# blefaudeux/rusty-marcher

Hardware: AMD Instinct MI355X
Metric: Mpixels/sec at 1920x1080, max-bounce=5 (higher is better)
Workload: dtype f64

## Files before the change

rusty-marcher_amd/csrc/rm_classify.inc:

```
namespace RM_FLAVOR_NS {
using namespace rmdev;

__device__ __forceinline__ V3 unit(V3 a) {
    const double x = dot(a, a);
    double y = __builtin_amdgcn_rsq(x);
    const double h = 0.5 * x;
    y = y * (1.5 - h * y * y);
    y = y * (1.5 - h * y * y);
    return scaled(a, y);
}

#if RM_KERNEL_ORIENTED
__device__ __forceinline__ V3 cls_dir(const KernelArgs &a, double bx, double by) {
    return mk((bx * a.cam_rx + by * a.cam_ux) + a.cam_fx, (bx * a.cam_ry + by * a.cam_uy) + a.cam_fy, (bx * a.cam_rz + by * a.cam_uz) + a.cam_fz);
}
#else
__device__ __forceinline__ V3 cls_dir(const KernelArgs &, double bx, double by) { return mk(bx, by, -1.); }
#endif
template <bool SHARED>
__device__ __forceinline__ bool cone_of(Bundle &b, const KernelArgs &a, double bx0, double bx1, double by0, double by1, uint32_t sub) {
    const V3 u = unit(cls_dir(a, 0.5 * (bx0 + bx1), 0.5 * (by0 + by1)));
    double cm;
    if (SHARED) {
        cm = dot(unit(cls_dir(a, (sub & 1u) ? bx1 : bx0, (sub & 2u) ? by1 : by0)), u);
        cm = __builtin_fmin(cm, __shfl_xor(cm, 1, 64));
        cm = __builtin_fmin(cm, __shfl_xor(cm, 2, 64));
    } else {
        cm = __builtin_fmin(__builtin_fmin(dot(unit(cls_dir(a, bx0, by0)), u), dot(unit(cls_dir(a, bx1, by0)), u)),
                            __builtin_fmin(dot(unit(cls_dir(a, bx0, by1)), u), dot(unit(cls_dir(a, bx1, by1)), u)));
    }
    cm -= 1e-9;
    b.ax = a.cam_x; b.ay = a.cam_y; b.az = a.cam_z;
    b.ux = u.x; b.uy = u.y; b.uz = u.z;
    b.cos2 = cm * cm;
    b.sin_t = (double)__builtin_sqrtf((float)__builtin_fmax((1. - cm) * (1. + cm), 0.)) * (1. + 1e-6) + 1e-7;
    b.chord = (double)__builtin_sqrtf((float)__builtin_fmax(2. * (1. - cm), 0.)) * (1. + 1e-6) + 1e-7;
    b.rho = 0.;
    b.two_sided = false;
    b.narrow = true;
    return cm > 0.5;
}

struct ClsView { const double *bounds, *planar, *poly, *tri; uint32_t poly_stride, tri_stride; };
__device__ __forceinline__ ClsView cls_view_of_blob(const double *blob, const rm_dev_header &H) {
    return ClsView{blob + H.off_bounds, blob + H.off_planar, blob + H.off_polygons, blob + H.off_triangles, RM_POLYGON_WORDS, RM_TRIANGLE_WORDS};
}
__device__ __forceinline__ uint32_t cls_stage_words(const rm_dev_header &H) {
    return 4u * (H.n_spheres + H.n_polygons + H.n_triangles) + 22u * (H.n_polygons + H.n_triangles);
}
__device__ __forceinline__ ClsView cls_stage(const double *__restrict__ blob, const rm_dev_header &H, double *lds) {
    const uint32_t lane = threadIdx.x & 63u, n = H.n_spheres + H.n_polygons + H.n_triangles, npl = H.n_polygons + H.n_triangles;
    double *bounds = lds, *planar = bounds + 4u * n, *poly = planar + 16u * npl, *tri = poly + 6u * H.n_polygons;
    cull_stage(blob, H, lds);
    for (uint32_t i = lane; i < 3u * H.n_polygons; i += 64u)
        reinterpret_cast<double2 *>(poly)[i] = reinterpret_cast<const double2 *>(blob + H.off_polygons + RM_POLYGON_WORDS * (i / 3u))[i % 3u];
    for (uint32_t i = lane; i < 3u * H.n_triangles; i += 64u)
        reinterpret_cast<double2 *>(tri)[i] = reinterpret_cast<const double2 *>(blob + H.off_triangles + RM_TRIANGLE_WORDS * (i / 3u))[i % 3u];
    __syncthreads();
    return ClsView{bounds, planar, poly, tri, 6u, 6u};
}

template <bool EDGES>
__device__ __forceinline__ bool keeps(const ClsView &v, const KernelArgs &a, const Bundle &b, uint32_t pid, bool in) {
    const uint32_t ns = a.H.n_spheres, np = a.H.n_polygons;
    const double2 *bp = reinterpret_cast<const double2 *>(v.bounds) + 2u * (in ? pid : 0u);
    const SphereCull sph = cull_sphere(bp, b);
    bool out = sph.out;
    const bool planar = in & (pid >= ns);
    if (EDGES && __any(planar)) {
        const double2 *pp = reinterpret_cast<const double2 *>(v.planar) + 8u * (planar ? pid - ns : 0u);
        out = out | cull_edges(pp, b, sph, planar & !out);
        const double *recw = !planar ? v.bounds : pid < ns + np ? v.poly + v.poly_stride * (pid - ns) : v.tri + v.tri_stride * (pid - ns - np);
        const double2 *rec = reinterpret_cast<const double2 *>(recw);
        const double2 r0 = rec[0], r1 = rec[1], r2 = rec[2];
        const double nn = (double)__builtin_sqrtf((float)(r0.x * r0.x + r0.y * r0.y + r1.x * r1.x)) * (1. + 1e-6);
        const double num = (r1.y - b.ax) * r0.x + (r2.x - b.ay) * r0.y + (r2.y - b.az) * r1.x;
        const double un = b.ux * r0.x + b.uy * r0.y + b.uz * r1.x, spread = (b.chord + 1e-7) * nn;
        const double tiny = 1e-9 * nn * (__builtin_fabs(r1.y - b.ax) + __builtin_fabs(r2.x - b.ay) + __builtin_fabs(r2.y - b.az)) + 1e-290;
        const bool away = ((num > tiny) & (un + spread < 0.)) | ((num < -tiny) & (un - spread > 0.));
        out = out | (planar & away);
    }
    return in & !out;
}

template <bool EDGES>
__device__ __forceinline__ void keeps2(const ClsView &v, const KernelArgs &a, const Bundle &b, uint32_t pid_a, bool in_a, uint32_t pid_b, bool in_b,
                                       bool &keep_a, bool &keep_b) {
    const uint32_t ns = a.H.n_spheres, np = a.H.n_polygons;
    const double2 *bounds = reinterpret_cast<const double2 *>(v.bounds);
    const SphereCull sph_a = cull_sphere(bounds + 2u * (in_a ? pid_a : 0u), b), sph_b = cull_sphere(bounds + 2u * (in_b ? pid_b : 0u), b);
    bool out_a = sph_a.out, out_b = sph_b.out;
    const bool planar_a = in_a & (pid_a >= ns), planar_b = in_b & (pid_b >= ns);
    if (EDGES && __any(planar_a | planar_b)) {
        const double2 *planar = reinterpret_cast<const double2 *>(v.planar);
        EdgeCull ea = cull_edges_begin(planar + 8u * (planar_a ? pid_a - ns : 0u), b, sph_a, planar_a & !out_a);
        EdgeCull eb = cull_edges_begin(planar + 8u * (planar_b ? pid_b - ns : 0u), b, sph_b, planar_b & !out_b);
        if (__any((ea.nv == 4u) | (eb.nv == 4u))) { cull_edges_fourth(ea, b); cull_edges_fourth(eb, b); }
        out_a = out_a | cull_edges_end(ea, b, planar_a & !out_a);
        out_b = out_b | cull_edges_end(eb, b, planar_b & !out_b);
        auto away = [&](uint32_t pid, bool planar_p) {
            const double *recw = !planar_p ? v.bounds : pid < ns + np ? v.poly + v.poly_stride * (pid - ns) : v.tri + v.tri_stride * (pid - ns - np);
            const double2 *rec = reinterpret_cast<const double2 *>(recw);
            const double2 r0 = rec[0], r1 = rec[1], r2 = rec[2];
            const double nn = (double)__builtin_sqrtf((float)(r0.x * r0.x + r0.y * r0.y + r1.x * r1.x)) * (1. + 1e-6);
            const double num = (r1.y - b.ax) * r0.x + (r2.x - b.ay) * r0.y + (r2.y - b.az) * r1.x;
            const double un = b.ux * r0.x + b.uy * r0.y + b.uz * r1.x, spread = (b.chord + 1e-7) * nn;
            const double tiny = 1e-9 * nn * (__builtin_fabs(r1.y - b.ax) + __builtin_fabs(r2.x - b.ay) + __builtin_fabs(r2.y - b.az)) + 1e-290;
            return planar_p & (((num > tiny) & (un + spread < 0.)) | ((num < -tiny) & (un - spread > 0.)));
        };
        const bool away_a = away(pid_a, planar_a), away_b = away(pid_b, planar_b);
        out_a = out_a | away_a;
        out_b = out_b | away_b;
    }
    keep_a = in_a & !out_a;
    keep_b = in_b & !out_b;
}

struct ClsAsked { double px0, px1, py0, py1, tx0, tx1, ty0, ty1; };
__device__ __forceinline__ ClsAsked classify_ask(const KernelArgs &a, uint32_t patch, bool valid) {
    const uint32_t tile = (valid ? patch : 0u) * 16u + (threadIdx.x & 15u);
    uint32_t tx0, ty0, tyf, ty8;
    tile_origin(a, tile, tx0, ty0, tyf, ty8);
    const uint32_t px0 = tx0 & ~31u, py0 = ty0 & ~31u;
    return ClsAsked{a.bp_x[px0], a.bp_x[px0 + 31u], a.bp_y[py0], a.bp_y[py0 + 31u],
                    a.bp_x[tx0], a.bp_x[tx0 + TILE_W - 1u], a.bp_y[ty0], a.bp_y[ty0 + TILE_H - 1u]};
}
template <bool EDGES>
__device__ __forceinline__ bool classify_patches(const ClsView &scene_blob, const KernelArgs &a, uint32_t patch, bool valid, const ClsAsked &asked,
                                                 unsigned long long *__restrict__ tile_mask, uint32_t n, uint32_t tag, unsigned long long &sig, unsigned long long &own) {
    const uint32_t lane = threadIdx.x & 63u, sub = lane & 15u;
    const uint32_t tile = (valid ? patch : 0u) * 16u + sub;

    Bundle b;
    const bool patch_usable = cone_of<true>(b, a, asked.px0, asked.px1, asked.py0, asked.py1, sub);
    unsigned long long pm = 0ull;
#ifdef RM_CLASSIFY_TWO_CHAINS
    for (uint32_t base = 0; base < n; base += 32u) {
        const uint32_t pid_a = base + sub, pid_b = base + 16u + sub;
        const bool in_a = pid_a < n, in_b = pid_b < n;
        bool keep_a, keep_b;
        keeps2<EDGES>(scene_blob, a, b, pid_a, in_a, pid_b, in_b, keep_a, keep_b);
        pm |= (in_a & (keep_a | !patch_usable)) ? (1ull << (pid_a & 63u)) : 0ull;
        pm |= (in_b & (keep_b | !patch_usable)) ? (1ull << (pid_b & 63u)) : 0ull;
    }
#else
    for (uint32_t base = 0; base < n; base += 16u) {
        const uint32_t pid = base + sub;
        const bool in = pid < n;
        const bool keep = in & (keeps<EDGES>(scene_blob, a, b, pid, in) | !patch_usable);
        pm |= keep ? (1ull << (pid & 63u)) : 0ull;
    }
#endif
    auto group_or = [](unsigned long long v) {
        for (uint32_t off = 1u; off < 16u; off <<= 1) {
            const uint32_t lo = (uint32_t)v | (uint32_t)__shfl_xor((int)(uint32_t)v, (int)off, 64);
            const uint32_t hi = (uint32_t)(v >> 32) | (uint32_t)__shfl_xor((int)(uint32_t)(v >> 32), (int)off, 64);
            v = ((unsigned long long)hi << 32) | lo;
        }
        return v;
    };
    pm = group_or(pm);

    unsigned long long mask = 0ull;
    if (n > (tag ? 56u : 64u)) {
        mask = pm != 0ull ? ~0ull : 0ull;
    } else if (__any(pm != 0ull)) {
        const bool tile_usable = cone_of<false>(b, a, asked.tx0, asked.tx1, asked.ty0, asked.ty1, sub);
        unsigned long long m = pm;
#ifdef RM_CLASSIFY_TWO_CHAINS
        while (__any(m != 0ull)) {
            const bool in_a = m != 0ull;
            const uint32_t pid_a = in_a ? (uint32_t)__builtin_ctzll(m) : 0u;
            m &= m - 1ull;
            const bool in_b = m != 0ull;
            const uint32_t pid_b = in_b ? (uint32_t)__builtin_ctzll(m) : 0u;
            m &= m - 1ull;
            bool keep_a, keep_b;
            keeps2<EDGES>(scene_blob, a, b, pid_a, in_a, pid_b, in_b, keep_a, keep_b);
            mask |= (in_a & (keep_a | !tile_usable)) ? (1ull << pid_a) : 0ull;
            mask |= (in_b & (keep_b | !tile_usable)) ? (1ull << pid_b) : 0ull;
        }
#else
        while (__any(m != 0ull)) {
            const bool in = m != 0ull;
            const uint32_t pid = in ? (uint32_t)__builtin_ctzll(m) : 0u;
            m &= m - 1ull;
            const bool keep = in & (keeps<EDGES>(scene_blob, a, b, pid, in) | !tile_usable);
            mask |= keep ? (1ull << pid) : 0ull;
        }
#endif
    }
    if (valid) {
        if (tag) __hip_atomic_store(tile_mask + tile, ((unsigned long long)tag << 56) | (mask & 0x00FFFFFFFFFFFFFFull), __ATOMIC_RELAXED, __HIP_MEMORY_SCOPE_AGENT);
        else tile_mask[tile] = mask;
    }
    own = valid ? mask : 0ull;
    sig = group_or(own);
    return sig != 0ull;
}

__device__ __forceinline__ uint32_t cost_bucket(uint32_t ticks) {
    if (ticks < 512u) return RM_ORD_SKY - 1u;
    const uint32_t e = 31u - (uint32_t)__builtin_clz(ticks);
    const uint32_t b = 2u * (e - 9u) + ((ticks >> (e - 1u)) & 1u);
    return RM_ORD_SKY - 1u - min(b, RM_ORD_SKY - 1u);
}

struct OrdRec { uint32_t patch, bucket_slot, index; };

// ... 131 lines not shown
```

rusty-marcher_amd/csrc/rm_device.hip:

```cpp
#include <hip/hip_runtime.h>

#include <chrono>
#include <cmath>
#include <cstdio>
#include <cstdlib>
#include <cstring>
#include <initializer_list>
#include <limits>
#include <new>
#include <string>
#include <utility>
#include <vector>

#include "rm_image.hpp"
#include "rm_internal.h"
#include "rm_kernel_args.hpp"
#include "rm_plan.hpp"
#include "rm_sampling.hpp"
#include "rm_query.hpp"
#include "rm_radiance.hpp"
#include "rm_refine.hpp"
#include "rm_lens.hpp"
#include "rm_accum.hpp"
#include "rm_soft.hpp"
// ... 133 lines not shown

    uint32_t *d_pid_map = nullptr;
    size_t pid_map_words = 0;
    void *d_query = nullptr;
    size_t query_bytes = 0;

    std::vector<std::pair<const void *, int>> shade_occupancy;

    void *d_refine_ws = nullptr;
    size_t refine_ws_bytes = 0;

    void *d_lens_table = nullptr;
    void *d_lens_frame = nullptr;
    size_t lens_frame_bytes = 0;

    rm_progressive *progressive = nullptr;

    rm_converging *converging = nullptr;

    unsigned long long *d_max = nullptr;
    uint8_t *d_rgb8 = nullptr;
    size_t rgb8_bytes = 0;
};

static void hostio_destroy(rm_ctx *ctx, bool device_ok);
static bool hostio_packs(rm_ctx *ctx, size_t band_bytes);
static void progressive_destroy(rm_ctx *ctx, bool device_ok);
static void converging_destroy(rm_ctx *ctx, bool device_ok);

static rm_status ctx_fail(rm_ctx *ctx, rm_status st, const std::string &msg) {
    if (ctx) ctx->error = msg;
    else rm_set_host_error(msg);
    return st;
}

template <class F>
static rm_status guarded(rm_ctx *ctx, const char *who, F &&body) {
    try {
        return body();
    } catch (const std::bad_alloc &) {
        return ctx_fail(ctx, RM_ERR_INVALID_ARG, std::string(who) + ": out of host memory");
    } catch (const std::exception &e) {
        return ctx_fail(ctx, RM_ERR_INVALID_ARG, std::string(who) + ": " + e.what());
    } catch (...) {
        return ctx_fail(ctx, RM_ERR_INVALID_ARG, std::string(who) + ": unexpected exception");
    }
}

template <class T>
static T *entry_of(std::vector<T> &v, hipStream_t stream) {
    T *t = nullptr;
    for (T &g : v)
        if (g.stream == stream) t = &g;
    return t;
}

#define RM_HIP(ctx, call)                                                                          \
    do {                                                                                           \
        hipError_t e__ = (call);                                                                   \
        if (e__ != hipSuccess)                                                                     \
            return ctx_fail(ctx, RM_ERR_HIP, std::string(#call) + ": " + hipGetErrorString(e__)); \
    } while (0)

static rm_status grow_device_buffer(rm_ctx *ctx, void **d, size_t *have, size_t need) {
    if (*have >= need) return RM_OK;
    if (*d) RM_HIP(ctx, hipFree(*d));
    *d = nullptr;
    *have = 0;
    RM_HIP(ctx, hipMalloc(d, need));
    *have = need;
    return RM_OK;
}

#define RM_DECLARE_GROUP(g) \
    const void *rm_pick_kernel_strict_g##g(bool edges, int order, int stack, int pow_mode); \
    const void *rm_pick_kernel_fast_g##g(bool edges, int order, int stack, int pow_mode);
#define RM_DECL_PICK_O(g) \
    const void *rm_pick_kernel_strict_o_g##g(bool edges, int order, int stack, int pow_mode); \
    const void *rm_pick_kernel_fast_o_g##g(bool edges, int order, int stack, int pow_mode);
RM_DECL_PICK_O(0) RM_DECL_PICK_O(1) RM_DECL_PICK_O(2) RM_DECL_PICK_O(3)
RM_DECLARE_GROUP(0) RM_DECLARE_GROUP(1) RM_DECLARE_GROUP(2) RM_DECLARE_GROUP(3) RM_DECLARE_GROUP(4)
#undef RM_DECLARE_GROUP

const void *rm_pick_kernel(bool fast, bool staged, bool bvh, bool cull, bool edges, int order, bool feedback, int stack, int pow_mode) {
    const int group = staged ? (cull ? 1 : 0) : !bvh ? 2 : feedback ? 4 : 3;
    if (staged && (bvh || feedback)) return nullptr;
    if (!staged && !cull) return nullptr;
    switch (group) {
    case 0: return fast ? rm_pick_kernel_fast_g0(edges, order, stack, pow_mode) : rm_pick_kernel_strict_g0(edges, order, stack, pow_mode);
    case 1: return fast ? rm_pick_kernel_fast_g1(edges, order, stack, pow_mode) : rm_pick_kernel_strict_g1(edges, order, stack, pow_mode);
    case 2: return fast ? rm_pick_kernel_fast_g2(edges, order, stack, pow_mode) : rm_pick_kernel_strict_g2(edges, order, stack, pow_mode);
    case 3: return fast ? rm_pick_kernel_fast_g3(edges, order, stack, pow_mode) : rm_pick_kernel_strict_g3(edges, order, stack, pow_mode);
    default: return fast ? rm_pick_kernel_fast_g4(edges, order, stack, pow_mode) : rm_pick_kernel_strict_g4(edges, order, stack, pow_mode);
    }
}

const void *rm_pick_kernel_oriented(bool fast, bool staged, bool bvh, bool cull, bool edges, int stack, int pow_mode) {
    const int group = staged ? (cull ? 1 : 0) : !bvh ? 2 : 3;
    if (staged && bvh) return nullptr;
    if (!staged && !cull) return nullptr;
    switch (group) {
    case 0: return fast ? rm_pick_kernel_fast_o_g0(edges, 1, stack, pow_mode) : rm_pick_kernel_strict_o_g0(edges, 1, stack, pow_mode);
    case 1: return fast ? rm_pick_kernel_fast_o_g1(edges, 1, stack, pow_mode) : rm_pick_kernel_strict_o_g1(edges, 1, stack, pow_mode);
    case 2: return fast ? rm_pick_kernel_fast_o_g2(edges, 1, stack, pow_mode) : rm_pick_kernel_strict_o_g2(edges, 1, stack, pow_mode);
    default: return fast ? rm_pick_kernel_fast_o_g3(edges, 1, stack, pow_mode) : rm_pick_kernel_strict_o_g3(edges, 1, stack, pow_mode);
    }
}

extern "C" {

const char *rm_build_info(void) {
    return "rusty-marcher_amd " RM_BUILD_FLAVOR " gfx950 abi5 queries camera ranges radiance antialias lens progressive soft motion moving-shapes converge-motion converge";
}

const char *rm_last_error(const rm_ctx *ctx) {
    return ctx ? ctx->error.c_str() : rm_get_host_error();
}

rm_status rm_init(int device_ordinal, rm_ctx **out) {
    if (!out) return ctx_fail(nullptr, RM_ERR_INVALID_ARG, "rm_init: out is NULL");
    *out = nullptr;
    int n = 0;
    hipError_t e = hipGetDeviceCount(&n);
    if (e != hipSuccess || n <= 0)
        return ctx_fail(nullptr, RM_ERR_NO_DEVICE,
                        std::string("rm_init: no HIP device visible (") + hipGetErrorString(e) +
                            "); this backend has no CPU fallback");
    if (device_ordinal < 0 || device_ordinal >= n)
        return ctx_fail(nullptr, RM_ERR_NO_DEVICE, "rm_init: device ordinal out of range");
    rm_ctx *ctx = new rm_ctx();
    ctx->device = device_ordinal;
    auto bail = [&](const char *what, hipError_t err) {
        rm_set_host_error(std::string("rm_init: ") + what + ": " + hipGetErrorString(err));
        delete ctx;
        return RM_ERR_HIP;
    };
    if ((e = hipSetDevice(device_ordinal)) != hipSuccess) return bail("hipSetDevice", e);
    if ((e = hipGetDeviceProperties(&ctx->prop, device_ordinal)) != hipSuccess) return bail("hipGetDeviceProperties", e);
    if (std::string(ctx->prop.gcnArchName).rfind("gfx950", 0) != 0) {
        rm_set_host_error(std::string("rm_init: device is ") + ctx->prop.gcnArchName +
                          ", this library carries gfx950 code only");
        delete ctx;
        return RM_ERR_NO_DEVICE;
    }
    if ((e = hipStreamCreateWithFlags(&ctx->stream, hipStreamNonBlocking)) != hipSuccess) return bail("hipStreamCreate", e);
    if ((e = hipEventCreate(&ctx->ev0)) != hipSuccess) return bail("hipEventCreate", e);
    if ((e = hipEventCreate(&ctx->ev1)) != hipSuccess) return bail("hipEventCreate", e);
    if ((e = hipMalloc(&ctx->d_max, sizeof(unsigned long long))) != hipSuccess) return bail("hipMalloc", e);
    if ((e = hipMalloc(&ctx->d_redo, sizeof(uint32_t))) != hipSuccess) return bail("hipMalloc", e);
    if ((e = hipMemset(ctx->d_redo, 0, sizeof(uint32_t))) != hipSuccess) return bail("hipMemset", e);
    *out = ctx;
    return RM_OK;
}

void rm_destroy(rm_ctx *ctx) {
    if (!ctx) return;
    (void)hipSetDevice(ctx->device);
    if (ctx->stream && !ctx->comm_failed) (void)hipStreamSynchronize(ctx->stream);
    rm_comm_destroy(ctx);
    const bool device_ok = !ctx->comm_stuck;
    hostio_destroy(ctx, device_ok);
    progressive_destroy(ctx, device_ok);
    converging_destroy(ctx, device_ok);
    if (device_ok) {
        for (rm_frame_slot &s : ctx->slots) {
            if (s.render && !ctx->comm_failed) { (void)hipStreamSynchronize(s.render); (void)hipStreamDestroy(s.render); }
            for (hipEvent_t e : {s.begun, s.rendered, s.gathered, s.exchanged})
// ... 501 lines not shown
        ctx->frame_w = params->frame_width;
        ctx->frame_h = params->frame_height;
    }

    const size_t row_bytes = (size_t)params->frame_width * 3u * sizeof(double);
    const uint32_t n_rows = band.count();
    if (host_rgb && n_rows > 0 && hostio_packs(ctx, (size_t)n_rows * 32u * row_bytes)) {
        std::vector<double *> rows(params->frame_height);
        for (uint32_t y = 0; y < params->frame_height; y++) rows[y] = host_rgb + (size_t)y * params->frame_width * 3u;
        return rm_render_rows(ctx, params, rows.data(), timing);
    }
    RM_HIP(ctx, hipEventRecord(ctx->ev0, ctx->stream));
    st = launch_render(ctx, params, band, ctx->d_frame, nullptr, ctx->stream);
    if (st != RM_OK) return st;
    RM_HIP(ctx, hipEventRecord(ctx->ev1, ctx->stream));

    double d2h_ms = 0.;
    if (host_rgb && n_rows > 0) {
        RM_HIP(ctx, hipStreamSynchronize(ctx->stream));
        const auto t0 = std::chrono::steady_clock::now();
        const uint32_t run = band.stride == 1 ? n_rows : 1u;
        for (uint32_t k = 0; k < n_rows; k += run) {
            const size_t off = (size_t)(band.begin + k * band.stride) * 32u * row_bytes;
            RM_HIP(ctx, hipMemcpy((char *)host_rgb + off, (const char *)ctx->d_frame + off, (size_t)run * 32u * row_bytes,
                                  hipMemcpyDeviceToHost));
        }
        d2h_ms = std::chrono::duration<double, std::milli>(std::chrono::steady_clock::now() - t0).count();
    } else {
        RM_HIP(ctx, hipStreamSynchronize(ctx->stream));
    }
    if (rm_status vst = void_frame_check(ctx, "rm_render")) return vst;
    if (timing) {
        float ms = 0.f;
        RM_HIP(ctx, hipEventElapsedTime(&ms, ctx->ev0, ctx->ev1));
        timing->kernel_ms = ms;
        timing->d2h_ms = d2h_ms;
        timing->total_ms = std::chrono::duration<double, std::milli>(std::chrono::steady_clock::now() - t_begin).count();
    }
    return RM_OK;
}

rm_status rm_render(rm_ctx *ctx, const rm_params *params, double *host_rgb, rm_timing *timing) {
    return guarded(ctx, "rm_render", [&]() { return rm_render_impl(ctx, params, host_rgb, timing); });
}

rm_status rm_kernel_name(rm_ctx *ctx, const rm_params *params, char *buf, size_t buflen) {
    if (!ctx) return ctx_fail(nullptr, RM_ERR_INVALID_ARG, "rm_kernel_name: NULL ctx");
    if (!buf || buflen == 0) return ctx_fail(ctx, RM_ERR_INVALID_ARG, "rm_kernel_name: NULL buffer");
    rm_band band;
    rm_status st = check_params(ctx, params, &band);
    if (st != RM_OK) return st;
    if (params->max_depth == 0) { std::snprintf(buf, buflen, "rm_fill_band_kernel"); return RM_OK; }
    rm_kernel_choice k;
    st = choose_kernel(ctx, params, band.count() * (params->frame_width / RM_PATCH_SIZE) * 16u, &k);
    if (st != RM_OK) return st;
    std::snprintf(buf, buflen, "%s%s::rm_render_static<%d, %d, %d, %d, %s, %s, %s, %s, %s, %s>", k.fast ? "rmdev_fast" : "rmdev_strict", ctx->oriented ? "_o" : "", k.stack,
                  k.pow_mode, k.mode.waves, k.mode.per_wave, k.staged ? "true" : "false", k.bvh ? "true" : "false",
                  k.cull ? "true" : "false", k.edges ? "true" : "false", (k.order || ctx->oriented) ? "true" : "false", k.feedback ? "true" : "false");
    return RM_OK;
}

rm_status rm_launch_stats(rm_ctx *ctx, uint32_t *workgroups, uint32_t *tail_patches) {
    if (!ctx) return ctx_fail(nullptr, RM_ERR_INVALID_ARG, "rm_launch_stats: NULL ctx");
    if (workgroups) *workgroups = ctx->last_launch_grid;
    if (tail_patches) *tail_patches = ctx->last_launch_tail;
    return RM_OK;
}

static rm_status rm_tile_stats_impl(rm_ctx *ctx, void *hip_stream, uint32_t *tiles, uint32_t *tiles_listed) {
    if (!ctx) return ctx_fail(nullptr, RM_ERR_INVALID_ARG, "rm_tile_stats: NULL ctx");
    RM_HIP(ctx, hipSetDevice(ctx->device));
    RM_HIP(ctx, hipDeviceSynchronize());
    const uint32_t n = ctx->last_launch_tiles;
    uint32_t listed = n;
    for (const rm_tile_lists &t : ctx->tile_lists)
        if (t.stream == (hip_stream ? (hipStream_t)hip_stream : ctx->last_launch_stream) && t.block && ctx->last_launch_classified && n <= t.cap) {
            std::vector<unsigned long long> m(n);
            RM_HIP(ctx, hipMemcpy(m.data(), t.mask(), (size_t)n * 8u, hipMemcpyDeviceToHost));
            listed = 0;
            uint32_t hist[64] = {};
            uint64_t bits = 0;
            for (unsigned long long v : m) {
                if (t.s.tagged) v &= 0x00FFFFFFFFFFFFFFull;
                listed += v != 0ull;
                for (int b = 0; b < 64 && v != ~0ull; b++)
                    if (v >> b & 1ull) { hist[b]++; bits++; }
            }
            if (std::getenv("RM_DEBUG_CLASSIFY")) {
                std::fprintf(stderr, "[rm_classify] %u of %u tiles have something to hit, %.2f primitives each; tiles per pid:", listed, n,
                             listed ? (double)bits / listed : 0.);
                for (int b = 0; b < 64; b++)
                    if (hist[b]) std::fprintf(stderr, " %d:%u", b, hist[b]);
                std::fprintf(stderr, "\n");
            }
        }
    if (tiles) *tiles = n;
    if (tiles_listed) *tiles_listed = listed;
    return RM_OK;
}

rm_status rm_tile_stats(rm_ctx *ctx, void *hip_stream, uint32_t *tiles, uint32_t *tiles_listed) {
    return guarded(ctx, "rm_tile_stats", [&]() { return rm_tile_stats_impl(ctx, hip_stream, tiles, tiles_listed); });
}

rm_status rm_device_framebuffer(rm_ctx *ctx, void **device_rgb, size_t *bytes) {
    if (!ctx) return ctx_fail(nullptr, RM_ERR_INVALID_ARG, "rm_device_framebuffer: NULL ctx");
    if (!ctx->d_frame) return ctx_fail(ctx, RM_ERR_INVALID_ARG, "rm_device_framebuffer: nothing rendered yet");
    if (device_rgb) *device_rgb = ctx->d_frame;
    if (bytes) *bytes = ctx->frame_bytes;
    return RM_OK;
}

static rm_status rm_postprocess_impl(rm_ctx *ctx, void *device_rgb, uint32_t w, uint32_t h, int normalize, uint8_t *host_rgb8,
                         double *max_out) {
    if (!ctx) return ctx_fail(nullptr, RM_ERR_INVALID_ARG, "rm_postprocess: NULL ctx");
    RM_HIP(ctx, hipSetDevice(ctx->device));
    double *v = (double *)device_rgb;
    if (!v) {
        if (!ctx->d_frame) return ctx_fail(ctx, RM_ERR_INVALID_ARG, "rm_postprocess: nothing rendered yet");
        if (w != ctx->frame_w || h != ctx->frame_h)
            return ctx_fail(ctx, RM_ERR_INVALID_ARG, "rm_postprocess: size differs from the rendered frame");
        v = ctx->d_frame;
    }
    const size_t n = (size_t)w * h * 3u;
    if (n == 0) return ctx_fail(ctx, RM_ERR_INVALID_ARG, "rm_postprocess: empty frame");
    const unsigned blocks = (unsigned)std::min<size_t>((n + 255) / 256, 2048);
    RM_HIP(ctx, hipMemsetAsync(ctx->d_max, 0, sizeof(unsigned long long), ctx->stream));
    if (normalize) {
        hipLaunchKernelGGL(rm_max_kernel, dim3(blocks), dim3(256), 0, ctx->stream, v, n, ctx->d_max);
        RM_HIP(ctx, hipGetLastError());
    }
    uint8_t *d8 = nullptr;
    if (host_rgb8) {
        if (ctx->rgb8_bytes < n) {
            RM_HIP(ctx, hipStreamSynchronize(ctx->stream));
            if (ctx->d_rgb8) RM_HIP(ctx, hipFree(ctx->d_rgb8));
            ctx->d_rgb8 = nullptr;
            ctx->rgb8_bytes = 0;
            RM_HIP(ctx, hipMalloc(&ctx->d_rgb8, n));
            ctx->rgb8_bytes = n;
        }
        d8 = ctx->d_rgb8;
    }
    if (normalize || d8) {
        hipLaunchKernelGGL(rm_scale_quantize_kernel, dim3(blocks), dim3(256), 0, ctx->stream, v, n, ctx->d_max,
                           normalize ? 1 : 0, d8);
        RM_HIP(ctx, hipGetLastError());
    }
    RM_HIP(ctx, hipStreamSynchronize(ctx->stream));
    if (host_rgb8) RM_HIP(ctx, hipMemcpy(host_rgb8, d8, n, hipMemcpyDeviceToHost));
    if (max_out) {
        unsigned long long bits = 0;
        RM_HIP(ctx, hipMemcpy(&bits, ctx->d_max, sizeof bits, hipMemcpyDeviceToHost));
        std::memcpy(max_out, &bits, sizeof bits);
    }
    return RM_OK;
}

rm_status rm_postprocess(rm_ctx *ctx, void *device_rgb, uint32_t w, uint32_t h, int normalize, uint8_t *host_rgb8,
                         double *max_out) {
    return guarded(ctx, "rm_postprocess", [&]() { return rm_postprocess_impl(ctx, device_rgb, w, h, normalize, host_rgb8, max_out); });
}

}

#include "rm_exchange.inc"
#include "rm_hostio.inc"
#include "rm_query_host.inc"
#include "rm_shade_host.inc"
#include "rm_radiance_host.inc"
#include "rm_refine_host.inc"
#include "rm_lens_host.inc"
#include "rm_accum_host.inc"
#include "rm_soft_host.inc"
#include "rm_motion_host.inc"
#include "rm_motion_shapes_host.inc"
#include "rm_converge_host.inc"
#include "rm_converge_motion_host.inc"
```

rusty-marcher_amd/csrc/rm_kernel_args.hpp:

```cpp
#ifndef RM_KERNEL_ARGS_HPP
#define RM_KERNEL_ARGS_HPP

#include <stdint.h>

#include "rm_internal.h"

#define RM_ORD_BUCKETS 16u
#define RM_ORD_SKY 15u
#define RM_ORD_MAX_CLS 1024u
#define RM_ORD_LINE 32u
#define RM_ORD_SUBS 4u
#define RM_ORD_COUNTERS (RM_ORD_BUCKETS * RM_ORD_SUBS)
#define RM_ORD_FIRST (RM_ORD_COUNTERS * RM_ORD_LINE)
#define RM_ORD_ARRIVE (2u * RM_ORD_COUNTERS * RM_ORD_LINE)
#define RM_ORD_GROUPS (RM_ORD_ARRIVE + (RM_ORD_MAX_CLS / 32u) * RM_ORD_LINE)
#define RM_ORD_GO (RM_ORD_GROUPS + RM_ORD_LINE)
#define RM_ORD_CNT_WORDS (RM_ORD_GO + RM_ORD_LINE)
#define RM_ORD_STATIC_BIT 0x80000000u
#define RM_ORD_FALLBACK_BIT 0x80000000u
#define RM_ORD_PATIENCE 4096u
#define RM_ORD_PATCH_BITS 20u
#define RM_ORD_SKY_BIT (1u << RM_ORD_PATCH_BITS)
#define RM_ORD_TAG_SHIFT (RM_ORD_PATCH_BITS + 1u)
#define RM_ORD_TAG_BITS 11u
// ... 12 lines not shown
enum { POW_GENERIC = 0, POW_INTEGER = 1 };


#ifndef RM_TILE_W
#define RM_TILE_W 16
#endif
constexpr uint32_t TILE_W = RM_TILE_W, TILE_H = 64u / RM_TILE_W;
static_assert(TILE_W == 8 || TILE_W == 16 || TILE_W == 32, "tile width");

struct KernelArgs {
    rm_dev_header H;
    double half_fov, height, width, ratio;
    double cam_x, cam_y, cam_z;
    double bg_x, bg_y, bg_z;
    uint32_t frame_width;
    uint32_t patch_row_begin;
    uint32_t patch_row_stride;
    uint32_t u8_compact;
    uint32_t max_depth;
    uint32_t n_width;
    uint32_t n_tiles;
    uint32_t order_mul;
    uint32_t order_add;
    uint32_t f64_compact;
    double cull_cos;
    uint8_t *frame8;
    const double *bp_x, *bp_y;
    unsigned long long *debug_stamps;
    const uint32_t *fb_list;
    const uint32_t *fb_count;
    const uint8_t *fb_flag;
    const uint32_t *fb_hist;
    uint32_t *fb_next_list, *fb_next_count, *fb_next_hist;
    uint8_t *fb_next_flag;
    uint32_t *fb_zero;
    uint32_t *fb_threshold;
    uint32_t fb_cap;
    uint32_t fb_long_ticks;
    uint32_t fb_target;
    const unsigned long long *tile_mask;
    uint32_t mask_exact;
    uint32_t mask_tag;
    uint32_t mask_tag_prev;
    uint32_t cls_blocks;
    uint32_t cls_prims;
    uint32_t cls_lds_words;
    uint32_t cull_lds_words;
    uint32_t *ord_cnt;
    uint32_t *ord_cnt_next;
    uint32_t *ord_flat;
    const uint32_t *ord_read;
    uint32_t ord_read_tag;
    uint32_t *ord_rec;
    uint32_t ord_cap;
    uint32_t ord_tag;
    uint32_t cls_iters;
    const uint32_t *static_list;
    const uint32_t *dyn_index;
    const uint32_t *dyn_inv;
    uint32_t *static_next, *dyn_index_next, *dyn_inv_next;
    const uint32_t *lists_done;
    uint32_t lists_tag;
    uint32_t *lists_done_next;
    uint32_t n_static;
    uint32_t key_mode;
    uint32_t *patch_cost;
    const uint32_t *cost_prev;
    uint32_t *cost_zero;
    const uint32_t *ctab;
    uint32_t *ctab_cur;
    uint32_t *ctab_zero;
    uint32_t tail_patches;
    uint32_t ov_cap;
    uint32_t first_round;
    uint32_t tail_q;
    unsigned long long *ord_hint;
    unsigned long long *err_word;
    uint32_t launch_seq;
    uint32_t test_stall;
    double cam_rx, cam_ry, cam_rz, cam_ux, cam_uy, cam_uz, cam_fx, cam_fy, cam_fz;
    uint32_t exact_only;
    uint32_t dead_children;
    uint32_t *redo_count;
};

struct ClassifyArgs {
    unsigned long long *tile_mask;
    uint32_t n_prims;
    uint32_t _pad;
};

const void *rm_classify_kernel(bool edges);
const void *rm_classify_kernel_oriented(bool edges);

#define RM_FB_BUCKETS 64u
#define RM_FB_SAMPLE 8u
struct StackEntry {
    double ox, oy, oz, dx, dy, dz, w;
    uint32_t depth, _pad;
};

#define RM_WAVE_L0_DEPTH_WORDS 448u
#define RM_WAVE_BVH_STACK_WORDS 480u
#define RM_WAVE_SUM_WORDS 512u
#define RM_WAVE_PAIR_WORDS 704u
#define RM_WAVE_T0_WORDS 736u
#define RM_WAVE_LDS_WORDS 738u
#define RM_LDS_SCENE_LIMIT_WORDS 512u

}

const void *rm_pick_kernel(bool fast, bool staged, bool bvh, bool cull, bool edges, int order, bool feedback, int stack, int pow_mode);
const void *rm_pick_kernel_oriented(bool fast, bool staged, bool bvh, bool cull, bool edges, int stack, int pow_mode);

#endif
```

rusty-marcher_amd/csrc/rm_kernels.hip:

```cpp
#include "rm_render_kernel.hpp"

#if RM_KERNEL_FAST && RM_KERNEL_ORIENTED
namespace flavour = rmdev_fast_o;
#elif RM_KERNEL_FAST
namespace flavour = rmdev_fast;
#elif RM_KERNEL_ORIENTED
namespace flavour = rmdev_strict_o;
#else
namespace flavour = rmdev_strict;
#endif

using namespace rmdev;

namespace {

template <bool STAGED, bool BVH, bool CULL, bool EDGES, bool ORDER, bool FB>
const void *pick(int stack, int pow_mode) {
#define RM_ROW(S)                                                                                                            \
    if (stack == S)                                                                                                          \
        return pow_mode == POW_INTEGER ? (const void *)flavour::rm_render_static<S, POW_INTEGER, 1, 1, STAGED, BVH, CULL, EDGES, ORDER, FB> \
                                       : (const void *)flavour::rm_render_static<S, POW_GENERIC, 1, 1, STAGED, BVH, CULL, EDGES, ORDER, FB>;
    RM_ROW(4) RM_ROW(8) RM_ROW(16) RM_ROW(32)
#undef RM_ROW
    return nullptr;
}

}

#define RM_PICK_CAT2(a, b, c) rm_pick_kernel_##a##_g##b
#define RM_PICK_CAT(a, b) RM_PICK_CAT2(a, b, )
#if RM_KERNEL_FAST && RM_KERNEL_ORIENTED
#define RM_PICK_NAME RM_PICK_CAT(fast_o, RM_KERNEL_GROUP)
#elif RM_KERNEL_FAST
#define RM_PICK_NAME RM_PICK_CAT(fast, RM_KERNEL_GROUP)
#elif RM_KERNEL_ORIENTED
#define RM_PICK_NAME RM_PICK_CAT(strict_o, RM_KERNEL_GROUP)
#else
#define RM_PICK_NAME RM_PICK_CAT(strict, RM_KERNEL_GROUP)
#endif

template <bool STAGED, bool BVH, bool CULL, bool FB>
static const void *pick_eo(bool edges, int order, int stack, int pow_mode) {
#if RM_KERNEL_ORIENTED
    static_assert(!FB, "no oriented kernels with the tile-level feedback");
    (void)order;
    if constexpr (CULL) {
        if (edges) return pick<STAGED, BVH, CULL, true, true, false>(stack, pow_mode);
    }
    return pick<STAGED, BVH, CULL, false, true, false>(stack, pow_mode);
#else
    if constexpr (FB) {
        return edges ? pick<STAGED, BVH, CULL, true, false, true>(stack, pow_mode) : pick<STAGED, BVH, CULL, false, false, true>(stack, pow_mode);
    } else {
        if constexpr (CULL) {
            if (edges) return order ? pick<STAGED, BVH, CULL, true, true, false>(stack, pow_mode) : pick<STAGED, BVH, CULL, true, false, false>(stack, pow_mode);
        }
        return order ? pick<STAGED, BVH, CULL, false, true, false>(stack, pow_mode) : pick<STAGED, BVH, CULL, false, false, false>(stack, pow_mode);
    }
#endif
}

const void *RM_PICK_NAME(bool edges, int order, int stack, int pow_mode) {
#if RM_KERNEL_GROUP == 0
    return pick_eo<true, false, false, false>(false, order, stack, pow_mode);
#elif RM_KERNEL_GROUP == 1
    return pick_eo<true, false, true, false>(edges, order, stack, pow_mode);
#elif RM_KERNEL_GROUP == 2
    return pick_eo<false, false, true, false>(edges, order, stack, pow_mode);
#elif RM_KERNEL_GROUP == 3
    return pick_eo<false, true, true, false>(edges, order, stack, pow_mode);
#elif RM_KERNEL_GROUP == 4 && !RM_KERNEL_ORIENTED
    return pick_eo<false, true, true, true>(edges, 0, stack, pow_mode);
#else
#error "RM_KERNEL_GROUP must be 0..4"
#endif
}
```

rusty-marcher_amd/csrc/rm_plan.cpp:

```cpp
#include "rm_plan.hpp"

#include <algorithm>
#include <cmath>
#include <cstdlib>
#include <cstring>
#include <string>

using namespace rmdev;

namespace {

enum knob_rule {
    IS_1,
    NOT_0,
    IS_SET,
    ONE_OR_ZERO,
    ATOI,
    ATOI_MIN_0,
    ATOI_MIN_1,
    STRTOUL,
    TILE_ORDER,
    TAIL_PLACE,
    CULL_OFF,
    CULL_COS,
};

struct knob {
    const char *name;
    knob_rule rule;
    bool rm_knobs::*b = nullptr;
    int rm_knobs::*i = nullptr;
    uint32_t rm_knobs::*u = nullptr;
    double rm_knobs::*d = nullptr;
    constexpr knob(const char *n, bool rm_knobs::*f, knob_rule r) : name(n), rule(r), b(f) {}
    constexpr knob(const char *n, int rm_knobs::*f, knob_rule r) : name(n), rule(r), i(f) {}
    constexpr knob(const char *n, uint32_t rm_knobs::*f, knob_rule r) : name(n), rule(r), u(f) {}
    constexpr knob(const char *n, double rm_knobs::*f, knob_rule r) : name(n), rule(r), d(f) {}
};

const knob k_knobs[] = {
    {"RM_FORCE_GENERIC_POW", &rm_knobs::force_generic_pow, IS_1},
    {"RM_FORCE_FAST_FP", &rm_knobs::force_fast_fp, IS_1},
    {"RM_FORCE_UNSTAGED", &rm_knobs::force_unstaged, IS_1},
    {"RM_SHADOW_MASKS", &rm_knobs::shadow_masks, NOT_0},
    {"RM_DEAD_CHILDREN", &rm_knobs::dead_children, NOT_0},
    {"RM_DISABLE_BVH", &rm_knobs::disable_bvh, IS_1},
    {"RM_FORCE_STACK", &rm_knobs::force_stack, ATOI},
    {"RM_FEEDBACK", &rm_knobs::feedback_mode, ONE_OR_ZERO},
    {"RM_FEEDBACK_US", &rm_knobs::feedback_us, ATOI_MIN_1},
    {"RM_FEEDBACK_TARGET", &rm_knobs::feedback_target, ATOI_MIN_0},
    {"RM_DEBUG_EMPTY", &rm_knobs::debug_empty, IS_1},
    {"RM_TILE_CLASSIFY", &rm_knobs::classify_mode, ONE_OR_ZERO},
    {"RM_CLASSIFY_IN_LAUNCH", &rm_knobs::classify_in_launch, IS_1},
    {"RM_PATCH_ORDER", &rm_knobs::patch_order_mode, ONE_OR_ZERO},
    {"RM_SKY_TAIL", &rm_knobs::sky_tail, NOT_0},
    {"RM_SKY_TAIL_FORCE", &rm_knobs::sky_tail_force, ATOI},
    {"RM_PATCH_ORDER_MAX", &rm_knobs::patch_order_max, ATOI_MIN_0},
    {"RM_SKY_TAIL_BIG", &rm_knobs::sky_tail_big, NOT_0},
    {"RM_PATCH_ORDER_MAX_DEEP", &rm_knobs::patch_order_max_deep, ATOI_MIN_0},
    {"RM_SKY_TAIL_ROOM_DIV", &rm_knobs::sky_tail_room_div, ATOI_MIN_1},
    {"RM_SKY_TAIL_BIG_MIN", &rm_knobs::sky_tail_big_min, ATOI_MIN_0},
    {"RM_SKY_TAIL_PLACE", &rm_knobs::sky_tail_place, TAIL_PLACE},
    {"RM_SKY_TAIL_MOTION", &rm_knobs::sky_tail_motion, NOT_0},
    {"RM_SKY_TAIL_CAP", &rm_knobs::sky_tail_cap, ATOI_MIN_0},
    {"RM_ORDER_KEYS", &rm_knobs::order_keys, ATOI},
    {"RM_FIRST_ROUND", &rm_knobs::first_round, ATOI_MIN_0},
    {"RM_FIRST_ROUND_FROM_ORDER", &rm_knobs::first_round_from_order, NOT_0},
    {"RM_ORDER_REUSE", &rm_knobs::order_reuse, NOT_0},
    {"RM_STATIC_ROUNDS", &rm_knobs::static_rounds, ATOI_MIN_1},
    {"RM_CLS_MAX_BLOCKS", &rm_knobs::cls_max_blocks, ATOI_MIN_1},
    {"RM_ORDER_FREEZE", &rm_knobs::order_freeze, ATOI_MIN_0},
    {"RM_ORDER_LATE_PLACES", &rm_knobs::order_late_places, NOT_0},
    {"RM_MASK_REUSE", &rm_knobs::mask_reuse, NOT_0},
    {"RM_CLASSIFY_LDS", &rm_knobs::classify_lds, NOT_0},
    {"RM_CLASSIFY_IN_LAUNCH_PRIMS", &rm_knobs::classify_in_launch_prims, ATOI_MIN_0},
    {"RM_CLASSIFY_MIN_TILES", &rm_knobs::classify_min_tiles, ATOI_MIN_0},
    {"RM_ORD_TAG_WRAP", &rm_knobs::ord_tag_wrap, ATOI_MIN_1},
    {"RM_TEST_STALL_ORDER", &rm_knobs::test_stall_order, ATOI},
    {"RM_TILE_ORDER", &rm_knobs::tile_order, TILE_ORDER},
    {"RM_DISABLE_CULL", &rm_knobs::cull_cos, CULL_OFF},
    {"RM_CULL_COS", &rm_knobs::cull_cos, CULL_COS},
    {"RM_CULL_MIN", &rm_knobs::cull_min_prims, STRTOUL},
    {"RM_CULL_EDGES", &rm_knobs::cull_edges, NOT_0},
    {"RM_CHECKED_NUMERICS", &rm_knobs::checked_numerics, NOT_0},
    {"RM_REFINE_MAX_BLOCKS", &rm_knobs::refine_max_blocks, ATOI_MIN_0},
    {"RM_LENS_MAX_BLOCKS", &rm_knobs::lens_max_blocks, ATOI_MIN_0},
    {"RM_DEBUG_TAIL", &rm_knobs::debug_tail, IS_SET},
};

}

rm_knobs rm_knobs_from_env() {
    rm_knobs kn;
    for (const knob &k : k_knobs) {
        const char *env = std::getenv(k.name);
        if (!env) continue;
        switch (k.rule) {
        case IS_1: kn.*k.b = env[0] == '1'; break;
        case NOT_0: kn.*k.b = env[0] != '0'; break;
        case IS_SET: kn.*k.b = true; break;
        case ONE_OR_ZERO: kn.*k.i = env[0] == '1' ? 1 : 0; break;
        case ATOI: kn.*k.i = std::atoi(env); break;
        case ATOI_MIN_0:
            if (k.i) kn.*k.i = std::max(0, std::atoi(env));
            else kn.*k.u = (uint32_t)std::max(0, std::atoi(env));
            break;
        case ATOI_MIN_1: kn.*k.u = (uint32_t)std::max(1, std::atoi(env)); break;
        case STRTOUL: kn.*k.u = (uint32_t)std::strtoul(env, nullptr, 10); break;
        case TILE_ORDER:
            kn.*k.i = !std::strcmp(env, "reverse") ? TILE_ORDER_REVERSE : !std::strcmp(env, "hash") ? TILE_ORDER_HASH : TILE_ORDER_NATURAL;
            break;
        case TAIL_PLACE: kn.*k.i = env[0] == 'e' && env[1] == 'v' ? 1 : env[0] == 'e' ? 2 : 0; break;
        case CULL_OFF: kn.*k.d = env[0] == '1' ? 2. : kn.*k.d; break;
        case CULL_COS: kn.*k.d = std::max(0.05, std::atof(env)); break;
        }
    }
    if (kn.classify_min_tiles == 0u) kn.classify_min_tiles = RM_CLASSIFY_MIN_TILES_DEFAULT;
    return kn;
}


static constexpr size_t RM_LDS_SCENE_LIMIT_BYTES = RM_LDS_SCENE_LIMIT_WORDS * sizeof(double);
static constexpr uint32_t RM_FEEDBACK_MIN_TILES = 32768;
static constexpr uint32_t RM_CLASSIFY_MAX_COST = 4000;
static constexpr uint32_t RM_CLASSIFY_IN_LAUNCH_MAX_COST = 1000;

bool choose_kernel(const rm_knobs &kn, const rm_plan_scene &sc, const rm_params &p, uint32_t tiles, rm_kernel_choice *k) {
    const rm_dev_header &H = *sc.H;
// ... 64 lines not shown

bool plan_launch(const rm_knobs &kn, const rm_plan_scene &sc, const rm_params &p, const rm_band &band, const rm_stream_state &before,
                 uint32_t order_cap, const rm_feedback_state &fb, unsigned long long hint, rm_launch_plan *out) {
    rm_launch_plan &P = *out;
    KernelArgs &a = P.args;
    const rm_dev_header &H = *sc.H;
    a.H = H;
    a.half_fov = p.half_fov; a.height = p.height; a.width = p.width; a.ratio = p.ratio;
    a.cam_x = sc.camera.x; a.cam_y = sc.camera.y; a.cam_z = sc.camera.z;
    const rm_camera_basis &cb = *sc.basis;
    a.cam_rx = cb.right.x; a.cam_ry = cb.right.y; a.cam_rz = cb.right.z;
    a.cam_ux = cb.up.x; a.cam_uy = cb.up.y; a.cam_uz = cb.up.z;
    a.cam_fx = cb.forward.x; a.cam_fy = cb.forward.y; a.cam_fz = cb.forward.z;
    if (!(std::fabs(sc.camera.x) + std::fabs(sc.camera.y) + std::fabs(sc.camera.z) <= sc.occ_camera_limit)) a.H.off_occ = 0u;
    a.bg_x = p.background.x; a.bg_y = p.background.y; a.bg_z = p.background.z;
    P.exact_only = !kn.checked_numerics || sc.exact_only || rm_camera_exact_only(sc);
    a.exact_only = P.exact_only ? 1u : 0u;
    a.frame_width = p.frame_width;
    a.patch_row_begin = band.begin;
    a.patch_row_stride = band.stride;
    a.u8_compact = (p.flags & RM_FLAG_U8_COMPACT) ? 1u : 0u;
    a.f64_compact = (p.flags & RM_FLAG_F64_COMPACT) ? 1u : 0u;
    a.max_depth = p.max_depth;
    a.n_width = p.frame_width / RM_PATCH_SIZE;
    a.n_tiles = band.count() * a.n_width * 16u;
    a.order_mul = 1; a.order_add = 0;
    if (kn.tile_order == TILE_ORDER_REVERSE && a.n_tiles > 1) {
        a.order_mul = a.n_tiles - 1; a.order_add = a.n_tiles - 1;
    } else if (kn.tile_order == TILE_ORDER_HASH && a.n_tiles > 2) {
        uint32_t mul = (uint32_t)(a.n_tiles * 0.6180339887) | 1u;
        auto gcd = [](uint32_t x, uint32_t y) { while (y) { uint32_t t = x % y; x = y; y = t; } return x; };
        while (gcd(mul, a.n_tiles) != 1) mul += 2;
        a.order_mul = mul % a.n_tiles;
    }

    if (!choose_kernel(kn, sc, p, a.n_tiles, &P.k)) return false;
    const rm_kernel_choice &k = P.k;
    const uint32_t n_prims = k.n_prims, n_planar = k.n_planar;
    a.dead_children = (kn.dead_children && !k.bvh && !k.cull && sc.dead_camera_limit > 0. &&
                       std::fabs(sc.camera.x) + std::fabs(sc.camera.y) + std::fabs(sc.camera.z) <= sc.dead_camera_limit) ? 1u : 0u;
    const uint32_t cull_steps = (n_prims + 63u) / 64u;
    const uint32_t planar_steps = n_planar ? cull_steps - H.n_spheres / 64u : 0u;
    const uint32_t cull_cost = 25u * cull_steps + (k.planar_edges ? 85u * planar_steps : 0u);
    a.cull_cos = cull_cost > RM_CULL_MAX_COST ? 2. : kn.cull_cos;
    a.first_round = sc.n_cus * 4u * (k.edges ? RM_EDGES_WAVES : RM_MIN_WAVES);
    if (kn.first_round >= 0) a.first_round = (uint32_t)kn.first_round;
    P.block = (uint32_t)k.mode.waves * 64u;
    P.lds_bytes = k.lds_bytes;
    const uint32_t per_wg = (uint32_t)(k.mode.waves * k.mode.per_wave);
    P.grid = (a.n_tiles + per_wg - 1) / per_wg;
    P.feedback = k.feedback && per_wg == 1u && !kn.debug_empty;
    if (P.feedback) {
        const rm_feedback_layout L(a.n_tiles);
        rm_feedback_state &next = P.feedback_after;
        next.valid = true;
        next.key[0] = (uint64_t)a.n_tiles | ((uint64_t)p.frame_width << 32);
        next.key[1] = (uint64_t)band.begin | ((uint64_t)band.stride << 32);
        next.key[2] = sc.scene_epoch;
        next.n_tiles = a.n_tiles;
        const bool same = fb.valid && fb.n_tiles == a.n_tiles && std::memcmp(fb.key, next.key, sizeof fb.key) == 0;
        P.feedback_reset = !same;
        P.feedback_bytes = L.bytes();
        P.feedback_set_bytes = L.set_bytes;
        const int r = same ? fb.cur : 0, w = (r + 1) % 3, z = (r + 2) % 3;
        next.cur = w;
        point(P, &KernelArgs::fb_list, RM_BUF_FEEDBACK, L.list(r)); point(P, &KernelArgs::fb_count, RM_BUF_FEEDBACK, L.count(r));
        point(P, &KernelArgs::fb_flag, RM_BUF_FEEDBACK, L.flag(r)); point(P, &KernelArgs::fb_hist, RM_BUF_FEEDBACK, L.hist(r));
        point(P, &KernelArgs::fb_next_list, RM_BUF_FEEDBACK, L.list(w)); point(P, &KernelArgs::fb_next_count, RM_BUF_FEEDBACK, L.count(w));
        point(P, &KernelArgs::fb_next_flag, RM_BUF_FEEDBACK, L.flag(w)); point(P, &KernelArgs::fb_next_hist, RM_BUF_FEEDBACK, L.hist(w));
        point(P, &KernelArgs::fb_zero, RM_BUF_FEEDBACK, L.hist(z));
        point(P, &KernelArgs::fb_threshold, RM_BUF_FEEDBACK, L.threshold());
        a.fb_cap = L.cap;
        a.fb_long_ticks = kn.feedback_us * 100u;
        const uint32_t slots = sc.n_cus * 16u;
        a.fb_target = kn.feedback_target >= 0 ? (uint32_t)kn.feedback_target : 4u * slots;
        a.fb_target = std::min(a.fb_target, L.cap / 2u);
        P.grid = a.n_tiles + L.cap;
    }
    if (kn.debug_empty) a.n_tiles = 0;

    rm_stream_state s = before;
    uint32_t mask_tag_before = 0u;
    uint32_t cls_words_wanted = 0u;
    P.classify = kn.classify_mode != 0 && !kn.debug_empty && per_wg == 1u && n_prims > 0u &&
                 k.classify_cost <= RM_CLASSIFY_MAX_COST && (kn.classify_mode == 1 || a.n_tiles >= kn.classify_min_tiles);
    if (P.classify) {
        const bool in_launch = kn.classify_in_launch && (n_prims <= kn.classify_in_launch_prims || k.order_in_big_scene) && !k.feedback;
        if (in_launch) {
            if (!s.tagged || s.tagged_tiles != a.n_tiles || s.tagged_scene != sc.scene_epoch || s.tag >= 255u) {
                P.clear_masks = true;
                s.tag = 0;
                s.tagged = true; s.tagged_tiles = a.n_tiles; s.tagged_scene = sc.scene_epoch;
            }
            a.mask_tag = ++s.tag;
            mask_tag_before = a.mask_tag > 1u ? a.mask_tag - 1u : 0u;
            a.cls_blocks = (a.n_tiles / 16u + 3u) / 4u;
            a.cls_prims = n_prims;
            P.grid += a.cls_blocks;
            cls_words_wanted = (!k.staged && kn.classify_lds) ? 4u * n_prims + 22u * n_planar : 0u;
        } else {
            s.tagged = false;
            P.cls_fn = sc.oriented ? rm_classify_kernel_oriented(n_planar > 0u) : rm_classify_kernel(n_planar > 0u);
            P.cls_grid = (a.n_tiles / 16u + 3u) / 4u;
            P.cls_args.n_prims = n_prims;
        }
        point(P, &KernelArgs::tile_mask, RM_BUF_MASKS, 0);
        a.mask_exact = n_prims <= (in_launch ? 56u : 64u) ? 1u : 0u;
    }
    const uint32_t n_patches = a.n_tiles / 16u;
    const uint64_t rounds = (uint64_t)a.first_round * kn.static_rounds * 2u <= a.n_tiles ? kn.static_rounds : 1u;
    a.n_static = (uint32_t)std::min<uint64_t>(((uint64_t)a.first_round * rounds) & ~15ull, a.n_tiles);
    const uint32_t n_dyn = n_patches - a.n_static / 16u;
    const uint32_t cls_max = std::min<uint32_t>(RM_ORD_MAX_CLS, std::max(1u, kn.cls_max_blocks));
    P.ordered = k.order && per_wg == 1u && a.cls_blocks != 0u && n_dyn > 0u && n_patches < (1u << RM_ORD_PATCH_BITS) &&
                n_patches <= 16u * 4u * cls_max;
    if (P.ordered) {
        const uint64_t key[3] = {(uint64_t)a.n_tiles | ((uint64_t)p.frame_width << 32), (uint64_t)band.begin | ((uint64_t)band.stride << 32),
                                 sc.scene_epoch ^ ((uint64_t)a.n_static << 40)};
        P.order_patches = n_patches;
        const bool grown = order_cap < n_patches;
        const rm_order_layout L{grown ? n_patches : order_cap};
        P.order_cap = (uint32_t)L.cap;
        const uint32_t tag_wrap = kn.ord_tag_wrap ? kn.ord_tag_wrap : (1u << RM_ORD_TAG_BITS) - 1u;
        const bool fresh = grown || std::memcmp(s.order_key, key, sizeof key) != 0;
        if (fresh || s.ord_tag >= tag_wrap) {
            P.order_clear = fresh ? rm_launch_plan::ORDER_CLEAR_ALL : rm_launch_plan::ORDER_CLEAR_FLAT;
            if (fresh) {
                std::memcpy(s.order_key, key, sizeof key);
                s.order_frames = 0;
                s.static_read = s.static_written = -1;
                s.list_tag[0] = s.list_tag[1] = 0u;
            }
            s.ord_tag = 0;
            s.last_tag = 0;
        }
        const uint32_t f = s.order_frames++;
        const uint32_t seq = ++s.seq;
        if (f == 0u) s.key_seq0 = seq;
        const double view[16] = {sc.camera.x, sc.camera.y, sc.camera.z, p.half_fov, p.height, p.width, p.ratio,
                                 cb.right.x, cb.right.y, cb.right.z, cb.up.x, cb.up.y, cb.up.z, cb.forward.x, cb.forward.y, cb.forward.z};
        if (f == 0u || std::memcmp(s.view, view, sizeof view) != 0) {
            std::memcpy(s.view, view, sizeof view);
            s.view_seq0 = seq;
        }
        const bool timed = n_patches <= (k.order_in_big_scene ? kn.patch_order_max_deep : kn.patch_order_max);
        const uint32_t groups4 = (n_patches + 3u) / 4u;
        a.cls_iters = (groups4 + cls_max - 1u) / cls_max;
        a.cls_blocks = (groups4 + a.cls_iters - 1u) / a.cls_iters;
        const bool reuse = kn.order_reuse && f >= 3u && seq >= s.view_seq0 + 3u && s.last_tag != 0u;
        a.ord_cap = P.order_cap;
        a.ord_tag = ++s.ord_tag;
        a.ord_read_tag = reuse ? s.last_tag : a.ord_tag;
        s.last_tag = a.ord_tag;
        const bool late_places = reuse && kn.order_late_places;
        a.mask_tag_prev = reuse && kn.mask_reuse ? mask_tag_before : 0u;
        P.frozen = kn.order_freeze > 0 && reuse && f >= 4u && before.frozen_run < (uint32_t)kn.order_freeze && a.mask_tag > 1u &&
                   a.mask_tag_prev != 0u && late_places && kn.test_stall_order == 0 && kn.sky_tail_force < 0 && !kn.debug_tail;
        const bool lays_out = !P.frozen;
        point(P, &KernelArgs::ord_cnt, RM_BUF_ORDER, 4u * L.cnt(f & 1u));
        point(P, &KernelArgs::ord_flat, RM_BUF_ORDER, 4u * L.flat(f & 1u));
        point(P, &KernelArgs::ord_read, RM_BUF_ORDER, 4u * L.flat(reuse ? (f + 1u) & 1u : f & 1u));
        if (lays_out) point(P, &KernelArgs::ord_cnt_next, RM_BUF_ORDER, 4u * L.cnt((f + 1u) & 1u));
        if (lays_out && late_places) point(P, &KernelArgs::ord_rec, RM_BUF_ORDER, 4u * L.rec());
        if (timed) point(P, &KernelArgs::patch_cost, RM_BUF_ORDER, 4u * L.cost(f % 3u));
        if (timed) point(P, &KernelArgs::cost_prev, RM_BUF_ORDER, 4u * L.cost((f + 2u) % 3u));
        if (timed && lays_out) point(P, &KernelArgs::cost_zero, RM_BUF_ORDER, 4u * L.cost((f + 1u) % 3u));
        point(P, &KernelArgs::ctab, RM_BUF_ORDER, 4u * L.ctab((f + 2u) % 3u));
        if (timed && kn.order_keys != 1) point(P, &KernelArgs::ctab_cur, RM_BUF_ORDER, 4u * L.ctab(f % 3u));
        if (lays_out) point(P, &KernelArgs::ctab_zero, RM_BUF_ORDER, 4u * L.ctab((f + 1u) % 3u));
        if (kn.first_round_from_order) {
            const int read = reuse ? s.static_read : s.static_written;
            const uint32_t write = read == 0 ? 1u : 0u;
            if (read >= 0) {
                point(P, &KernelArgs::static_list, RM_BUF_ORDER, 4u * L.first((uint32_t)read));
                point(P, &KernelArgs::dyn_index, RM_BUF_ORDER, 4u * L.index((uint32_t)read));
                point(P, &KernelArgs::dyn_inv, RM_BUF_ORDER, 4u * L.inv((uint32_t)read));
                point(P, &KernelArgs::lists_done, RM_BUF_ORDER, 4u * (L.done() + (uint32_t)read));
                a.lists_tag = s.list_tag[read];
            }
            if (lays_out) {
                point(P, &KernelArgs::static_next, RM_BUF_ORDER, 4u * L.first(write));
                point(P, &KernelArgs::dyn_index_next, RM_BUF_ORDER, 4u * L.index(write));
                point(P, &KernelArgs::dyn_inv_next, RM_BUF_ORDER, 4u * L.inv(write));
                point(P, &KernelArgs::lists_done_next, RM_BUF_ORDER, 4u * (L.done() + write));
            }
            s.list_tag[write] = a.ord_tag;
            s.static_read = read;
            s.static_written = (int)write;
        } else {
            s.static_read = s.static_written = -1;
        }
        a.key_mode = !timed || f == 0u || kn.order_keys == 0 ? RM_KEY_PLACE
                   : (seq > s.view_seq0 && kn.order_keys != 2) ? RM_KEY_COST
                   : (a.mask_exact && a.mask_tag && kn.order_keys != 1) ? RM_KEY_CONTENT : RM_KEY_PLACE;
        point(P, &KernelArgs::ord_hint, RM_BUF_HINT, 0);
        point(P, &KernelArgs::err_word, RM_BUF_HINT, sizeof(unsigned long long));
        a.launch_seq = seq;
        a.test_stall = (uint32_t)kn.test_stall_order;
        uint32_t tail = 0, cap = 0;
        if (kn.sky_tail) {
            bool guess = false;
            if (kn.sky_tail_force >= 0) {
                tail = std::min((uint32_t)kn.sky_tail_force, n_dyn);
                guess = true;
            } else {
                const uint32_t h_seq = (uint32_t)(hint >> 32), n_lit = (uint32_t)hint;
                const bool valid = h_seq >= s.key_seq0 && h_seq < seq && hint != 0ull && n_lit <= n_dyn;
                guess = h_seq < s.view_seq0 + 1u;
                if (valid && (!guess || kn.sky_tail_motion)) tail = n_dyn - n_lit;
                if (tail < 8u) tail = 0u;
            }
            if (tail) cap = std::min(tail, kn.sky_tail_cap >= 0 ? (uint32_t)kn.sky_tail_cap : guess ? std::max(768u, n_patches / kn.sky_tail_room_div) : 32u);
        }
        a.tail_patches = tail;
        a.ov_cap = cap;
        const uint64_t behind = 16ull * (n_dyn - tail);
        a.tail_q = (tail && behind) ? (uint32_t)((((uint64_t)tail << 32) + behind + tail - 1u) / (behind + tail)) : 0u;
        if (a.tail_q > 1u && (kn.sky_tail_place == 2 || (kn.sky_tail_place == 0 && timed))) a.tail_q = 1u;
        if (P.frozen) {
            a.cls_blocks = 0u; a.cls_iters = 0u; a.cls_prims = 0u;
            a.mask_tag = a.mask_tag_prev = before.tag;
            cls_words_wanted = 0u;
            s = before;
            s.frozen_run = before.frozen_run + 1u;
        } else {
            s.frozen_run = 0u;
        }
        P.grid = a.cls_blocks + a.n_static + 16u * (n_dyn - tail) + tail + 16u * cap + (lays_out && late_places ? a.cls_blocks : 0u);
    }
    if (cls_words_wanted) {
        const uint32_t rec_words = (std::max(a.cls_iters, 1u) * 4u * 3u + 1u) / 2u;
        if (cls_words_wanted + rec_words <= (k.edges ? 1664u : 1248u)) {
            a.cls_lds_words = cls_words_wanted;
            P.lds_bytes = std::max(P.lds_bytes, (size_t)(cls_words_wanted + rec_words) * sizeof(double));
        }
    }
    P.after = s;
    return true;
// ... 8 lines not shown
    band->end = e;
    band->stride = p.patch_row_stride == 0 ? 1u : p.patch_row_stride;
    return true;
}

struct rmi_plan_case {
    uint32_t n_spheres, n_polygons, n_triangles, total_words;
    uint32_t bvh, integer_exponents, oriented, n_cus;
    uint64_t scene_epoch;
    rm_params params;
    rm_vec3 camera;
    rm_camera_basis basis;
    unsigned long long hint;
};
struct rmi_plan_row {
    uint32_t grid, block, lds_bytes;
    uint32_t fast, stack, pow_mode, waves, per_wave, staged, bvh, cull, edges, order, feedback;
    uint32_t classify, classify_in_front, ordered, frozen;
    uint32_t clear_masks, order_patches, order_clear;
    uint32_t n_tiles, cls_blocks, cls_iters, n_static, tail_patches, ov_cap, key_mode, mask_tag, mask_tag_prev, ord_tag, ord_read_tag, launch_seq;
    uint32_t reads_own_order, late_places;
    rm_stream_state after;
};
extern "C" rm_status rmi_plan_launches(const rmi_plan_case *cases, uint32_t n, rmi_plan_row *rows) {
    if (!cases || !rows) { rm_set_host_error("rmi_plan_launches: NULL argument"); return RM_ERR_INVALID_ARG; }
    const rm_knobs kn = rm_knobs_from_env();
    rm_stream_state s;
    rm_feedback_state fb;
    uint32_t order_cap = 0;
    for (uint32_t i = 0; i < n; i++) {
        const rmi_plan_case &c = cases[i];
        rm_dev_header H{};
        H.n_spheres = c.n_spheres; H.n_polygons = c.n_polygons; H.n_triangles = c.n_triangles; H.total_words = c.total_words;
        H.off_bvh_spheres = c.bvh;
        const rm_plan_scene sc{&H, c.scene_epoch, 0., c.integer_exponents != 0, c.oriented != 0, c.camera, &c.basis, c.n_cus};
        rm_band band;
        rm_launch_plan P;
        if (!rm_band_of(c.params, &band) || band.count() == 0 || !plan_launch(kn, sc, c.params, band, s, order_cap, fb, c.hint, &P)) {
            rm_set_host_error("rmi_plan_launches: launch " + std::to_string(i) + " has no plan");
            return RM_ERR_INVALID_ARG;
        }
        auto offset_of = [&](size_t field) {
            for (uint32_t r = 0; r < P.n_refs; r++)
                if (P.refs[r].field == field) return P.refs[r].offset + 1u;
            return 0u;
        };
        const KernelArgs &a = P.args;
        const rm_kernel_choice &k = P.k;
        rows[i] = rmi_plan_row{P.grid, P.block, (uint32_t)P.lds_bytes,
                               k.fast, (uint32_t)k.stack, (uint32_t)k.pow_mode, (uint32_t)k.mode.waves, (uint32_t)k.mode.per_wave, k.staged, k.bvh, k.cull, k.edges, k.order || c.oriented, k.feedback,
                               P.classify, P.cls_fn != nullptr, P.ordered, P.frozen, P.clear_masks, P.order_patches, (uint32_t)P.order_clear,
                               a.n_tiles, a.cls_blocks, a.cls_iters, a.n_static, a.tail_patches, a.ov_cap, a.key_mode, a.mask_tag, a.mask_tag_prev, a.ord_tag, a.ord_read_tag, a.launch_seq,
                               P.ordered && offset_of(offsetof(KernelArgs, ord_read)) == offset_of(offsetof(KernelArgs, ord_flat)), offset_of(offsetof(KernelArgs, ord_rec)) != 0u,
                               P.after};
        if (P.classify) s = P.after;
        if (P.ordered) order_cap = P.order_cap;
        if (P.feedback) fb = P.feedback_after;
    }
    return RM_OK;
}

extern "C" rm_status rmi_plan_dead_children(const rm_vec3 *camera, double dead_camera_limit, uint32_t n_spheres, uint32_t n_polygons,
                                            uint32_t n_triangles, uint32_t total_words, uint32_t *out) {
    if (!camera || !out) { rm_set_host_error("rmi_plan_dead_children: NULL argument"); return RM_ERR_INVALID_ARG; }
    const rm_knobs kn = rm_knobs_from_env();
    rm_dev_header H{};
    H.n_spheres = n_spheres; H.n_polygons = n_polygons; H.n_triangles = n_triangles; H.total_words = total_words;
    const rm_camera_basis basis{rm_vec3{1., 0., 0.}, rm_vec3{0., 1., 0.}, rm_vec3{0., 0., -1.}};
    const rm_plan_scene sc{&H, 1u, 0., true, false, *camera, &basis, 256u, false, dead_camera_limit};
    rm_params p{};
    p.half_fov = 0.75; p.height = 64.; p.width = 64.; p.ratio = 1.;
    p.frame_width = 64; p.frame_height = 64; p.max_depth = 3;
    rm_band band;
    rm_launch_plan P;
    if (!rm_band_of(p, &band) || !plan_launch(kn, sc, p, band, rm_stream_state{}, 0u, rm_feedback_state{}, 0ull, &P)) {
        rm_set_host_error("rmi_plan_dead_children: no plan");
        return RM_ERR_INVALID_ARG;
    }
    out[0] = P.args.dead_children;
    out[1] = (!P.k.bvh && !P.k.cull) ? 1u : 0u;
    return RM_OK;
}

extern "C" rm_status rmi_plan_exact_only(const rm_vec3 *camera, const rm_camera_basis *basis, uint32_t oriented, uint32_t scene_exact_only, uint32_t *out) {
    if (!camera || !basis || !out) { rm_set_host_error("rmi_plan_exact_only: NULL argument"); return RM_ERR_INVALID_ARG; }
    const rm_knobs kn = rm_knobs_from_env();
    rm_dev_header H{};
    H.n_spheres = 1; H.total_words = 128;
    const rm_plan_scene sc{&H, 1u, 0., true, oriented != 0, *camera, basis, 256u, scene_exact_only != 0};
    rm_params p{};
    p.half_fov = 0.75; p.height = 64.; p.width = 64.; p.ratio = 1.;
    p.frame_width = 64; p.frame_height = 64; p.max_depth = 3;
    rm_band band;
    rm_launch_plan P;
    if (!rm_band_of(p, &band) || !plan_launch(kn, sc, p, band, rm_stream_state{}, 0u, rm_feedback_state{}, 0ull, &P)) {
        rm_set_host_error("rmi_plan_exact_only: no plan");
        return RM_ERR_INVALID_ARG;
    }
    *out = (P.exact_only ? 1u : 0u) | (P.args.exact_only ? 2u : 0u);
    return RM_OK;
}

extern "C" rm_status rmi_shading_launch(const uint32_t *header, uint32_t integer_exponents, uint32_t max_depth, uint32_t *variant,
                                        uint32_t total, uint32_t rays_per_pixel, int32_t n_cus, int32_t per_cu, uint32_t max_blocks,
                                        uint32_t *grid) {
    if (header) {
        if (!variant) { rm_set_host_error("rmi_shading_launch: NULL variant"); return RM_ERR_INVALID_ARG; }
        rm_dev_header H{};
        std::memcpy(&H, header, 19u * sizeof(uint32_t));
        const rm_shading_variant v = rm_shading_variant_of(rm_knobs_from_env(), H, integer_exponents != 0, max_depth);
        variant[0] = v.bvh ? 1u : 0u; variant[1] = (uint32_t)v.pow_mode; variant[2] = (uint32_t)v.stack;
    }
    if (grid) {
        if (rays_per_pixel < 1u || rays_per_pixel > 64u) { rm_set_host_error("rmi_shading_launch: rays_per_pixel is outside 1..64"); return RM_ERR_INVALID_ARG; }
        *grid = rm_shading_grid(total, rays_per_pixel, n_cus, per_cu, max_blocks);
    }
    return RM_OK;
}
```

rusty-marcher_amd/csrc/rm_plan.hpp:

```cpp
#ifndef RM_PLAN_HPP
#define RM_PLAN_HPP

#include <stddef.h>
#include <stdint.h>

#include "rm_internal.h"
#include "rm_kernel_args.hpp"

enum { TILE_ORDER_NATURAL = 0, TILE_ORDER_REVERSE = 1, TILE_ORDER_HASH = 2 };

static constexpr uint32_t RM_CLASSIFY_MIN_TILES_DEFAULT = 3584;
static constexpr uint32_t RM_CULL_MIN_PRIMS = 12, RM_CULL_EDGES_MIN_PLANAR = 4, RM_CULL_MAX_COST = 250;

struct rm_knobs {
    bool force_generic_pow = false;
    bool force_fast_fp = false;
    int tile_order = TILE_ORDER_REVERSE;
    bool disable_bvh = false;
    double cull_cos = 0.975;
    uint32_t cull_min_prims = RM_CULL_MIN_PRIMS;
    bool cull_edges = true;
    bool force_unstaged = false;
    bool shadow_masks = true;
    bool dead_children = true;
    int force_stack = 0;
    bool debug_empty = false;
    int feedback_mode = -1;
    uint32_t feedback_us = 50;
    int feedback_target = -1;
    int classify_mode = -1;
    bool classify_in_launch = true;
    bool sky_tail = true;
    uint32_t patch_order_max = 4096;
    uint32_t patch_order_max_deep = 65536;
    uint32_t sky_tail_big_min = 16384;
    uint32_t sky_tail_room_div = 16;
    bool sky_tail_big = true;
    bool sky_tail_motion = true;
    int sky_tail_place = 0;
    int sky_tail_cap = -1;
    bool classify_lds = true;
    uint32_t classify_in_launch_prims = 56;
    uint32_t classify_min_tiles = RM_CLASSIFY_MIN_TILES_DEFAULT;
    bool mask_reuse = true;
    uint32_t static_rounds = 2;
    uint32_t cls_max_blocks = RM_ORD_MAX_CLS;
    int order_freeze = 7;
    bool order_late_places = true;
    bool order_reuse = true;
    bool first_round_from_order = true;
    int first_round = -1;
    int order_keys = -1;
    uint32_t ord_tag_wrap = 0;
    int test_stall_order = 0;
    int sky_tail_force = -1;
    int patch_order_mode = -1;
    bool checked_numerics = true;
    uint32_t refine_max_blocks = 0;
    uint32_t lens_max_blocks = 0;
    bool debug_tail = false;
};
rm_knobs rm_knobs_from_env();

struct rm_band {
    uint32_t begin = 0, end = 0, stride = 1;
    uint32_t count() const { return end > begin ? (end - begin + stride - 1) / stride : 0; }
};

bool rm_band_of(const rm_params &p, rm_band *band);

struct rm_plan_scene {
    const rm_dev_header *H;
    uint64_t scene_epoch;
    double occ_camera_limit;
    bool integer_exponents;
    bool oriented;
    rm_vec3 camera;
    const rm_camera_basis *basis;
    uint32_t n_cus;
    bool exact_only = false;
    double dead_camera_limit = 0.;
};

static constexpr double RM_CHECKED_COORD_MAX = 0x1p+200;
static constexpr double RM_CHECKED_R2_MIN = 0x1p-600, RM_CHECKED_R2_MAX = 0x1p+600;
inline bool rm_checked_coord_ok(double v) { return v >= -RM_CHECKED_COORD_MAX && v <= RM_CHECKED_COORD_MAX; }
bool rm_camera_exact_only(const rm_plan_scene &sc);

struct rm_launch_mode {
    int waves = 0;
    int per_wave = 1;
};

struct rm_kernel_choice {
    const void *fn = nullptr;
    rm_launch_mode mode;
    size_t lds_bytes = 0;
    int stack = 0, pow_mode = 0;
    bool fast = false, staged = false, bvh = false, cull = false, edges = false, order = false, feedback = false;
    bool order_in_big_scene = false;
    uint32_t n_prims = 0, n_planar = 0, classify_cost = 0;
    bool planar_edges = false;
};
bool choose_kernel(const rm_knobs &kn, const rm_plan_scene &sc, const rm_params &p, uint32_t tiles, rm_kernel_choice *k);

struct rm_shading_variant {
    bool bvh;
    int pow_mode;
    int stack;
};
rm_shading_variant rm_shading_variant_of(const rm_knobs &kn, const rm_dev_header &H, bool integer_exponents, uint32_t max_depth);

uint32_t rm_shading_grid(uint32_t total, uint32_t rays_per_pixel, int n_cus, int per_cu, uint32_t max_blocks);

struct rm_stream_state {
    uint32_t order_frames = 0;
    uint64_t order_key[3] = {0, 0, 0};
    uint32_t list_tag[2] = {0, 0};
    int static_read = -1, static_written = -1;
    uint32_t last_tag = 0;
    uint32_t seq = 0, view_seq0 = 0, key_seq0 = 0, ord_tag = 0;
    double view[16] = {0., 0., 0., 0., 0., 0., 0., 0., 0., 0., 0., 0., 0., 0., 0., 0.};
    uint32_t tag = 0, tagged_tiles = 0;
    uint64_t tagged_scene = 0;
    bool tagged = false;
    uint32_t frozen_run = 0;
};

struct rm_feedback_state {
    bool valid = false;
    uint64_t key[3] = {0, 0, 0};
    uint32_t n_tiles = 0;
    int cur = 0;
};

struct rm_order_layout {
    size_t cap;
    size_t cost(uint32_t j) const { return (size_t)j * cap; }
    size_t ctab(uint32_t j) const { return 3u * cap + j * RM_CTAB_WORDS; }
    size_t cnt(uint32_t j) const { return 3u * cap + 3u * RM_CTAB_WORDS + j * RM_ORD_CNT_WORDS; }
    size_t flat(uint32_t j) const { return cnt(2) + (size_t)j * cap; }
    size_t first(uint32_t j) const { return flat(2u + j); }
    size_t index(uint32_t j) const { return flat(4u + j); }
    size_t inv(uint32_t j) const { return flat(6u + j); }
    size_t rec() const { return flat(8u); }
    size_t done() const { return rec() + 3u * (cap + 4096u); }
    size_t bytes() const { return (cap * 11u + 64u + 3u * (cap + 4096u) + 3u * RM_CTAB_WORDS + 2u * RM_ORD_CNT_WORDS) * 4u; }
};

struct rm_feedback_layout {
    uint32_t n_tiles, cap;
    size_t set_bytes;
    explicit rm_feedback_layout(uint32_t tiles)
        : n_tiles(tiles), cap((tiles + 7u) / 8u > 64u ? (tiles + 7u) / 8u : 64u),
          set_bytes((((size_t)cap + RM_FB_BUCKETS + 4u) * sizeof(uint32_t) + tiles + 255u) & ~(size_t)255u) {}
    size_t hist(int j) const { return (size_t)j * set_bytes; }
    size_t count(int j) const { return hist(j) + RM_FB_BUCKETS * 4u; }
    size_t list(int j) const { return hist(j) + (RM_FB_BUCKETS + 4u) * 4u; }
    size_t flag(int j) const { return list(j) + (size_t)cap * 4u; }
    size_t threshold() const { return hist(3); }
    size_t bytes() const { return 3u * set_bytes + 256u; }
};

enum rm_buf : uint8_t { RM_BUF_MASKS, RM_BUF_ORDER, RM_BUF_HINT, RM_BUF_FEEDBACK, RM_BUF_COUNT };
struct rm_arg_ref {
    uint16_t field;
    rm_buf buf;
    uint32_t offset;
};

struct rm_launch_plan {
    rm_kernel_choice k;
    uint32_t grid = 0, block = 0;
    size_t lds_bytes = 0;
    rmdev::KernelArgs args{};
    rm_arg_ref refs[40];
    uint32_t n_refs = 0;
    bool feedback = false;
    bool classify = false;
    const void *cls_fn = nullptr;
    uint32_t cls_grid = 0;
    rmdev::ClassifyArgs cls_args{};
    bool exact_only = false;
    bool ordered = false;
    bool frozen = false;
    bool feedback_reset = false;
    size_t feedback_bytes = 0, feedback_set_bytes = 0;
    bool clear_masks = false;
    uint32_t order_patches = 0;
    enum { ORDER_CLEAR_NONE, ORDER_CLEAR_FLAT, ORDER_CLEAR_ALL } order_clear = ORDER_CLEAR_NONE;
    uint32_t order_cap = 0;
    rm_stream_state after;
    rm_feedback_state feedback_after;
};

bool plan_launch(const rm_knobs &kn, const rm_plan_scene &sc, const rm_params &p, const rm_band &band, const rm_stream_state &s,
                 uint32_t order_cap, const rm_feedback_state &fb, unsigned long long hint, rm_launch_plan *out);

#endif
```

rusty-marcher_amd/csrc/rm_render_kernel.hpp:

```cpp
#ifndef RM_RENDER_KERNEL_HPP
#define RM_RENDER_KERNEL_HPP

#include <hip/hip_runtime.h>

#include "rm_kernel_args.hpp"

namespace rmdev {

__device__ __forceinline__ uint32_t fb_bucket(uint32_t ticks) {
    const uint32_t t = ticks < 4u ? 4u : ticks;
    const uint32_t e = 31u - (uint32_t)__builtin_clz(t);
    const uint32_t b = 4u * (e - 2u) + ((t >> (e - 2u)) & 3u);
    return b < RM_FB_BUCKETS ? b : RM_FB_BUCKETS - 1u;
}
__device__ __forceinline__ uint32_t fb_edge(uint32_t b) { return (4u + (b & 3u)) << (b >> 2); }

__device__ __forceinline__ double own_sgpr(double v) { double r; asm("s_mov_b64 %0, %1" : "=s"(r) : "s"(v)); return r; }
__device__ __forceinline__ uint32_t own_sgpr(uint32_t v) { uint32_t r; asm("s_mov_b32 %0, %1" : "=s"(r) : "s"(v)); return r; }

__device__ __forceinline__ uint32_t uniform_u32(uint32_t v) { return (uint32_t)__builtin_amdgcn_readfirstlane((int)v); }
__device__ __forceinline__ unsigned long long uniform_u64(unsigned long long v) {
    return ((unsigned long long)uniform_u32((uint32_t)(v >> 32)) << 32) | uniform_u32((uint32_t)v);
}

__device__ __forceinline__ bool lists_ok(const KernelArgs &a) {
    return a.static_list && a.lists_done && uniform_u32(*a.lists_done) == a.lists_tag;
}

__device__ __forceinline__ const char *reread_kernargs(const char *kargs) {
    unsigned long long p = uniform_u64((unsigned long long)kargs);
    asm volatile("s_mov_b64 %0, %1" : "=s"(p) : "s"(p));
    return (const char *)reinterpret_cast<const __attribute__((address_space(4))) char *>(p);
}

extern __shared__ double rm_lds[];

__device__ __forceinline__ void stage_scene(const double *__restrict__ scene_blob, const rm_dev_header &H) {
    const double2 *src = reinterpret_cast<const double2 *>(scene_blob);
    double2 *dst = reinterpret_cast<double2 *>(rm_lds);
    const uint32_t n2 = H.total_words / 2;
    for (uint32_t i = threadIdx.x; i < n2; i += blockDim.x) dst[i] = src[i];
    __syncthreads();
}

struct SceneAsked { double2 v[RM_LDS_SCENE_LIMIT_WORDS / 128u]; };
__device__ __forceinline__ SceneAsked stage_scene_ask(const double *__restrict__ scene_blob, const rm_dev_header &H) {
    const double2 *src = reinterpret_cast<const double2 *>(scene_blob);
    const uint32_t n2 = H.total_words / 2, lane = threadIdx.x & 63u;
    SceneAsked p;
#pragma unroll
    for (uint32_t k = 0; k < RM_LDS_SCENE_LIMIT_WORDS / 128u; k++) {
        p.v[k] = double2{0., 0.};
        if (lane + 64u * k < n2) p.v[k] = src[lane + 64u * k];
    }
    return p;
}
__device__ __forceinline__ void stage_scene_put(const SceneAsked &p, const rm_dev_header &H) {
    double2 *dst = reinterpret_cast<double2 *>(rm_lds);
    const uint32_t n2 = H.total_words / 2, lane = threadIdx.x & 63u;
#pragma unroll
    for (uint32_t k = 0; k < RM_LDS_SCENE_LIMIT_WORDS / 128u; k++)
        if (lane + 64u * k < n2) dst[lane + 64u * k] = p.v[k];
    __syncthreads();
}

__device__ __forceinline__ uint32_t tile_of_id(const KernelArgs &a, uint32_t id) {
    const uint32_t last = a.n_tiles - 1u;
    return (a.order_mul == 1u && a.order_add == 0u) ? id
         : (a.order_mul == last && a.order_add == last) ? last - id
         : (uint32_t)(((unsigned long long)id * a.order_mul + a.order_add) % a.n_tiles);
}

__device__ __forceinline__ void tile_origin(const KernelArgs &a, uint32_t tile, uint32_t &tx0, uint32_t &ty0, uint32_t &tyf,
                                            uint32_t &ty8) {
    const uint32_t patch = tile >> 4, sub = tile & 15u;
    const uint32_t pcol = patch % a.n_width, prow = patch / a.n_width;
    tx0 = pcol * 32u + (sub & (32u / TILE_W - 1u)) * TILE_W;
    const uint32_t in_patch = (sub / (32u / TILE_W)) * TILE_H;
    ty0 = (a.patch_row_begin + prow * a.patch_row_stride) * 32u + in_patch;
    const uint32_t packed = prow * 32u + in_patch;
    tyf = a.f64_compact ? packed : ty0;
    ty8 = a.u8_compact ? packed : ty0;
}

}

#ifndef RM_KERNEL_ORIENTED
#define RM_KERNEL_ORIENTED 0
#endif
#if !defined(RM_KERNEL_FAST) || !RM_KERNEL_FAST
#if RM_KERNEL_ORIENTED
#define RM_FLAVOR_NS rmdev_strict_o
#else
#define RM_FLAVOR_NS rmdev_strict
#endif
#define RM_FAST 0
#pragma clang fp contract(off)
#if defined(RM_KERNEL_GROUP) && RM_KERNEL_GROUP == 0 && !defined(RM_CHECKED_NUMERICS_OFF)
#if RM_KERNEL_ORIENTED
#define RM_CHECKED_NS rmdev_strict_o_checked
#else
#define RM_CHECKED_NS rmdev_strict_checked
#endif
#undef RM_FLAVOR_NS
#define RM_FLAVOR_NS RM_CHECKED_NS
#define RM_CHECKED 1
#include "rm_trace.inc"
#include "rm_render_kernel.inc"
#undef RM_CHECKED
#undef RM_FLAVOR_NS
#if RM_KERNEL_ORIENTED
#define RM_FLAVOR_NS rmdev_strict_o
#else
#define RM_FLAVOR_NS rmdev_strict
#endif
#endif
#include "rm_trace.inc"
#include "rm_classify.inc"
#include "rm_render_kernel.inc"
#undef RM_FLAVOR_NS
#undef RM_FAST
#endif

#if !defined(RM_KERNEL_FAST) || RM_KERNEL_FAST
#if RM_KERNEL_ORIENTED
#define RM_FLAVOR_NS rmdev_fast_o
#else
#define RM_FLAVOR_NS rmdev_fast
#endif
#define RM_FAST 1
#pragma clang fp contract(fast)
#include "rm_trace.inc"
#include "rm_classify.inc"
#include "rm_render_kernel.inc"
#undef RM_FLAVOR_NS
#undef RM_FAST
#pragma clang fp contract(off)
#endif

#endif
```

rusty-marcher_amd/csrc/rm_render_kernel.inc:

```
namespace RM_FLAVOR_NS {
using namespace rmdev;

template <int STACK, int POW, bool BVH, bool CULL, bool EDGES, bool PREFETCHED>
__device__ __forceinline__ bool render_tile(const SceneView &sc, const KernelArgs &a, uint32_t tx0, uint32_t ty0,
                                            uint32_t tyf, uint32_t ty8, double bp_x, double bp_y, double *wl,
                                            double *__restrict__ frame_in, unsigned long long *stats, bool have_mask,
                                            unsigned long long first_mask, const char *kargs_of_kernel) {
    const uint32_t lane = threadIdx.x & 63u;
    const V3 bg = mk(own_sgpr(a.bg_x), own_sgpr(a.bg_y), own_sgpr(a.bg_z));
    const uint32_t max_depth = own_sgpr(a.max_depth);
#if RM_CHECKED
    bool sus = false;
#endif

    double *const lds0 = wl + lane;
    uint32_t *const l0_depth = reinterpret_cast<uint32_t *>(wl + RM_WAVE_L0_DEPTH_WORDS);
    double *const sum = wl + RM_WAVE_SUM_WORDS;
    uint32_t *const pair = reinterpret_cast<uint32_t *>(wl + RM_WAVE_PAIR_WORDS);

#if RM_KERNEL_ORIENTED
    const double bx = PREFETCHED ? bp_x : a.bp_x[tx0 + (lane % TILE_W)], by = PREFETCHED ? bp_y : a.bp_y[ty0 + (lane / TILE_W)];
    V3 dir = RM_NORMALIZED(mk((bx * a.cam_rx + by * a.cam_ux) + a.cam_fx, (bx * a.cam_ry + by * a.cam_uy) + a.cam_fy, (bx * a.cam_rz + by * a.cam_uz) + a.cam_fz), true);
#else
    V3 dir = RM_NORMALIZED(PREFETCHED ? mk(bp_x, bp_y, -1.) : mk(a.bp_x[tx0 + (lane % TILE_W)], a.bp_y[ty0 + (lane / TILE_W)], -1.), true);
#endif
    V3 orig = mk(a.cam_x, a.cam_y, a.cam_z);
    double weight = 1.;
    uint32_t depth = 1;
    uint32_t pix = lane;
    bool on = true;
    V3 acc = mk(0., 0., 0.);
    bool handed = false;

    StackEntry deep[STACK > 1 ? STACK - 1 : 1];
    uint32_t n_deep = 0;
    bool l0_full = false;
#ifdef RM_EXP_STAMPS
    uint32_t st_steps = 0, st_rays = 0, st_taken = 0;
#endif
    __builtin_amdgcn_wave_barrier();
#if defined(RM_EXP_STAMPS) && defined(RM_EXP_STARTUP)
    if (dir.x == 12345.678) sc.cnt[2] = 1u;
    sc.cnt[1] |= (((uint32_t)__builtin_amdgcn_s_memrealtime() - sc.cnt[3]) & 0xFFFFu) << 16;
#endif

    constexpr bool DIV = !CULL;
    constexpr bool HANDOVER = CULL;
    const bool dead_children = DIV && own_sgpr(a.dead_children) != 0u;
    uint32_t step = 0;
    for (;; step++) {
        if (step == 1u) __builtin_amdgcn_s_setprio(1);
        else if (step == 2u) __builtin_amdgcn_s_setprio(2);
        else if (step == 3u) __builtin_amdgcn_s_setprio(3);
#ifdef RM_EXP_STAMPS
        st_steps++; st_rays += (uint32_t)__popcll(__ballot(on));
#endif
        bool next = false;
        if (where<DIV>(on)) {
            Hit h;
            const unsigned long long t_ch = RM_PHASE_T();
            const bool got = closest_hit<BVH, CULL, EDGES>(sc, orig, dir, on, h, have_mask & (step == 0u), first_mask) & on;
            RM_PHASE_ADD(sc, 0, t_ch);
            V3 L = bg;
            const double w_add = (on & (got | (depth > 1u))) ? weight : 0.;
            double w_cap = 0.;
            if (DIV && !got && depth > 1u) acc = acc + scaled(bg, weight);
            if (where<DIV>(got)) {
                const Surface s = surface_at<DIV>(sc, orig, dir, h, got RM_SUS_ARG);
                const unsigned long long t_sd = RM_PHASE_T();
                L = pick(got, bg + shade_direct<POW, BVH, CULL, EDGES>(sc, neg(dir), s, got, h.pid RM_SUS_ARG), bg);
                RM_PHASE_ADD(sc, 3, t_sd);
                if (DIV) acc = acc + scaled(L, weight);
                const bool glass = got & (s.mat[8] != 0.);
                if (where<DIV>(glass)) {
                    const double reflection = s.mat[6], ri = s.mat[7], inv_ri = s.mat[9];
                    V3 ro, rd, to, td;
                    double dn_r, dn_t;
                    const bool has_r = glass & reflect_child<DIV>(dir, s, ri, inv_ri, ro, rd, dn_r);
                    const bool has_t = glass & refract_child(dir, s, ri, inv_ri, glass, to, td, dn_t RM_SUS_ARG);
                    const double wr = weight * reflection, wt = weight * (1. - reflection);
                    const bool capped = depth + 1u > max_depth;
                    w_cap = ((capped & has_r) ? wr : 0.) + ((capped & has_t) ? wt : 0.);
                    if (DIV && capped) acc = acc + scaled(bg, w_cap);
                    bool live_r = has_r & !capped, live_t = has_t & !capped;
                    if (DIV && dead_children) {
                        const uint32_t sides = (uint32_t)s.mat[8];
                        const bool dead_t = live_t & (((dn_t > 0.) & ((sides & 2u) != 0u)) | ((dn_t < 0.) & ((sides & 4u) != 0u)));
                        if (dead_t) acc = acc + scaled(bg, wt);
                        live_t = live_t & !dead_t;
                        if (live_r & !live_t) {
                            const bool dead_r = ((dn_r > 0.) & ((sides & 2u) != 0u)) | ((dn_r < 0.) & ((sides & 4u) != 0u));
                            if (dead_r) acc = acc + scaled(bg, wr);
                            live_r = live_r & !dead_r;
                        }
                    }
                    const bool park = live_r & live_t, park_l0 = park & (n_deep == 0u) & !l0_full;
                    if (park_l0) {
                        lds0[0] = ro.x; lds0[64] = ro.y; lds0[128] = ro.z;
                        lds0[192] = rd.x; lds0[256] = rd.y; lds0[320] = rd.z;
                        lds0[384] = wr;
                        l0_depth[lane] = depth + 1u;
                    }
                    if (park & !park_l0) {
                        StackEntry &e = deep[n_deep];
                        e.ox = ro.x; e.oy = ro.y; e.oz = ro.z;
                        e.dx = rd.x; e.dy = rd.y; e.dz = rd.z;
                        e.w = wr; e.depth = depth + 1u;
                    }
                    n_deep += (park & !park_l0) ? 1u : 0u;
                    l0_full = l0_full | park_l0;
                    next = live_r | live_t;
                    orig = pick(live_t, to, ro);
                    dir = pick(live_t, td, rd);
                    weight = live_t ? wt : wr;
                    depth += 1u;
                }
            }
            const V3 term = mk(__builtin_fma(bg.x, w_cap, L.x * w_add), __builtin_fma(bg.y, w_cap, L.y * w_add),
                               __builtin_fma(bg.z, w_cap, L.z * w_add));
            if (DIV) {
            } else if (!HANDOVER || pix == lane) {
                acc = acc + term;
            } else {
                __hip_atomic_fetch_add(&sum[pix * 3 + 0], term.x, __ATOMIC_RELAXED, __HIP_MEMORY_SCOPE_WAVEFRONT);
                __hip_atomic_fetch_add(&sum[pix * 3 + 1], term.y, __ATOMIC_RELAXED, __HIP_MEMORY_SCOPE_WAVEFRONT);
                __hip_atomic_fetch_add(&sum[pix * 3 + 2], term.z, __ATOMIC_RELAXED, __HIP_MEMORY_SCOPE_WAVEFRONT);
            }
            const bool pop_deep = on & !next & (n_deep > 0u);
            if (where<DIV>(pop_deep)) {
                n_deep -= pop_deep ? 1u : 0u;
                const StackEntry &e = deep[pop_deep ? n_deep : 0u];
                orig = pick(pop_deep, mk(e.ox, e.oy, e.oz), orig);
                dir = pick(pop_deep, mk(e.dx, e.dy, e.dz), dir);
                weight = pop_deep ? e.w : weight;
                depth = pop_deep ? e.depth : depth;
            }
            const bool pop_l0 = on & !next & !pop_deep & l0_full;
            if (where<DIV>(pop_l0)) {
                orig = pick(pop_l0, mk(lds0[0], lds0[64], lds0[128]), orig);
                dir = pick(pop_l0, mk(lds0[192], lds0[256], lds0[320]), dir);
                weight = pop_l0 ? lds0[384] : weight;
                depth = pop_l0 ? l0_depth[lane] : depth;
                l0_full = l0_full & !pop_l0;
            }
            next = next | pop_deep | pop_l0;
        }
        on = on & next;

        if (!HANDOVER) {
            if (!on) break;
            continue;
        }
        const unsigned long long idle = __ballot(!on), donors = __ballot(l0_full);
        if (idle == ~0ull) break;
        if (idle != 0ull && donors != 0ull) {
            const uint32_t n_pairs = min((uint32_t)__popcll(idle), (uint32_t)__popcll(donors));
            const uint32_t my_idle = __builtin_amdgcn_mbcnt_hi((uint32_t)(idle >> 32), __builtin_amdgcn_mbcnt_lo((uint32_t)idle, 0u));
            const uint32_t my_donor = __builtin_amdgcn_mbcnt_hi((uint32_t)(donors >> 32), __builtin_amdgcn_mbcnt_lo((uint32_t)donors, 0u));
            const bool give = l0_full & (my_donor < n_pairs), take = !on & (my_idle < n_pairs);
            if (!handed) {
                sum[lane * 3 + 0] = 0.; sum[lane * 3 + 1] = 0.; sum[lane * 3 + 2] = 0.;
                handed = true;
            }
            if (give) pair[my_donor] = lane | (pix << 8);
            __builtin_amdgcn_wave_barrier();
            if (take) {
                const uint32_t from = pair[my_idle];
                const double *src = wl + (from & 63u);
                orig = mk(src[0], src[64], src[128]);
                dir = mk(src[192], src[256], src[320]);
                weight = src[384];
                depth = l0_depth[from & 63u];
                pix = from >> 8;
                on = true;
            }
            l0_full = l0_full & !give;
            __builtin_amdgcn_wave_barrier();
#ifdef RM_EXP_STAMPS
// ... 34 lines not shown
        dst[piece] = sum2[row * PIECES + piece];
    }

    if (frame8) {
        const double vx = acc.x, vy = acc.y, vz = acc.z;
        uint8_t *slab8 = reinterpret_cast<uint8_t *>(wl);
        slab8[lane * 3 + 0] = (uint8_t)(255. * __builtin_fmin(__builtin_fmax(vx, 0.), 1.));
        slab8[lane * 3 + 1] = (uint8_t)(255. * __builtin_fmin(__builtin_fmax(vy, 0.), 1.));
        slab8[lane * 3 + 2] = (uint8_t)(255. * __builtin_fmin(__builtin_fmax(vz, 0.), 1.));
        __builtin_amdgcn_wave_barrier();
        constexpr uint32_t P8 = TILE_W * 3u / 8u;
        if (lane < 24u) {
            const uint32_t row = lane / P8, piece = lane % P8;
            unsigned long long *dst = reinterpret_cast<unsigned long long *>(
                frame8 + ((size_t)(ty8 + row) * frame_width + tx0) * 3u);
            dst[piece] = reinterpret_cast<const unsigned long long *>(wl)[row * P8 + piece];
        }
    }
    __builtin_amdgcn_wave_barrier();
#ifdef RM_EXP_STAMPS
    if (stats) *stats = (unsigned long long)st_steps | ((unsigned long long)st_rays << 16) | ((unsigned long long)st_taken << 40);
#else
    (void)stats;
#endif
    return false;
}
#undef RM_SUS_PARAM
#undef RM_SUS_ARG
#undef RM_NORMALIZED
#undef RM_SQRT_DISCRIMINANT
#if RM_CHECKED
#undef RM_CHECKED_X_MIN
#undef RM_CHECKED_X_MAX
#endif

#if !RM_CHECKED

#ifndef RM_PATCH_COST_OP
#define RM_PATCH_COST_OP atomicMax
#endif

#ifndef RM_ORD_POLLS
#define RM_ORD_POLLS 65536u
#endif
__device__ __forceinline__ uint32_t order_entry(const KernelArgs &a, uint32_t k, bool &sky, bool &last_resort) {
    const uint32_t n_dyn = (a.n_tiles >> 4) - (a.n_static >> 4);
    uint32_t entry = 0u;
    bool gave_up = k >= a.ord_cap || k >= n_dyn;
    last_resort = false;
    if (a.ord_read != a.ord_flat) {
        if (!gave_up) entry = a.ord_read[k];
        last_resort = (entry >> RM_ORD_TAG_SHIFT) != a.ord_read_tag;
    } else {
        for (uint32_t polls = 0u; !gave_up; polls++) {
            entry = uniform_u32(__hip_atomic_load(a.ord_flat + k, __ATOMIC_RELAXED, __HIP_MEMORY_SCOPE_AGENT));
            if ((entry >> RM_ORD_TAG_SHIFT) == a.ord_tag) break;
            if ((polls & 63u) == 63u) {
                uint32_t go = uniform_u32(__hip_atomic_load(a.ord_cnt + RM_ORD_GO, __ATOMIC_RELAXED, __HIP_MEMORY_SCOPE_AGENT));
                if (go == 0u && polls >= RM_ORD_PATIENCE) {
                    uint32_t expected = 0u;
                    if ((threadIdx.x & 63u) == 0u)
                        (void)__hip_atomic_compare_exchange_strong(a.ord_cnt + RM_ORD_GO, &expected, a.ord_tag | RM_ORD_FALLBACK_BIT, __ATOMIC_RELAXED, __ATOMIC_RELAXED, __HIP_MEMORY_SCOPE_AGENT);
                    go = uniform_u32(__hip_atomic_load(a.ord_cnt + RM_ORD_GO, __ATOMIC_RELAXED, __HIP_MEMORY_SCOPE_AGENT));
                }
                if (go == (a.ord_tag | RM_ORD_FALLBACK_BIT)) { last_resort = true; break; }
                if (polls >= RM_ORD_POLLS) { gave_up = true; break; }
            }
            __builtin_amdgcn_s_sleep(8);
        }
    }
    uint32_t patch = entry & (RM_ORD_SKY_BIT - 1u);
    sky = (entry & RM_ORD_SKY_BIT) != 0u;
    if (last_resort && !gave_up) {
        patch = lists_ok(a) ? a.dyn_inv[k] : n_dyn - 1u - k;
        sky = false;
    }
    if (gave_up || patch >= (a.n_tiles >> 4)) {
        if ((threadIdx.x & 63u) == 0u && a.err_word) __hip_atomic_store(a.err_word, ((unsigned long long)a.launch_seq << 32) | 1ull, __ATOMIC_RELAXED, __HIP_MEMORY_SCOPE_SYSTEM);
        return ~0u;
    }
    return patch;
}

template <int STACK, int POW, bool STAGED, bool BVH, bool CULL, bool EDGES>
__device__ __attribute__((noinline)) void render_patch_alone(const char *kargs_of_kernel, uint32_t tile0, uint32_t n = 16u, bool staged = false) {
    const unsigned long long kv = (unsigned long long)kargs_of_kernel;
    const unsigned long long ku = ((unsigned long long)(uint32_t)__builtin_amdgcn_readfirstlane((int)(uint32_t)(kv >> 32)) << 32) |
                                  (uint32_t)__builtin_amdgcn_readfirstlane((int)(uint32_t)kv);
    const char *kargs = (const char *)reinterpret_cast<const __attribute__((address_space(4))) char *>(ku);
    const double *__restrict__ scene_blob = *reinterpret_cast<const double *const *>(kargs);
    const KernelArgs &a = *reinterpret_cast<const KernelArgs *>(kargs + sizeof(const double *));
    double *__restrict__ frame = *reinterpret_cast<double *const *>(kargs + sizeof(const double *) + sizeof(KernelArgs));
    for (uint32_t t = 0; t < n; t++) {
        const uint32_t tile = tile0 + t;
        uint32_t tx0, ty0, tyf, ty8;
        tile_origin(a, tile, tx0, ty0, tyf, ty8);
        unsigned long long first_mask = ~0ull;
        bool have_mask = false;
        if (a.tile_mask && a.mask_tag) {
            const unsigned long long w = uniform_u64(__hip_atomic_load(const_cast<unsigned long long *>(a.tile_mask) + tile, __ATOMIC_RELAXED, __HIP_MEMORY_SCOPE_AGENT));
            if ((uint32_t)(w >> 56) == a.mask_tag) { first_mask = w & 0x00FFFFFFFFFFFFFFull; have_mask = true; }
        }
        if (STAGED && !staged) stage_scene(scene_blob, a.H);
        double *wl = rm_lds + (STAGED ? a.H.total_words : 0u);
        const unsigned long long t0 = __builtin_amdgcn_s_memrealtime();
        SceneView sc;
        if (STAGED) sc.S = rm_lds; else sc.S = scene_blob;
        sc.G = scene_blob;
        sc.cull_bounds = scene_blob + a.H.off_bounds;
        sc.cull_planar = scene_blob + a.H.off_planar;
        sc.bstack = reinterpret_cast<uint32_t *>(wl + RM_WAVE_BVH_STACK_WORDS);
        sc.cull_cos = a.cull_cos;
        sc.H = a.H;
#ifdef RM_EXP_STAMPS
        uint32_t cull_counts[4] = {0u, 0u, 0u, 0u};
        sc.cnt = cull_counts;
#endif
        (void)render_tile<STACK, POW, BVH, CULL, EDGES, false>(sc, a, tx0, ty0, tyf, ty8, 0., 0., wl, frame, nullptr, have_mask & (a.mask_exact != 0u), first_mask, kargs_of_kernel);
        if (a.patch_cost && (threadIdx.x & 63u) == 0u) {
            const unsigned long long dt = __builtin_amdgcn_s_memrealtime() - t0;
            RM_PATCH_COST_OP(a.patch_cost + (tile >> 4), dt < 0x00FFFFFFull ? (uint32_t)dt : 0x00FFFFFFu);
        }
        __builtin_amdgcn_wave_barrier();
    }
}

template <int STACK, int POW, bool STAGED, bool BVH, bool CULL, bool EDGES>
__device__ __attribute__((noinline)) void sky_tail_patch(const char *kargs_of_kernel, uint32_t t) {
    const unsigned long long kv = (unsigned long long)kargs_of_kernel;
    const unsigned long long ku = ((unsigned long long)(uint32_t)__builtin_amdgcn_readfirstlane((int)(uint32_t)(kv >> 32)) << 32) |
                                  (uint32_t)__builtin_amdgcn_readfirstlane((int)(uint32_t)kv);
    const char *kargs = (const char *)reinterpret_cast<const __attribute__((address_space(4))) char *>(ku);
    const KernelArgs &a = *reinterpret_cast<const KernelArgs *>(kargs + sizeof(const double *));
    double *__restrict__ frame = *reinterpret_cast<double *const *>(kargs + sizeof(const double *) + sizeof(KernelArgs));
    const uint32_t n_dyn = (a.n_tiles >> 4) - (a.n_static >> 4);
    bool sky, last_resort;
    const uint32_t patch = order_entry(a, n_dyn - a.tail_patches + t, sky, last_resort);
    if (patch == ~0u) return;
    const uint32_t tile0 = patch * 16u, lane = threadIdx.x & 63u;
    if (last_resort && a.tile_mask && a.mask_tag) {
        unsigned long long *word = const_cast<unsigned long long *>(a.tile_mask) + tile0 + (lane & 15u);
        for (uint32_t polls = 0u; polls < 64u; polls++) {
            const unsigned long long w = __hip_atomic_load(word, __ATOMIC_RELAXED, __HIP_MEMORY_SCOPE_AGENT);
            if (__all((uint32_t)(w >> 56) == a.mask_tag)) { sky = !__any((w & 0x00FFFFFFFFFFFFFFull) != 0ull); break; }
            __builtin_amdgcn_s_sleep(8);
        }
    }
    if (!sky) {
        if (t < a.ov_cap && !last_resort) return;
        render_patch_alone<STACK, POW, STAGED, BVH, CULL, EDGES>(kargs, tile0);
        return;
    }
    constexpr uint32_t PIECES = TILE_W * 3u / 2u, P8 = TILE_W * 3u / 8u;
    for (uint32_t i = 0; i < 16u; i++) {
        uint32_t tx0, ty0, tyf, ty8;
        tile_origin(a, tile0 + i, tx0, ty0, tyf, ty8);
        for (uint32_t q = lane; q < 96u; q += 64u) {
            double2 *dst = reinterpret_cast<double2 *>(frame + ((size_t)(tyf + q / PIECES) * a.frame_width + tx0) * 3u);
            dst[q % PIECES] = double2{0., 0.};
        }
        if (a.frame8 && lane < 24u) {
            unsigned long long *dst = reinterpret_cast<unsigned long long *>(a.frame8 + ((size_t)(ty8 + lane / P8) * a.frame_width + tx0) * 3u);
            dst[lane % P8] = 0ull;
        }
    }
}

#ifndef RM_ORDERED_TILE_INLINE
#define RM_ORDERED_TILE_INLINE __forceinline__
#endif
template <int STACK, int POW, bool STAGED, bool BVH, bool CULL, bool EDGES>
__device__ RM_ORDERED_TILE_INLINE uint32_t ordered_tile(const char *kargs_of_kernel, uint32_t id_v) {
    const unsigned long long kv = (unsigned long long)kargs_of_kernel;
    const unsigned long long ku = ((unsigned long long)(uint32_t)__builtin_amdgcn_readfirstlane((int)(uint32_t)(kv >> 32)) << 32) |
                                  (uint32_t)__builtin_amdgcn_readfirstlane((int)(uint32_t)kv);
    const char *kargs = (const char *)reinterpret_cast<const __attribute__((address_space(4))) char *>(ku);
    const KernelArgs &a = *reinterpret_cast<const KernelArgs *>(kargs + sizeof(const double *));
    const uint32_t id = (uint32_t)__builtin_amdgcn_readfirstlane((int)id_v);
    const uint32_t n_dyn = (a.n_tiles >> 4) - (a.n_static >> 4), behind = 16u * (n_dyn - a.tail_patches);
    uint32_t m = id - a.n_static, k, sub;
    bool handed = false;
    if (m >= behind + a.tail_patches) {
        m -= behind + a.tail_patches;
        if (m >= 16u * a.ov_cap) {
            order_places(a, m - 16u * a.ov_cap, nullptr, false, true);
            return ~0u;
        }
        k = n_dyn - a.tail_patches + (m >> 4);
        sub = m & 15u;
        handed = true;
    } else {
        if (a.tail_patches) {
            const uint32_t before = a.tail_q == 1u ? (m >= behind ? m - behind : 0u) : a.tail_q ? __umulhi(m, a.tail_q) : min(m, a.tail_patches);
            const bool mine = a.tail_q == 1u ? m >= behind : a.tail_q ? __umulhi(m + 1u, a.tail_q) > before : m < a.tail_patches;
            if (mine) {
                sky_tail_patch<STACK, POW, STAGED, BVH, CULL, EDGES>(kargs_of_kernel, before);
                return ~0u;
            }
            m -= before;
        }
        k = m >> 4;
        sub = 15u - (m & 15u);
    }
    bool sky, last_resort;
    const uint32_t patch = order_entry(a, k, sky, last_resort);
    if (patch == ~0u || (handed && (sky || last_resort))) return ~0u;
    return patch * 16u + sub;
}

#ifndef RM_CLASSIFY_WG_INLINE
#define RM_CLASSIFY_WG_INLINE __forceinline__
#endif
template <bool ORDER, bool STAGED>
__device__ RM_CLASSIFY_WG_INLINE unsigned long long classify_workgroup(const char *kargs_of_kernel, uint32_t id_v, unsigned long long t_start) {
    const unsigned long long kv = (unsigned long long)kargs_of_kernel;
    const unsigned long long ku = ((unsigned long long)(uint32_t)__builtin_amdgcn_readfirstlane((int)(uint32_t)(kv >> 32)) << 32) |
                                  (uint32_t)__builtin_amdgcn_readfirstlane((int)(uint32_t)kv);
    const char *kargs = (const char *)reinterpret_cast<const __attribute__((address_space(4))) char *>(ku);
    const double *__restrict__ scene_blob = *reinterpret_cast<const double *const *>(kargs);
    const KernelArgs &a = *reinterpret_cast<const KernelArgs *>(kargs + sizeof(const double *));
    const uint32_t id = (uint32_t)__builtin_amdgcn_readfirstlane((int)id_v);
    unsigned long long stats = 0ull;
    (void)t_start;
    const uint32_t n_patches = a.n_tiles >> 4;
    const bool bottom_up = a.order_mul == a.n_tiles - 1u && a.order_add == a.n_tiles - 1u && a.n_tiles > 1u;
    const bool ordering = ORDER && a.ord_cnt;
    if (ordering && a.ord_read == a.ord_flat) __builtin_amdgcn_s_setprio(3);
    const uint32_t iters = ordering ? a.cls_iters : 1u;
    auto patch_of = [&](uint32_t it, bool &valid) {
        const uint32_t q = (it * a.cls_blocks + id) * 4u + ((threadIdx.x & 63u) >> 4);
        valid = q < n_patches;
        return !valid ? 0u : bottom_up ? n_patches - 1u - q : q;
    };
    bool valid;
    uint32_t patch = patch_of(0u, valid);
    ClsAsked cls_asked = classify_ask(a, patch, valid);
    OrdAsked ord_asked{0u, 0u, 0u};
    if (ordering) ord_asked = order_ask(a, patch, valid);
    uint32_t ct_sum = 0u, ct_num = 0u;
    if (ordering && a.key_mode == RM_KEY_CONTENT) { ct_sum = a.ctab[threadIdx.x & 63u]; ct_num = a.ctab[64u + (threadIdx.x & 63u)]; }
#ifndef RM_CLASSIFY_FROM_MEMORY
    ClsView blob;
    OrdRec *rec;
    if (STAGED) {
        stage_scene(scene_blob, a.H);
        blob = cls_view_of_blob(rm_lds, a.H);
        rec = reinterpret_cast<OrdRec *>(rm_lds + a.H.total_words);
    } else if (a.cls_lds_words) {
        blob = cls_stage(scene_blob, a.H, rm_lds);
        rec = reinterpret_cast<OrdRec *>(rm_lds + a.cls_lds_words);
    } else {
        blob = cls_view_of_blob(scene_blob, a.H);
        rec = reinterpret_cast<OrdRec *>(rm_lds);
    }
#else
    const ClsView blob = cls_view_of_blob(scene_blob, a.H);
    OrdRec *rec = reinterpret_cast<OrdRec *>(rm_lds);
#endif
    const uint32_t prim_cost = !(ordering && a.key_mode == RM_KEY_CONTENT) ? 0u : ct_num ? (ct_sum / ct_num) << 6 : ~0u;
    if (ordering && id == 0u) {
        if (a.ord_cnt_next) for (uint32_t i = threadIdx.x & 63u; i < RM_ORD_CNT_WORDS; i += 64u) a.ord_cnt_next[i] = 0u;
        if (a.ctab_zero) for (uint32_t i = threadIdx.x & 63u; i < RM_CTAB_WORDS; i += 64u) a.ctab_zero[i] = 0u;
    }
    for (uint32_t it = 0; it < iters; it++) {
        bool valid_next = false;
        uint32_t patch_next = 0u;
        ClsAsked cls_next = cls_asked;
        OrdAsked ord_next = ord_asked;
        if (it + 1u < iters) {
            patch_next = patch_of(it + 1u, valid_next);
            cls_next = classify_ask(a, patch_next, valid_next);
            ord_next = order_ask(a, patch_next, valid_next);
        }
        unsigned long long sig, own;
        (void)classify_patches<true>(blob, a, patch, valid, cls_asked, const_cast<unsigned long long *>(a.tile_mask), a.cls_prims, a.mask_tag, sig, own);
#ifdef RM_EXP_STAMPS
        if (it + 1u == iters) stats = (__builtin_amdgcn_s_memrealtime() - t_start) & 0xFFFFFull;
#endif
        if (ordering) order_slot(a, id, patch, valid, sig, a.mask_exact ? own : ~0ull, prim_cost, ord_asked, rec + it * 4u, a.ord_rec ? a.ord_rec + (size_t)(it * a.cls_blocks + id) * 12u : nullptr);
        patch = patch_next; valid = valid_next; cls_asked = cls_next; ord_asked = ord_next;
    }
    if (ordering) {
        __builtin_amdgcn_wave_barrier();
#ifdef RM_EXP_STAMPS
        stats |= ((__builtin_amdgcn_s_memrealtime() - t_start) & 0xFFFFFull) << 20;
#endif
        order_places(a, id, rec, true, a.ord_rec == nullptr);
    }
    return stats;
}

template <int STACK, int POW, int WAVES, int TPW, bool STAGED = true, bool BVH = false, bool CULL = false, bool EDGES = false, bool ORDER = false, bool FEEDBACK = false>
__global__ __launch_bounds__(WAVES * 64) __attribute__((amdgpu_waves_per_eu(POW == POW_INTEGER ? (EDGES ? RM_EDGES_WAVES : RM_MIN_WAVES) : 1, 8))) void rm_render_static(const double *__restrict__ scene_blob, KernelArgs a,
                                                              double *__restrict__ frame) {
    static_assert(WAVES == 1 && TPW == 1, "one tile per wave, one wave per workgroup");
#ifdef RM_EXP_STAMPS
    const unsigned long long t_start = __builtin_amdgcn_s_memrealtime();
    unsigned long long tile_stats = 0;
    uint32_t cull_counts[4] = {0u, 0u, 0u, 0u};
    uint32_t st_tile = ~0u;
    unsigned long long st_mask = ~0ull;
    auto stamp = [&]() {
        if ((threadIdx.x & 63u) == 0 && a.debug_stamps) {
            unsigned long long *o = a.debug_stamps + 4ull * blockIdx.x;
            o[0] = t_start; o[1] = tile_stats; o[2] = __builtin_amdgcn_s_memrealtime();
            unsigned long long *x = a.debug_stamps + 4ull * gridDim.x + 2ull * blockIdx.x;
#if defined(RM_EXP_WALKSTATS) || defined(RM_EXP_PHASES) || defined(RM_EXP_STARTUP)
            o[3] = (unsigned long long)cull_counts[0] | ((unsigned long long)cull_counts[1] << 32);
            x[0] = st_tile; x[1] = (unsigned long long)cull_counts[2] | ((unsigned long long)cull_counts[3] << 32);
#else
            o[3] = (unsigned long long)cull_counts[0] | ((unsigned long long)cull_counts[1] << 16) |
                   ((unsigned long long)cull_counts[2] << 40) | ((unsigned long long)cull_counts[3] << 52);
            x[0] = st_tile; x[1] = st_mask;
#endif
        }
    };
#else
    auto stamp = []() {};
#endif
    const bool feedback = FEEDBACK && a.fb_flag != nullptr;
    if (feedback && blockIdx.x == 0u) {
        const uint32_t b = threadIdx.x;
        a.fb_zero[b] = 0u;
        if (b == 0u) a.fb_zero[RM_FB_BUCKETS] = 0u;
        if (a.fb_target != 0u) {
            uint32_t above = a.fb_hist[b] * RM_FB_SAMPLE;
            for (uint32_t off = 1u; off < 64u; off <<= 1) {
                const uint32_t o = (uint32_t)__shfl_down((int)above, off, 64);
                above += (b + off < 64u) ? o : 0u;
            }
            const unsigned long long fits = __ballot(above <= a.fb_target);
            const uint32_t first = (uint32_t)__builtin_ctzll(fits | (1ull << 63));
            const uint32_t total = (uint32_t)__shfl((int)above, 0, 64);
            if (b == 0u) *a.fb_threshold = total == 0u ? a.fb_long_ticks : max(fb_edge(first), 200u);
        }
    }

    uint32_t id = blockIdx.x;
    if (a.cls_blocks) {
        if (id < a.cls_blocks) {
#ifdef RM_EXP_STAMPS
            tile_stats = classify_workgroup<ORDER, STAGED>((const char *)__builtin_amdgcn_kernarg_segment_ptr(), id, t_start);
#else
            (void)classify_workgroup<ORDER, STAGED>((const char *)__builtin_amdgcn_kernarg_segment_ptr(), id, 0ull);
#endif
            stamp();
            return;
        }
        id -= a.cls_blocks;
    }
#ifdef RM_EARLY_LOADS
    constexpr bool EARLY = ORDER;
#else
    constexpr bool EARLY = false;
#endif
    SceneAsked scene_asked;
    if (STAGED && EARLY) scene_asked = stage_scene_ask(scene_blob, a.H);
    uint32_t tile = 0u;
    bool late = id >= a.first_round;
    bool listed_tile = false;
    if (ORDER && a.ord_cnt && id >= a.n_static) {
        tile = uniform_u32(ordered_tile<STACK, POW, STAGED, BVH, CULL, EDGES>((const char *)__builtin_amdgcn_kernarg_segment_ptr(), id));
        if (tile == ~0u) { stamp(); return; }
        late = true;
    } else if (feedback && id < a.fb_cap) {
        if (id >= min(a.fb_count[0], a.fb_cap)) { stamp(); return; }
        tile = a.fb_list[id];
        if (tile >= a.n_tiles) { stamp(); return; }
        listed_tile = true;
    } else {
        if (feedback) id -= a.fb_cap;
        if (id >= a.n_tiles) { stamp(); return; }
        if (ORDER && a.ord_cnt && a.static_list && a.lists_done) {
            const uint32_t done = *a.lists_done, cand = a.static_list[id >> 4];
            tile = done == a.lists_tag ? cand * 16u + (15u - (id & 15u)) : tile_of_id(a, id);
        } else {
            tile = tile_of_id(a, id);
        }
    }
#if defined(RM_EXP_STAMPS) && defined(RM_EXP_STARTUP)
    cull_counts[3] = (uint32_t)t_start;
    cull_counts[0] = ((uint32_t)__builtin_amdgcn_s_memrealtime() - cull_counts[3]) & 0xFFFFu;
#endif
    const uint32_t flagged = (feedback && !listed_tile) ? a.fb_flag[tile] : 0u;
    uint32_t tx0, ty0, tyf, ty8;
    tile_origin(a, tile, tx0, ty0, tyf, ty8);
    double bp_x = 0., bp_y = 0.;
    if (FEEDBACK || EARLY) { bp_x = a.bp_x[tx0 + ((threadIdx.x & 63u) % TILE_W)]; bp_y = a.bp_y[ty0 + ((threadIdx.x & 63u) / TILE_W)]; }
    uint32_t fb_thr = a.fb_long_ticks;
    if (feedback && a.fb_target != 0u) {
        fb_thr = __hip_atomic_load(a.fb_threshold, __ATOMIC_RELAXED, __HIP_MEMORY_SCOPE_AGENT);
        fb_thr = fb_thr ? fb_thr : a.fb_long_ticks;
    }
    if (flagged) { stamp(); return; }

    bool have_mask = a.tile_mask != nullptr && a.mask_exact != 0u;
    unsigned long long first_mask = ~0ull;
    if (a.tile_mask && a.mask_tag) {
        have_mask = false;
        if (late || a.mask_tag_prev) {
            unsigned long long *word = const_cast<unsigned long long *>(a.tile_mask) + tile;
            const unsigned long long t0 = __builtin_amdgcn_s_memrealtime();
            if (a.mask_tag_prev) {
                const unsigned long long w = a.tile_mask[tile];
                if ((uint32_t)(w >> 56) == a.mask_tag || (uint32_t)(w >> 56) == a.mask_tag_prev) { first_mask = w & 0x00FFFFFFFFFFFFFFull; have_mask = true; }
            }
            while (!have_mask) {
                const unsigned long long w = uniform_u64(__hip_atomic_load(word, __ATOMIC_RELAXED, __HIP_MEMORY_SCOPE_AGENT));
                if ((uint32_t)(w >> 56) == a.mask_tag || (a.mask_tag_prev && (uint32_t)(w >> 56) == a.mask_tag_prev)) { first_mask = w & 0x00FFFFFFFFFFFFFFull; have_mask = true; break; }
                if (__builtin_amdgcn_s_memrealtime() - t0 > 2000ull) break;
                __builtin_amdgcn_s_sleep(4);
            }
        }
    } else if (a.tile_mask) {
        first_mask = uniform_u64(a.tile_mask[tile]);
    }
    if (a.tile_mask) {
        if (first_mask == 0ull && !listed_tile) {
            const uint32_t lane = threadIdx.x & 63u;
            constexpr uint32_t PIECES = TILE_W * 3u / 2u, P8 = TILE_W * 3u / 8u;
            for (uint32_t q = lane; q < 96u; q += 64u) {
                double2 *dst = reinterpret_cast<double2 *>(frame + ((size_t)(tyf + q / PIECES) * a.frame_width + tx0) * 3u);
                dst[q % PIECES] = double2{0., 0.};
            }
            if (a.frame8 && lane < 24u) {
                unsigned long long *dst = reinterpret_cast<unsigned long long *>(a.frame8 + ((size_t)(ty8 + lane / P8) * a.frame_width + tx0) * 3u);
                dst[lane % P8] = 0ull;
            }
            if (feedback && (threadIdx.x & 63u) == 0u) a.fb_next_flag[tile] = 0;
            stamp();
            return;
        }
    }

#ifdef RM_EXP_STAMPS
    st_tile = tile; st_mask = have_mask ? first_mask : ~0ull;
#endif
    have_mask = have_mask & (a.mask_exact != 0u);
#if defined(RM_EXP_STAMPS) && defined(RM_EXP_STARTUP)
    cull_counts[0] |= (((uint32_t)__builtin_amdgcn_s_memrealtime() - cull_counts[3]) & 0xFFFFu) << 16;
#endif
    if (STAGED) { if (EARLY) stage_scene_put(scene_asked, a.H); else stage_scene(scene_blob, a.H); }
#if defined(RM_EXP_STAMPS) && defined(RM_EXP_STARTUP)
    cull_counts[1] = ((uint32_t)__builtin_amdgcn_s_memrealtime() - cull_counts[3]) & 0xFFFFu;
#endif
    const uint32_t cull_words = (!STAGED && CULL) ? a.cull_lds_words : 0u;
    if (!STAGED && CULL && cull_words) { cull_stage(scene_blob, a.H, rm_lds); __syncthreads(); }
    double *wl = rm_lds + (STAGED ? a.H.total_words : cull_words);
    if (ORDER && (threadIdx.x & 63u) == 0u) reinterpret_cast<uint32_t *>(wl + RM_WAVE_T0_WORDS)[0] = (uint32_t)__builtin_amdgcn_s_memrealtime();
#ifdef RM_CHECKED_NS
    constexpr bool CHECKED = STAGED && !BVH && !CULL;
    namespace tile_ns = RM_CHECKED_NS;
#else
    constexpr bool CHECKED = false;
    namespace tile_ns = RM_FLAVOR_NS;
#endif
    const unsigned long long fb_t0 = feedback ? __builtin_amdgcn_s_memrealtime() : 0ull;
    bool exact = CHECKED && a.exact_only != 0u;
    if (!exact) {
        tile_ns::SceneView sc;
        if (STAGED) sc.S = rm_lds; else sc.S = scene_blob;
        sc.G = scene_blob;
        sc.cull_bounds = cull_words ? rm_lds : scene_blob + a.H.off_bounds;
        sc.cull_planar = cull_words ? rm_lds + 4u * (a.H.n_spheres + a.H.n_polygons + a.H.n_triangles) : scene_blob + a.H.off_planar;
        sc.bstack = reinterpret_cast<uint32_t *>(wl + RM_WAVE_BVH_STACK_WORDS);
        sc.cull_cos = own_sgpr(a.cull_cos);
#ifdef RM_EXP_STAMPS
        sc.cnt = cull_counts;
#endif
        sc.H.n_spheres = own_sgpr(a.H.n_spheres);         sc.H.n_polygons = own_sgpr(a.H.n_polygons);
        sc.H.n_triangles = own_sgpr(a.H.n_triangles);     sc.H.n_lights = own_sgpr(a.H.n_lights);
        sc.H.off_spheres = own_sgpr(a.H.off_spheres);     sc.H.off_polygons = own_sgpr(a.H.off_polygons);
        sc.H.off_pverts = own_sgpr(a.H.off_pverts);       sc.H.off_triangles = own_sgpr(a.H.off_triangles);
        sc.H.off_materials = own_sgpr(a.H.off_materials); sc.H.off_lights = own_sgpr(a.H.off_lights);
        sc.H.off_keys = own_sgpr(a.H.off_keys);           sc.H.total_words = a.H.total_words;
        sc.H.list_ordered = own_sgpr(a.H.list_ordered);   sc.H.off_bvh_spheres = own_sgpr(a.H.off_bvh_spheres);
        sc.H.off_bvh_triangles = own_sgpr(a.H.off_bvh_triangles); sc.H.off_bounds = own_sgpr(a.H.off_bounds);
        sc.H.off_planar = own_sgpr(a.H.off_planar);       sc.H.off_groups = own_sgpr(a.H.off_groups);
        sc.H.off_occ = own_sgpr(a.H.off_occ);
        sc.H.shadow_rho = own_sgpr(a.H.shadow_rho);

#if defined(RM_EXP_STAMPS) && defined(RM_EXP_PHASES)
        cull_counts[2] = (uint32_t)(__builtin_amdgcn_s_memrealtime() - t_start);
#endif
#ifdef RM_EXP_STAMPS
        exact = tile_ns::render_tile<STACK, POW, BVH, CULL, EDGES, FEEDBACK || EARLY>(sc, a, tx0, ty0, tyf, ty8, bp_x, bp_y, wl, frame, &tile_stats, have_mask, first_mask, (const char *)__builtin_amdgcn_kernarg_segment_ptr());
#else
        exact = tile_ns::render_tile<STACK, POW, BVH, CULL, EDGES, FEEDBACK || EARLY>(sc, a, tx0, ty0, tyf, ty8, bp_x, bp_y, wl, frame, nullptr, have_mask, first_mask, (const char *)__builtin_amdgcn_kernarg_segment_ptr());
#endif
        if (CHECKED && exact) {
            const KernelArgs &b = *reinterpret_cast<const KernelArgs *>(reread_kernargs((const char *)__builtin_amdgcn_kernarg_segment_ptr()) + sizeof(const double *));
            if (b.redo_count && (threadIdx.x & 63u) == 0u) atomicAdd(b.redo_count, 1u);
        }
    }
    if constexpr (CHECKED) if (exact) render_patch_alone<STACK, POW, STAGED, BVH, CULL, EDGES>((const char *)__builtin_amdgcn_kernarg_segment_ptr(), tile, 1u, true);
    if (ORDER) {
#ifdef RM_NO_REREAD
        const KernelArgs &b = a;
#else
        const KernelArgs &b = *reinterpret_cast<const KernelArgs *>(reread_kernargs((const char *)__builtin_amdgcn_kernarg_segment_ptr()) + sizeof(const double *));
#endif
        if (b.patch_cost) {
            const uint32_t dt = min(uniform_u32((uint32_t)__builtin_amdgcn_s_memrealtime() - reinterpret_cast<const uint32_t *>(wl + RM_WAVE_T0_WORDS)[0]), 0x00FFFFFFu);
            if ((threadIdx.x & 63u) == 0u) RM_PATCH_COST_OP(b.patch_cost + (tile >> 4), dt);
            if ((tile & 15u) == 0u && b.ctab_cur && b.tile_mask && b.mask_tag && b.mask_exact) {
                const unsigned long long w = uniform_u64(__hip_atomic_load(const_cast<unsigned long long *>(b.tile_mask) + tile, __ATOMIC_RELAXED, __HIP_MEMORY_SCOPE_AGENT));
                if ((uint32_t)(w >> 56) == b.mask_tag && ((w >> (threadIdx.x & 63u)) & 1ull) && (threadIdx.x & 63u) < 56u) {
                    atomicAdd(b.ctab_cur + (threadIdx.x & 63u), dt >> 6);
                    atomicAdd(b.ctab_cur + 64u + (threadIdx.x & 63u), 1u);
                }
            }
        }
    }
#ifdef RM_EXP_STAMPS
    if (a.tile_mask) st_mask = __hip_atomic_load(const_cast<unsigned long long *>(a.tile_mask) + tile, __ATOMIC_RELAXED, __HIP_MEMORY_SCOPE_AGENT) & 0x00FFFFFFFFFFFFFFull;
#endif
    if (feedback) {
        const unsigned long long fb_dt = __builtin_amdgcn_s_memrealtime() - fb_t0;
        const uint32_t ticks = fb_dt < 0x7FFFFFFFull ? (uint32_t)fb_dt : 0x7FFFFFFFu;
        const bool is_long = ticks >= fb_thr;
        if ((threadIdx.x & 63u) == 0u) {
            if (a.fb_target != 0u && tile % RM_FB_SAMPLE == 0u) atomicAdd(a.fb_next_hist + fb_bucket(ticks), 1u);
            bool listed = false;
            if (is_long) {
                const uint32_t slot = atomicAdd(a.fb_next_count, 1u);
                if (slot < a.fb_cap) { a.fb_next_list[slot] = tile; listed = true; }
            }
            a.fb_next_flag[tile] = listed ? 1 : 0;
        }
    }
    stamp();
}

#endif

}
```

rusty-marcher_amd/csrc/rm_trace.inc:

```
namespace RM_FLAVOR_NS {
using namespace rmdev;


struct V3 { double x, y, z; };

__device__ __forceinline__ V3 mk(double x, double y, double z) { return V3{x, y, z}; }
__device__ __forceinline__ V3 operator+(V3 a, V3 b) { return mk(a.x + b.x, a.y + b.y, a.z + b.z); }
__device__ __forceinline__ V3 operator-(V3 a, V3 b) { return mk(a.x - b.x, a.y - b.y, a.z - b.z); }
__device__ __forceinline__ V3 operator*(V3 a, V3 b) { return mk(a.x * b.x, a.y * b.y, a.z * b.z); }
__device__ __forceinline__ V3 neg(V3 a) { return mk(-a.x, -a.y, -a.z); }
__device__ __forceinline__ V3 scaled(V3 a, double s) { return mk(a.x * s, a.y * s, a.z * s); }
__device__ __forceinline__ V3 pick(bool c, V3 a, V3 b) { return mk(c ? a.x : b.x, c ? a.y : b.y, c ? a.z : b.z); }
__device__ __forceinline__ double dot(V3 a, V3 b) { return a.x * b.x + a.y * b.y + a.z * b.z; }
#ifndef RM_CHECKED
#define RM_CHECKED 0
#endif
#if RM_CHECKED
#define RM_SUS_PARAM , bool &sus
#define RM_SUS_ARG , sus
#else
#define RM_SUS_PARAM
#define RM_SUS_ARG
#endif
#if RM_CHECKED
// ... 869 lines not shown
    const uint32_t ns = sc.H.n_spheres, np = sc.H.n_polygons;
    const uint32_t pid = got ? h.pid : 0u;
    const bool is_s = got & (pid < ns);
    const bool is_p = got & !is_s & (pid < ns + np);
    const bool is_t = got & !is_s & !is_p;
    s.normal = mk(0., 0., 0.);
    if (where<DIV>(is_s)) {
        const double *sp = sc.S + sc.H.off_spheres + RM_SPHERE_WORDS * (is_s ? pid : 0u);
        const V3 centre = spheres.centre(sp, is_s ? pid : 0u);
        s.normal = RM_NORMALIZED(mk(s.point.x - centre.x, s.point.y - centre.y, s.point.z - centre.z), is_s);
    }
    if (where<DIV>(is_p | is_t)) {
        const uint32_t word = is_p ? sc.H.off_polygons + RM_POLYGON_WORDS * (pid - ns)
                            : is_t ? sc.H.off_triangles + RM_TRIANGLE_WORDS * (pid - ns - np)
                                   : 0u;
        const double *rec = sc.S + word;
        s.normal = pick(is_s, s.normal, mk(rec[0], rec[1], rec[2]));
    }
    s.mat = sc.S + sc.H.off_materials + RM_MATERIAL_WORDS * pid;
    return s;
}

__device__ __forceinline__ V3 reflect(V3 incident, V3 normal) {
    return incident - scaled(normal, 2. * dot(incident, normal));
}

template <int POW>
__device__ __forceinline__ double specular_pow(double x, double y) {
    if (POW == POW_GENERIC) return pow(x, y);
    uint32_t n = (uint32_t)y;
    double r = 1., b = x;
    const uint32_t n0 = __builtin_amdgcn_readfirstlane(n);
    if (__all(n == n0)) {
        for (uint32_t m = n0; m != 0u; m >>= 1) {
            if (m & 1u) r = r * b;
            if (m > 1u) b = b * b;
        }
        return r;
    }
    while (__any(n != 0u)) {
        if (n & 1u) r = r * b;
        b = b * b;
        n >>= 1;
    }
    return r;
}

__device__ __forceinline__ double dot_fused(V3 a, V3 b) {
    return __builtin_fma(a.z, b.z, __builtin_fma(a.y, b.y, a.x * b.x));
}

struct LightAt {
    V3 dir;
    V3 from;
    V3 pos;
    double ldn, sf;
    bool dark;
};

struct StoredLights {
    __device__ __forceinline__ V3 operator()(const double *lt, uint32_t) const { return mk(lt[0], lt[1], lt[2]); }
};

template <class LIGHTS = StoredLights>
__device__ __forceinline__ LightAt light_at(const SceneView &sc, uint32_t l, const Surface &s, V3 dir_to_viewer, double exponent, bool got RM_SUS_PARAM,
                                            const LIGHTS &lights = LIGHTS()) {
    (void)got;
    LightAt a;
    const double *lt = sc.G + sc.H.off_lights + RM_LIGHT_WORDS * l;
    a.pos = lights(lt, l);
    a.dir = RM_NORMALIZED(a.pos - s.point, got);
    a.ldn = dot(a.dir, s.normal);
    a.from = s.point + scaled(s.normal, (a.ldn < 0.) ? -1e-3 : 1e-3);
    const double k2 = -2. * dot_fused(a.dir, s.normal);
    const V3 reflected = mk(__builtin_fma(-k2, s.normal.x, -a.dir.x), __builtin_fma(-k2, s.normal.y, -a.dir.y),
                            __builtin_fma(-k2, s.normal.z, -a.dir.z));
    a.sf = __builtin_fmax(dot_fused(reflected, dir_to_viewer), 0.);
    a.dark = !(a.ldn > 0.) & !(a.sf > 0.) & (exponent > 0.);
    return a;
}

template <int POW, bool BVH, bool CULL, bool EDGES, class LIGHTS = StoredLights, class SPHERES = StoredSpheres>
__device__ __forceinline__ V3 shade_direct(const SceneView &sc, V3 neg_dir, const Surface &s, bool got, uint32_t pid RM_SUS_PARAM,
                                           const LIGHTS &lights = LIGHTS(), const SPHERES &spheres = SPHERES()) {
    const double *m = s.mat;
    const double exponent = m[5];
    const V3 dir_to_viewer = neg_dir;
    V3 li = mk(0., 0., 0.);
    auto add_light = [&](uint32_t l, const LightAt &a, bool lit) {
        if (lit) {
            const double *lt = sc.G + sc.H.off_lights + RM_LIGHT_WORDS * l;
            const V3 lcol = mk(lt[3], lt[4], lt[5]);
            const double intensity = lt[6];
            const V3 diffuse_color = mk(m[1], m[2], m[3]);
            const double specular_k = m[4];
            const double diffusion = __builtin_fmax(a.ldn, 0.);
            const double di = diffusion * intensity;
            const double spec = specular_pow<POW>(a.sf * specular_k, exponent);
            li = mk(__builtin_fma(lcol.x, spec, __builtin_fma(lcol.x * diffuse_color.x, di, li.x)),
                    __builtin_fma(lcol.y, spec, __builtin_fma(lcol.y * diffuse_color.y, di, li.y)),
                    __builtin_fma(lcol.z, spec, __builtin_fma(lcol.z * diffuse_color.z, di, li.z)));
        }
    };
    const bool masks = !BVH && !CULL && !SPHERES::moves && sc.H.off_occ != 0u;
    for (uint32_t l = 0; l < sc.H.n_lights;) {
        const LightAt a = light_at(sc, l, s, dir_to_viewer, exponent, got RM_SUS_ARG, lights);
        const bool dec_a = !got | a.dark;
        if (!BVH && !CULL && l + 1u < sc.H.n_lights) {
            const LightAt b = light_at(sc, l + 1u, s, dir_to_viewer, exponent, got RM_SUS_ARG, lights);
            const bool dec_b = !got | b.dark;
            if (__all(dec_a | dec_b | ((a.ldn < 0.) == (b.ldn < 0.)))) {
                bool occ_a, occ_b;
                const unsigned long long t_sh = RM_PHASE_T();
                const V3 from = pick(dec_a, b.from, a.from);
                unsigned long long m_a = 0ull, m_b = 0ull;
                if (masks) shadow_masks2(sc, got, pid, l, m_a, m_b);
                const uint32_t n = sc.H.n_spheres + sc.H.n_polygons + sc.H.n_triangles;
                if (masks && (m_a & m_b) != ((n >= 64u) ? ~0ull : (1ull << n) - 1ull))
                    any_hit2_masked(sc, from, a.dir, b.dir, dec_a, dec_b, occ_a, occ_b, m_a, m_b);
                else
                    any_hit2(sc, from, a.dir, b.dir, dec_a, dec_b, occ_a, occ_b, spheres);
                RM_PHASE_ADD(sc, 1, t_sh);
                add_light(l, a, !occ_a);
                add_light(l + 1u, b, !occ_b);
                l += 2u;
                continue;
            }
        }
        const unsigned long long t_sh = RM_PHASE_T();
        const bool lit = !any_hit<BVH, CULL, EDGES>(sc, a.from, a.dir, dec_a, a.pos, sc.H.shadow_rho, spheres);
        RM_PHASE_ADD(sc, 1, t_sh);
        add_light(l, a, lit);
        l += 1u;
    }
    return scaled(li, m[0]);
}

template <bool LAZY>
__device__ __forceinline__ bool reflect_child(V3 incident, const Surface &s, double ri, double inv_ri, V3 &o, V3 &d, double &dn) {
    const double c = dot(s.normal, incident);
    const double r = (c < 0.) ? ri : inv_ri;
    const double cos_theta_2 = 1. - r * r * (1. - c * c);
    const bool has = !(cos_theta_2 > 0.);
    dn = 0.;
    if (!LAZY || has) {
        d = reflect(incident, s.normal);
        dn = dot(d, s.normal);
        o = s.point + scaled(s.normal, (dn < 0.) ? -1e-4 : 1e-4);
    }
    return has;
}
template <bool LAZY>
__device__ __forceinline__ bool reflect_child(V3 incident, const Surface &s, double ri, double inv_ri, V3 &o, V3 &d) {
    double dn;
    return reflect_child<LAZY>(incident, s, ri, inv_ri, o, d, dn);
}

__device__ __forceinline__ bool refract_child(V3 incident, const Surface &s, double ri, double inv_ri, bool glass, V3 &o, V3 &d, double &dn RM_SUS_PARAM) {
    (void)glass;
    const double c0 = -dot(s.normal, incident);
    const bool flip = c0 < 0.;
    const double r = flip ? ri : inv_ri;
    const double c = flip ? -c0 : c0;
    const double cos_theta_2 = 1. - r * r * (1. - c * c);
    const double k = r * c - __builtin_sqrt(cos_theta_2);
    d = RM_NORMALIZED(scaled(incident, r) + scaled(s.normal, flip ? -k : k), glass & !(cos_theta_2 < 0.));
    dn = dot(d, s.normal);
    const bool along = flip ? (dn < 0.) : (dn > 0.);
    o = s.point + scaled(s.normal, (along != flip) ? 1e-4 : -1e-4);
    return !(cos_theta_2 < 0.);
}
__device__ __forceinline__ bool refract_child(V3 incident, const Surface &s, double ri, double inv_ri, bool glass, V3 &o, V3 &d RM_SUS_PARAM) {
    double dn;
    return refract_child(incident, s, ri, inv_ri, glass, o, d, dn RM_SUS_ARG);
}

}
```

Before: 32550.

## Add per-tile light and reflection cone bundles to cull shadow and bounce candidates

During in-launch classification, a tile whose primary rays all hit a single planar primitive gets extra cone bundles. Each bundle runs from a light (or the camera's mirror point) to the tile's hit footprint, and the primitives that can intersect it are stored as 14-bit fields in the tile mask word. The render kernel uses these masks to restrict shadow any-hit tests (and possibly reflection rays) to candidate primitives, cutting per-pixel intersection work. The cost is an extra classification pass per tile, a new kernel variant, and a mask layout change that disables mask reuse across layouts. It only applies to small, non-BVH scenes with at most 14 primitives and 2 lights.

```diff
diff --git a/rusty-marcher_amd/csrc/rm_classify.inc b/rusty-marcher_amd/csrc/rm_classify.inc
--- a/rusty-marcher_amd/csrc/rm_classify.inc
+++ b/rusty-marcher_amd/csrc/rm_classify.inc
@@ -60,7 +60,7 @@
     return ClsView{bounds, planar, poly, tri, 6u, 6u};
 }
 
-template <bool EDGES>
+template <bool EDGES, bool PRIMARY = true>
 __device__ __forceinline__ bool keeps(const ClsView &v, const KernelArgs &a, const Bundle &b, uint32_t pid, bool in) {
     const uint32_t ns = a.H.n_spheres, np = a.H.n_polygons;
     const double2 *bp = reinterpret_cast<const double2 *>(v.bounds) + 2u * (in ? pid : 0u);
@@ -70,6 +70,7 @@
     if (EDGES && __any(planar)) {
         const double2 *pp = reinterpret_cast<const double2 *>(v.planar) + 8u * (planar ? pid - ns : 0u);
         out = out | cull_edges(pp, b, sph, planar & !out);
+        if (!PRIMARY) return in & !out;
         const double *recw = !planar ? v.bounds : pid < ns + np ? v.poly + v.poly_stride * (pid - ns) : v.tri + v.tri_stride * (pid - ns - np);
         const double2 *rec = reinterpret_cast<const double2 *>(recw);
         const double2 r0 = rec[0], r1 = rec[1], r2 = rec[2];
@@ -125,6 +126,84 @@
     return ClsAsked{a.bp_x[px0], a.bp_x[px0 + 31u], a.bp_y[py0], a.bp_y[py0 + 31u],
                     a.bp_x[tx0], a.bp_x[tx0 + TILE_W - 1u], a.bp_y[ty0], a.bp_y[ty0 + TILE_H - 1u]};
 }
+__device__ __forceinline__ bool cone_to_ball(Bundle &b, V3 apex, V3 F, double rho_f, double rho, bool two_sided) {
+    const V3 v = F - apex;
+    const double dd = dot(v, v);
+    const V3 u = unit(v);
+    const double s2 = (rho_f * rho_f) / dd;
+    const double cm = __builtin_sqrt(__builtin_fmax(1. - s2, 0.)) * (1. - 1e-9) - 1e-9;
+    b.ax = apex.x; b.ay = apex.y; b.az = apex.z;
+    b.ux = u.x; b.uy = u.y; b.uz = u.z;
+    b.cos2 = cm * cm;
+    b.sin_t = (double)__builtin_sqrtf((float)__builtin_fmax((1. - cm) * (1. + cm), 0.)) * (1. + 1e-6) + 1e-7;
+    b.chord = (double)__builtin_sqrtf((float)__builtin_fmax(2. * (1. - cm), 0.)) * (1. + 1e-6) + 1e-7;
+    b.rho = rho;
+    b.two_sided = two_sided;
+    b.narrow = true;
+    return (s2 <= 0.5) & (cm > 0.7) & (dd < 1e300);
+}
+template <bool EDGES>
+__device__ __forceinline__ unsigned long long tile_bundles(const ClsView &v, const KernelArgs &a, const double *__restrict__ lights, const ClsAsked &asked,
+                                                           unsigned long long mask, uint32_t n) {
+    const uint32_t ns = a.H.n_spheres, np = a.H.n_polygons;
+    const uint32_t q = mask ? (uint32_t)__builtin_ctzll(mask) : 0u;
+    bool ok = (mask != 0ull) & ((mask & (mask - 1ull)) == 0ull) & (q >= ns) & (q < n);
+    if (!__any(ok)) return 0ull;
+    const double *recw = !ok ? v.bounds : q < ns + np ? v.poly + v.poly_stride * (q - ns) : v.tri + v.tri_stride * (q - ns - np);
+    const double2 *rec = reinterpret_cast<const double2 *>(recw);
+    const double2 r0 = rec[0], r1 = rec[1], r2 = rec[2];
+    const V3 nrm = mk(r0.x, r0.y, r1.x), cam = mk(a.cam_x, a.cam_y, a.cam_z);
+    ok = ok & (__builtin_fabs(dot(nrm, nrm) - 1.) <= 1e-12);
+    const double num = (r1.y - cam.x) * nrm.x + (r2.x - cam.y) * nrm.y + (r2.y - cam.z) * nrm.z;
+    V3 hit[4];
+    double t2 = 0.;
+#pragma unroll
+    for (uint32_t k = 0; k < 4u; k++) {
+        const V3 d = cls_dir(a, (k & 1u) ? asked.tx1 : asked.tx0, (k & 2u) ? asked.ty1 : asked.ty0);
+        const double den = dot(d, nrm), len2 = dot(d, d);
+        ok = ok & (((num > 0.) & (den > 0.)) | ((num < 0.) & (den < 0.))) & (den * den >= 1e-6 * len2);
+        const double t = num / den;
+        hit[k] = cam + scaled(d, t);
+        t2 = __builtin_fmax(t2, (t * t) * len2);
+    }
+    const V3 F = scaled((hit[0] + hit[1]) + (hit[2] + hit[3]), 0.25);
+    double rr = 0.;
+#pragma unroll
+    for (uint32_t k = 0; k < 4u; k++) rr = __builtin_fmax(rr, dot(hit[k] - F, hit[k] - F));
+    const double slack = 1e-6 * (1. + __builtin_sqrt(t2) + (__builtin_fabs(cam.x) + __builtin_fabs(cam.y) + __builtin_fabs(cam.z)));
+    const double rho_f = __builtin_sqrt(rr) * (1. + 1e-6) + slack, rho = a.H.shadow_rho + slack;
+    ok = ok & (rho_f < 1e300) & (rho < 1e300);
+    const V3 mirror = cam + scaled(nrm, 2. * num);
+    unsigned long long fields = 0ull;
+#pragma unroll 1
+    for (uint32_t k = 0; k < 3u; k++) {
+        if (k < 2u && a.H.n_lights < 2u) continue;
+        const double *lt = lights + RM_LIGHT_WORDS * (k < 2u ? k : 0u);
+        const V3 apex = k < 2u ? mk(lt[0], lt[1], lt[2]) : mirror;
+        Bundle b;
+        ok = ok & cone_to_ball(b, apex, F, rho_f, rho, k < 2u);
+        unsigned long long m = 0ull;
+        for (uint32_t pid = 0; pid < n; pid++) {
+            const bool in = ok & (pid != q);
+            m |= keeps<EDGES, false>(v, a, b, pid, in) ? (1ull << pid) : 0ull;
+        }
+        fields |= m << (RM_TB_BITS * k);
+    }
+    const unsigned long long qbit = 1ull << q;
+    fields |= qbit | (qbit << RM_TB_BITS) | (qbit << (2u * RM_TB_BITS));
+    return ok ? fields : 0ull;
+}
+template <bool EDGES>
+__device__ __forceinline__ void add_tile_bundles(const ClsView &v, const KernelArgs &a, const double *__restrict__ lights, uint32_t patch, bool valid,
+                                                 unsigned long long *__restrict__ tile_mask) {
+    const ClsAsked asked = classify_ask(a, patch, valid);
+    unsigned long long *word = tile_mask + (valid ? patch : 0u) * 16u + (threadIdx.x & 15u);
+    const unsigned long long w = valid ? __hip_atomic_load(word, __ATOMIC_RELAXED, __HIP_MEMORY_SCOPE_AGENT) : 0ull;
+    const unsigned long long mask = (uint32_t)(w >> 56) == a.mask_tag ? w & RM_TB_FIELD : 0ull;
+    const unsigned long long fields = tile_bundles<EDGES>(v, a, lights, asked, mask, a.cls_prims) << RM_TB_BITS;
+    if (valid && fields != 0ull) __hip_atomic_store(word, w | fields, __ATOMIC_RELAXED, __HIP_MEMORY_SCOPE_AGENT);
+}
+
 template <bool EDGES>
 __device__ __forceinline__ bool classify_patches(const ClsView &scene_blob, const KernelArgs &a, uint32_t patch, bool valid, const ClsAsked &asked,
                                                  unsigned long long *__restrict__ tile_mask, uint32_t n, uint32_t tag, unsigned long long &sig, unsigned long long &own) {
diff --git a/rusty-marcher_amd/csrc/rm_device.hip b/rusty-marcher_amd/csrc/rm_device.hip
--- a/rusty-marcher_amd/csrc/rm_device.hip
+++ b/rusty-marcher_amd/csrc/rm_device.hip
@@ -239,7 +239,10 @@
 RM_DECLARE_GROUP(0) RM_DECLARE_GROUP(1) RM_DECLARE_GROUP(2) RM_DECLARE_GROUP(3) RM_DECLARE_GROUP(4)
 #undef RM_DECLARE_GROUP
 
+const void *rm_pick_kernel_strict_tb(int stack, int pow_mode);
+const void *rm_pick_kernel_fast_tb(int stack, int pow_mode);
 const void *rm_pick_kernel(bool fast, bool staged, bool bvh, bool cull, bool edges, int order, bool feedback, int stack, int pow_mode) {
+    if (order == 2) return (staged && !bvh && !cull && !feedback) ? (fast ? rm_pick_kernel_fast_tb(stack, pow_mode) : rm_pick_kernel_strict_tb(stack, pow_mode)) : nullptr;
     const int group = staged ? (cull ? 1 : 0) : !bvh ? 2 : feedback ? 4 : 3;
     if (staged && (bvh || feedback)) return nullptr;
     if (!staged && !cull) return nullptr;
@@ -907,6 +910,7 @@
             uint64_t bits = 0;
             for (unsigned long long v : m) {
                 if (t.s.tagged) v &= 0x00FFFFFFFFFFFFFFull;
+                if (t.s.tagged && t.s.tagged_bundles) v &= RM_TB_FIELD;
                 listed += v != 0ull;
                 for (int b = 0; b < 64 && v != ~0ull; b++)
                     if (v >> b & 1ull) { hist[b]++; bits++; }
@@ -921,6 +925,19 @@
         }
     if (tiles) *tiles = n;
     if (tiles_listed) *tiles_listed = listed;
+    return RM_OK;
+}
+
+extern "C" rm_status rmi_tile_words(rm_ctx *ctx, unsigned long long *out, uint32_t cap, uint32_t *info) {
+    if (!ctx || !info) return ctx_fail(ctx, RM_ERR_INVALID_ARG, "rmi_tile_words: NULL argument");
+    RM_HIP(ctx, hipSetDevice(ctx->device));
+    RM_HIP(ctx, hipDeviceSynchronize());
+    info[0] = info[1] = info[2] = info[3] = 0u;
+    for (const rm_tile_lists &t : ctx->tile_lists)
+        if (t.stream == ctx->last_launch_stream && t.block && ctx->last_launch_classified && ctx->last_launch_tiles <= t.cap) {
+            info[0] = ctx->last_launch_tiles; info[1] = t.s.tagged ? 1u : 0u; info[2] = t.s.tagged_bundles ? 1u : 0u; info[3] = t.s.tag;
+            if (out && info[0] <= cap) RM_HIP(ctx, hipMemcpy(out, t.mask(), (size_t)info[0] * 8u, hipMemcpyDeviceToHost));
+        }
     return RM_OK;
 }
 
diff --git a/rusty-marcher_amd/csrc/rm_kernel_args.hpp b/rusty-marcher_amd/csrc/rm_kernel_args.hpp
--- a/rusty-marcher_amd/csrc/rm_kernel_args.hpp
+++ b/rusty-marcher_amd/csrc/rm_kernel_args.hpp
@@ -118,7 +118,10 @@
     uint32_t exact_only;
     uint32_t dead_children;
     uint32_t *redo_count;
+    uint32_t tile_bundles;
 };
+#define RM_TB_BITS 14u
+#define RM_TB_FIELD 0x3FFFull
 
 struct ClassifyArgs {
     unsigned long long *tile_mask;
diff --git a/rusty-marcher_amd/csrc/rm_kernels.hip b/rusty-marcher_amd/csrc/rm_kernels.hip
--- a/rusty-marcher_amd/csrc/rm_kernels.hip
+++ b/rusty-marcher_amd/csrc/rm_kernels.hip
@@ -60,6 +60,19 @@
 #endif
 }
 
+#if RM_KERNEL_GROUP == 0 && !RM_KERNEL_ORIENTED
+#if RM_KERNEL_FAST
+const void *rm_pick_kernel_fast_tb(int stack, int pow_mode) {
+#else
+const void *rm_pick_kernel_strict_tb(int stack, int pow_mode) {
+#endif
+#define RM_ROW(S) if (stack == S) return pow_mode == POW_INTEGER ? (const void *)flavour::rm_render_static_tb<S, POW_INTEGER> : (const void *)flavour::rm_render_static_tb<S, POW_GENERIC>;
+    RM_ROW(4) RM_ROW(8) RM_ROW(16) RM_ROW(32)
+#undef RM_ROW
+    return nullptr;
+}
+#endif
+
 const void *RM_PICK_NAME(bool edges, int order, int stack, int pow_mode) {
 #if RM_KERNEL_GROUP == 0
     return pick_eo<true, false, false, false>(false, order, stack, pow_mode);
diff --git a/rusty-marcher_amd/csrc/rm_plan.cpp b/rusty-marcher_amd/csrc/rm_plan.cpp
--- a/rusty-marcher_amd/csrc/rm_plan.cpp
+++ b/rusty-marcher_amd/csrc/rm_plan.cpp
@@ -44,6 +44,7 @@
     {"RM_FORCE_UNSTAGED", &rm_knobs::force_unstaged, IS_1},
     {"RM_SHADOW_MASKS", &rm_knobs::shadow_masks, NOT_0},
     {"RM_DEAD_CHILDREN", &rm_knobs::dead_children, NOT_0},
+    {"RM_TILE_BUNDLES", &rm_knobs::tile_bundles, NOT_0},
     {"RM_DISABLE_BVH", &rm_knobs::disable_bvh, IS_1},
     {"RM_FORCE_STACK", &rm_knobs::force_stack, ATOI},
     {"RM_FEEDBACK", &rm_knobs::feedback_mode, ONE_OR_ZERO},
@@ -274,16 +275,19 @@
     rm_stream_state s = before;
     uint32_t mask_tag_before = 0u;
     uint32_t cls_words_wanted = 0u;
+    bool bundles_fit = false;
     P.classify = kn.classify_mode != 0 && !kn.debug_empty && per_wg == 1u && n_prims > 0u &&
                  k.classify_cost <= RM_CLASSIFY_MAX_COST && (kn.classify_mode == 1 || a.n_tiles >= kn.classify_min_tiles);
     if (P.classify) {
         const bool in_launch = kn.classify_in_launch && (n_prims <= kn.classify_in_launch_prims || k.order_in_big_scene) && !k.feedback;
         if (in_launch) {
+            bundles_fit = kn.tile_bundles && !k.bvh && !k.cull && !sc.oriented && n_prims <= RM_TB_BITS && H.n_lights <= 2u;
             if (!s.tagged || s.tagged_tiles != a.n_tiles || s.tagged_scene != sc.scene_epoch || s.tag >= 255u) {
                 P.clear_masks = true;
                 s.tag = 0;
                 s.tagged = true; s.tagged_tiles = a.n_tiles; s.tagged_scene = sc.scene_epoch;
             }
+            s.tagged_bundles = false;
             a.mask_tag = ++s.tag;
             mask_tag_before = a.mask_tag > 1u ? a.mask_tag - 1u : 0u;
             a.cls_blocks = (a.n_tiles / 16u + 3u) / 4u;
@@ -335,6 +339,13 @@
             std::memcpy(s.view, view, sizeof view);
             s.view_seq0 = seq;
         }
+        if (bundles_fit && seq > s.view_seq0) {
+            if (const void *fn = rm_pick_kernel(k.fast, k.staged, k.bvh, k.cull, k.edges, 2, k.feedback, k.stack, k.pow_mode)) {
+                P.k.fn = fn;
+                a.tile_bundles = 2u;
+                s.tagged_bundles = true;
+            }
+        }
         const bool timed = n_patches <= (k.order_in_big_scene ? kn.patch_order_max_deep : kn.patch_order_max);
         const uint32_t groups4 = (n_patches + 3u) / 4u;
         a.cls_iters = (groups4 + cls_max - 1u) / cls_max;
@@ -345,7 +356,8 @@
         a.ord_read_tag = reuse ? s.last_tag : a.ord_tag;
         s.last_tag = a.ord_tag;
         const bool late_places = reuse && kn.order_late_places;
-        a.mask_tag_prev = reuse && kn.mask_reuse ? mask_tag_before : 0u;
+        const bool same_layout = before.tagged && before.tagged_bundles == (a.tile_bundles != 0u);
+        a.mask_tag_prev = reuse && kn.mask_reuse && same_layout ? mask_tag_before : 0u;
         P.frozen = kn.order_freeze > 0 && reuse && f >= 4u && before.frozen_run < (uint32_t)kn.order_freeze && a.mask_tag > 1u &&
                    a.mask_tag_prev != 0u && late_places && kn.test_stall_order == 0 && kn.sky_tail_force < 0 && !kn.debug_tail;
         const bool lays_out = !P.frozen;
@@ -520,6 +532,39 @@
     return RM_OK;
 }
 
+extern "C" rm_status rmi_plan_tile_bundles(uint32_t n_spheres, uint32_t n_polygons, uint32_t n_triangles, uint32_t n_lights, uint32_t total_words,
+                                           uint32_t oriented_from, uint32_t width, uint32_t height, uint32_t *out) {
+    if (!out) { rm_set_host_error("rmi_plan_tile_bundles: NULL argument"); return RM_ERR_INVALID_ARG; }
+    const rm_knobs kn = rm_knobs_from_env();
+    rm_dev_header H{};
+    H.n_spheres = n_spheres; H.n_polygons = n_polygons; H.n_triangles = n_triangles; H.n_lights = n_lights; H.total_words = total_words;
+    const rm_camera_basis basis{rm_vec3{1., 0., 0.}, rm_vec3{0., 1., 0.}, rm_vec3{0., 0., -1.}};
+    rm_params p{};
+    p.half_fov = 0.75; p.height = (double)height; p.width = (double)width; p.ratio = (double)width / (double)height;
+    p.frame_width = width; p.frame_height = height; p.max_depth = 5;
+    rm_band band;
+    rm_stream_state s;
+    uint32_t order_cap = 0u;
+    out[3] = out[4] = 0u;
+    for (uint32_t i = 0; i < 6u; i++) {
+        const rm_plan_scene sc{&H, 1u, 0., true, oriented_from != 0u && i >= oriented_from, rm_vec3{0., 0., 0.}, &basis, 256u};
+        rm_launch_plan P;
+        if (!rm_band_of(p, &band) || !plan_launch(kn, sc, p, band, s, order_cap, rm_feedback_state{}, 0ull, &P)) {
+            rm_set_host_error("rmi_plan_tile_bundles: no plan");
+            return RM_ERR_INVALID_ARG;
+        }
+        if (i == 0u) out[1] = P.args.mask_tag != 0u ? 1u : 0u;
+        if (i == 1u) out[0] = P.args.tile_bundles != 0u ? 1u : 0u;
+        if (P.args.tile_bundles != 0u && P.k.fn == rm_pick_kernel(P.k.fast, P.k.staged, P.k.bvh, P.k.cull, P.k.edges, P.k.order ? 1 : 0, P.k.feedback, P.k.stack, P.k.pow_mode)) out[4] |= 1u << 31;
+        out[2] = P.args.tile_bundles != 0u ? 1u : 0u;
+        out[4] |= (P.args.tile_bundles == 2u && P.args.cls_blocks != 0u) ? 1u << i : 0u;
+        out[3] |= P.args.mask_tag_prev != 0u ? 1u << i : 0u;
+        if (P.classify) s = P.after;
+        if (P.ordered) order_cap = P.order_cap;
+    }
+    return RM_OK;
+}
+
 extern "C" rm_status rmi_plan_exact_only(const rm_vec3 *camera, const rm_camera_basis *basis, uint32_t oriented, uint32_t scene_exact_only, uint32_t *out) {
     if (!camera || !basis || !out) { rm_set_host_error("rmi_plan_exact_only: NULL argument"); return RM_ERR_INVALID_ARG; }
     const rm_knobs kn = rm_knobs_from_env();
diff --git a/rusty-marcher_amd/csrc/rm_plan.hpp b/rusty-marcher_amd/csrc/rm_plan.hpp
--- a/rusty-marcher_amd/csrc/rm_plan.hpp
+++ b/rusty-marcher_amd/csrc/rm_plan.hpp
@@ -23,6 +23,7 @@
     bool force_unstaged = false;
     bool shadow_masks = true;
     bool dead_children = true;
+    bool tile_bundles = true;
     int force_stack = 0;
     bool debug_empty = false;
     int feedback_mode = -1;
@@ -124,6 +125,7 @@
     uint32_t tag = 0, tagged_tiles = 0;
     uint64_t tagged_scene = 0;
     bool tagged = false;
+    bool tagged_bundles = false;
     uint32_t frozen_run = 0;
 };
 
diff --git a/rusty-marcher_amd/csrc/rm_render_kernel.hpp b/rusty-marcher_amd/csrc/rm_render_kernel.hpp
--- a/rusty-marcher_amd/csrc/rm_render_kernel.hpp
+++ b/rusty-marcher_amd/csrc/rm_render_kernel.hpp
@@ -88,6 +88,10 @@
 #ifndef RM_KERNEL_ORIENTED
 #define RM_KERNEL_ORIENTED 0
 #endif
+namespace rmdev {
+template <bool BVH, bool CULL>
+constexpr bool tb_kernel = !BVH && !CULL && !RM_KERNEL_ORIENTED;
+}
 #if !defined(RM_KERNEL_FAST) || !RM_KERNEL_FAST
 #if RM_KERNEL_ORIENTED
 #define RM_FLAVOR_NS rmdev_strict_o
diff --git a/rusty-marcher_amd/csrc/rm_render_kernel.inc b/rusty-marcher_amd/csrc/rm_render_kernel.inc
--- a/rusty-marcher_amd/csrc/rm_render_kernel.inc
+++ b/rusty-marcher_amd/csrc/rm_render_kernel.inc
@@ -1,11 +1,11 @@
 namespace RM_FLAVOR_NS {
 using namespace rmdev;
 
-template <int STACK, int POW, bool BVH, bool CULL, bool EDGES, bool PREFETCHED>
+template <int STACK, int POW, bool BVH, bool CULL, bool EDGES, bool PREFETCHED, bool TBV = false>
 __device__ __forceinline__ bool render_tile(const SceneView &sc, const KernelArgs &a, uint32_t tx0, uint32_t ty0,
                                             uint32_t tyf, uint32_t ty8, double bp_x, double bp_y, double *wl,
                                             double *__restrict__ frame_in, unsigned long long *stats, bool have_mask,
-                                            unsigned long long first_mask, const char *kargs_of_kernel) {
+                                            unsigned long long first_mask, const char *kargs_of_kernel, unsigned long long tb_word = 0ull) {
     const uint32_t lane = threadIdx.x & 63u;
     const V3 bg = mk(own_sgpr(a.bg_x), own_sgpr(a.bg_y), own_sgpr(a.bg_z));
     const uint32_t max_depth = own_sgpr(a.max_depth);
@@ -47,6 +47,12 @@
     constexpr bool DIV = !CULL;
     constexpr bool HANDOVER = CULL;
     const bool dead_children = DIV && own_sgpr(a.dead_children) != 0u;
+    constexpr bool TB = tb_kernel<BVH, CULL> && TBV;
+    static_assert(!TB || (!HANDOVER && !BVH), "the fields' LDS words are the hand-over's and the hierarchy's");
+    static_assert(RM_WAVE_T0_WORDS - RM_WAVE_PAIR_WORDS >= 1u && RM_WAVE_SUM_WORDS - RM_WAVE_BVH_STACK_WORDS >= 32u, "a word, and 64 flags");
+    unsigned long long *const tb_slot = reinterpret_cast<unsigned long long *>(pair);
+    uint32_t *const refl_flag = reinterpret_cast<uint32_t *>(wl + RM_WAVE_BVH_STACK_WORDS);
+    if (TB) { tb_slot[0] = tb_word; refl_flag[lane] = 0u; }
     uint32_t step = 0;
     for (;; step++) {
         if (step == 1u) __builtin_amdgcn_s_setprio(1);
@@ -59,7 +65,16 @@
         if (where<DIV>(on)) {
             Hit h;
             const unsigned long long t_ch = RM_PHASE_T();
-            const bool got = closest_hit<BVH, CULL, EDGES>(sc, orig, dir, on, h, have_mask & (step == 0u), first_mask) & on;
+            bool walk_masked = have_mask & (step == 0u);
+            unsigned long long walk_mask = first_mask;
+            if (TB && step == 1u) {
+                const unsigned long long w = uniform_u64(tb_slot[0]);
+                if (w != 0ull && !__any(on & (refl_flag[lane] == 0u))) {
+                    walk_masked = true;
+                    walk_mask = (w >> (2u * RM_TB_BITS)) & RM_TB_FIELD;
+                }
+            }
+            const bool got = closest_hit<BVH, CULL, EDGES>(sc, orig, dir, on, h, walk_masked, walk_mask) & on;
             RM_PHASE_ADD(sc, 0, t_ch);
             V3 L = bg;
             const double w_add = (on & (got | (depth > 1u))) ? weight : 0.;
@@ -68,7 +83,12 @@
             if (where<DIV>(got)) {
                 const Surface s = surface_at<DIV>(sc, orig, dir, h, got RM_SUS_ARG);
                 const unsigned long long t_sd = RM_PHASE_T();
-                L = pick(got, bg + shade_direct<POW, BVH, CULL, EDGES>(sc, neg(dir), s, got, h.pid RM_SUS_ARG), bg);
+                if constexpr (TB) {
+                    const unsigned long long w = step == 0u ? uniform_u64(tb_slot[0]) : 0ull;
+                    L = pick(got, bg + shade_direct<POW, BVH, CULL, EDGES>(sc, neg(dir), s, got, h.pid RM_SUS_ARG, StoredLights(), StoredSpheres(),
+                                                                           w != 0ull, w & RM_TB_FIELD, (w >> RM_TB_BITS) & RM_TB_FIELD), bg);
+                } else
+                    L = pick(got, bg + shade_direct<POW, BVH, CULL, EDGES>(sc, neg(dir), s, got, h.pid RM_SUS_ARG), bg);
                 RM_PHASE_ADD(sc, 3, t_sd);
                 if (DIV) acc = acc + scaled(L, weight);
                 const bool glass = got & (s.mat[8] != 0.);
@@ -94,6 +114,7 @@
                             live_r = live_r & !dead_r;
                         }
                     }
+                    if (TB && step == 0u) refl_flag[lane] = (live_r & !live_t) ? 1u : 0u;
                     const bool park = live_r & live_t, park_l0 = park & (n_deep == 0u) & !l0_full;
                     if (park_l0) {
                         lds0[0] = ro.x; lds0[64] = ro.y; lds0[128] = ro.z;
@@ -294,7 +315,7 @@
     return patch;
 }
 
-template <int STACK, int POW, bool STAGED, bool BVH, bool CULL, bool EDGES>
+template <int STACK, int POW, bool STAGED, bool BVH, bool CULL, bool EDGES, bool TBK = false>
 __device__ __attribute__((noinline)) void render_patch_alone(const char *kargs_of_kernel, uint32_t tile0, uint32_t n = 16u, bool staged = false) {
     const unsigned long long kv = (unsigned long long)kargs_of_kernel;
     const unsigned long long ku = ((unsigned long long)(uint32_t)__builtin_amdgcn_readfirstlane((int)(uint32_t)(kv >> 32)) << 32) |
@@ -312,6 +333,7 @@
         if (a.tile_mask && a.mask_tag) {
             const unsigned long long w = uniform_u64(__hip_atomic_load(const_cast<unsigned long long *>(a.tile_mask) + tile, __ATOMIC_RELAXED, __HIP_MEMORY_SCOPE_AGENT));
             if ((uint32_t)(w >> 56) == a.mask_tag) { first_mask = w & 0x00FFFFFFFFFFFFFFull; have_mask = true; }
+            if (TBK && a.tile_bundles) first_mask &= RM_TB_FIELD;
         }
         if (STAGED && !staged) stage_scene(scene_blob, a.H);
         double *wl = rm_lds + (STAGED ? a.H.total_words : 0u);
@@ -337,7 +359,7 @@
     }
 }
 
-template <int STACK, int POW, bool STAGED, bool BVH, bool CULL, bool EDGES>
+template <int STACK, int POW, bool STAGED, bool BVH, bool CULL, bool EDGES, bool TBK = false>
 __device__ __attribute__((noinline)) void sky_tail_patch(const char *kargs_of_kernel, uint32_t t) {
     const unsigned long long kv = (unsigned long long)kargs_of_kernel;
     const unsigned long long ku = ((unsigned long long)(uint32_t)__builtin_amdgcn_readfirstlane((int)(uint32_t)(kv >> 32)) << 32) |
@@ -354,13 +376,13 @@
         unsigned long long *word = const_cast<unsigned long long *>(a.tile_mask) + tile0 + (lane & 15u);
         for (uint32_t polls = 0u; polls < 64u; polls++) {
             const unsigned long long w = __hip_atomic_load(word, __ATOMIC_RELAXED, __HIP_MEMORY_SCOPE_AGENT);
-            if (__all((uint32_t)(w >> 56) == a.mask_tag)) { sky = !__any((w & 0x00FFFFFFFFFFFFFFull) != 0ull); break; }
+            if (__all((uint32_t)(w >> 56) == a.mask_tag)) { sky = !__any((w & ((TBK && a.tile_bundles) ? RM_TB_FIELD : 0x00FFFFFFFFFFFFFFull)) != 0ull); break; }
             __builtin_amdgcn_s_sleep(8);
         }
     }
     if (!sky) {
         if (t < a.ov_cap && !last_resort) return;
-        render_patch_alone<STACK, POW, STAGED, BVH, CULL, EDGES>(kargs, tile0);
+        render_patch_alone<STACK, POW, STAGED, BVH, CULL, EDGES, TBK>(kargs, tile0);
         return;
     }
     constexpr uint32_t PIECES = TILE_W * 3u / 2u, P8 = TILE_W * 3u / 8u;
@@ -381,7 +403,7 @@
 #ifndef RM_ORDERED_TILE_INLINE
 #define RM_ORDERED_TILE_INLINE __forceinline__
 #endif
-template <int STACK, int POW, bool STAGED, bool BVH, bool CULL, bool EDGES>
+template <int STACK, int POW, bool STAGED, bool BVH, bool CULL, bool EDGES, bool TBK = false>
 __device__ RM_ORDERED_TILE_INLINE uint32_t ordered_tile(const char *kargs_of_kernel, uint32_t id_v) {
     const unsigned long long kv = (unsigned long long)kargs_of_kernel;
     const unsigned long long ku = ((unsigned long long)(uint32_t)__builtin_amdgcn_readfirstlane((int)(uint32_t)(kv >> 32)) << 32) |
@@ -406,7 +428,7 @@
             const uint32_t before = a.tail_q == 1u ? (m >= behind ? m - behind : 0u) : a.tail_q ? __umulhi(m, a.tail_q) : min(m, a.tail_patches);
             const bool mine = a.tail_q == 1u ? m >= behind : a.tail_q ? __umulhi(m + 1u, a.tail_q) > before : m < a.tail_patches;
             if (mine) {
-                sky_tail_patch<STACK, POW, STAGED, BVH, CULL, EDGES>(kargs_of_kernel, before);
+                sky_tail_patch<STACK, POW, STAGED, BVH, CULL, EDGES, TBK>(kargs_of_kernel, before);
                 return ~0u;
             }
             m -= before;
@@ -423,7 +445,7 @@
 #ifndef RM_CLASSIFY_WG_INLINE
 #define RM_CLASSIFY_WG_INLINE __forceinline__
 #endif
-template <bool ORDER, bool STAGED>
+template <bool ORDER, bool STAGED, bool TB = false>
 __device__ RM_CLASSIFY_WG_INLINE unsigned long long classify_workgroup(const char *kargs_of_kernel, uint32_t id_v, unsigned long long t_start) {
     const unsigned long long kv = (unsigned long long)kargs_of_kernel;
     const unsigned long long ku = ((unsigned long long)(uint32_t)__builtin_amdgcn_readfirstlane((int)(uint32_t)(kv >> 32)) << 32) |
@@ -499,251 +521,36 @@
 #endif
         order_places(a, id, rec, true, a.ord_rec == nullptr);
     }
+    if constexpr (TB) {
+        if (a.tile_bundles == 2u && a.mask_tag && a.cls_prims <= RM_TB_BITS) {
+            for (uint32_t it = 0; it < iters; it++) {
+                bool valid_it;
+                const uint32_t patch_it = patch_of(it, valid_it);
+                add_tile_bundles<true>(blob, a, scene_blob + a.H.off_lights, patch_it, valid_it, const_cast<unsigned long long *>(a.tile_mask));
+            }
+        }
+    }
     return stats;
 }
 
+template <int STACK, int POW, int WAVES, int TPW, bool STAGED, bool BVH, bool CULL, bool EDGES, bool ORDER, bool FEEDBACK>
+__device__ __forceinline__ void render_kernel_body(const double *__restrict__ scene_blob, const KernelArgs &a, double *__restrict__ frame) {
+    constexpr bool TBK = false;
+#include "rm_render_kernel_body.inc"
+}
 template <int STACK, int POW, int WAVES, int TPW, bool STAGED = true, bool BVH = false, bool CULL = false, bool EDGES = false, bool ORDER = false, bool FEEDBACK = false>
 __global__ __launch_bounds__(WAVES * 64) __attribute__((amdgpu_waves_per_eu(POW == POW_INTEGER ? (EDGES ? RM_EDGES_WAVES : RM_MIN_WAVES) : 1, 8))) void rm_render_static(const double *__restrict__ scene_blob, KernelArgs a,
                                                               double *__restrict__ frame) {
-    static_assert(WAVES == 1 && TPW == 1, "one tile per wave, one wave per workgroup");
-#ifdef RM_EXP_STAMPS
-    const unsigned long long t_start = __builtin_amdgcn_s_memrealtime();
-    unsigned long long tile_stats = 0;
-    uint32_t cull_counts[4] = {0u, 0u, 0u, 0u};
-    uint32_t st_tile = ~0u;
-    unsigned long long st_mask = ~0ull;
-    auto stamp = [&]() {
-        if ((threadIdx.x & 63u) == 0 && a.debug_stamps) {
-            unsigned long long *o = a.debug_stamps + 4ull * blockIdx.x;
-            o[0] = t_start; o[1] = tile_stats; o[2] = __builtin_amdgcn_s_memrealtime();
-            unsigned long long *x = a.debug_stamps + 4ull * gridDim.x + 2ull * blockIdx.x;
-#if defined(RM_EXP_WALKSTATS) || defined(RM_EXP_PHASES) || defined(RM_EXP_STARTUP)
-            o[3] = (unsigned long long)cull_counts[0] | ((unsigned long long)cull_counts[1] << 32);
-            x[0] = st_tile; x[1] = (unsigned long long)cull_counts[2] | ((unsigned long long)cull_counts[3] << 32);
-#else
-            o[3] = (unsigned long long)cull_counts[0] | ((unsigned long long)cull_counts[1] << 16) |
-                   ((unsigned long long)cull_counts[2] << 40) | ((unsigned long long)cull_counts[3] << 52);
-            x[0] = st_tile; x[1] = st_mask;
-#endif
-        }
-    };
-#else
-    auto stamp = []() {};
-#endif
-    const bool feedback = FEEDBACK && a.fb_flag != nullptr;
-    if (feedback && blockIdx.x == 0u) {
-        const uint32_t b = threadIdx.x;
-        a.fb_zero[b] = 0u;
-        if (b == 0u) a.fb_zero[RM_FB_BUCKETS] = 0u;
-        if (a.fb_target != 0u) {
-            uint32_t above = a.fb_hist[b] * RM_FB_SAMPLE;
-            for (uint32_t off = 1u; off < 64u; off <<= 1) {
-                const uint32_t o = (uint32_t)__shfl_down((int)above, off, 64);
-                above += (b + off < 64u) ? o : 0u;
-            }
-            const unsigned long long fits = __ballot(above <= a.fb_target);
-            const uint32_t first = (uint32_t)__builtin_ctzll(fits | (1ull << 63));
-            const uint32_t total = (uint32_t)__shfl((int)above, 0, 64);
-            if (b == 0u) *a.fb_threshold = total == 0u ? a.fb_long_ticks : max(fb_edge(first), 200u);
-        }
-    }
-
-    uint32_t id = blockIdx.x;
-    if (a.cls_blocks) {
-        if (id < a.cls_blocks) {
-#ifdef RM_EXP_STAMPS
-            tile_stats = classify_workgroup<ORDER, STAGED>((const char *)__builtin_amdgcn_kernarg_segment_ptr(), id, t_start);
-#else
-            (void)classify_workgroup<ORDER, STAGED>((const char *)__builtin_amdgcn_kernarg_segment_ptr(), id, 0ull);
-#endif
-            stamp();
-            return;
-        }
-        id -= a.cls_blocks;
-    }
-#ifdef RM_EARLY_LOADS
-    constexpr bool EARLY = ORDER;
-#else
-    constexpr bool EARLY = false;
-#endif
-    SceneAsked scene_asked;
-    if (STAGED && EARLY) scene_asked = stage_scene_ask(scene_blob, a.H);
-    uint32_t tile = 0u;
-    bool late = id >= a.first_round;
-    bool listed_tile = false;
-    if (ORDER && a.ord_cnt && id >= a.n_static) {
-        tile = uniform_u32(ordered_tile<STACK, POW, STAGED, BVH, CULL, EDGES>((const char *)__builtin_amdgcn_kernarg_segment_ptr(), id));
-        if (tile == ~0u) { stamp(); return; }
-        late = true;
-    } else if (feedback && id < a.fb_cap) {
-        if (id >= min(a.fb_count[0], a.fb_cap)) { stamp(); return; }
-        tile = a.fb_list[id];
-        if (tile >= a.n_tiles) { stamp(); return; }
-        listed_tile = true;
-    } else {
-        if (feedback) id -= a.fb_cap;
-        if (id >= a.n_tiles) { stamp(); return; }
-        if (ORDER && a.ord_cnt && a.static_list && a.lists_done) {
-            const uint32_t done = *a.lists_done, cand = a.static_list[id >> 4];
-            tile = done == a.lists_tag ? cand * 16u + (15u - (id & 15u)) : tile_of_id(a, id);
-        } else {
-            tile = tile_of_id(a, id);
-        }
-    }
-#if defined(RM_EXP_STAMPS) && defined(RM_EXP_STARTUP)
-    cull_counts[3] = (uint32_t)t_start;
-    cull_counts[0] = ((uint32_t)__builtin_amdgcn_s_memrealtime() - cull_counts[3]) & 0xFFFFu;
-#endif
-    const uint32_t flagged = (feedback && !listed_tile) ? a.fb_flag[tile] : 0u;
-    uint32_t tx0, ty0, tyf, ty8;
-    tile_origin(a, tile, tx0, ty0, tyf, ty8);
-    double bp_x = 0., bp_y = 0.;
-    if (FEEDBACK || EARLY) { bp_x = a.bp_x[tx0 + ((threadIdx.x & 63u) % TILE_W)]; bp_y = a.bp_y[ty0 + ((threadIdx.x & 63u) / TILE_W)]; }
-    uint32_t fb_thr = a.fb_long_ticks;
-    if (feedback && a.fb_target != 0u) {
-        fb_thr = __hip_atomic_load(a.fb_threshold, __ATOMIC_RELAXED, __HIP_MEMORY_SCOPE_AGENT);
-        fb_thr = fb_thr ? fb_thr : a.fb_long_ticks;
-    }
-    if (flagged) { stamp(); return; }
-
-    bool have_mask = a.tile_mask != nullptr && a.mask_exact != 0u;
-    unsigned long long first_mask = ~0ull;
-    if (a.tile_mask && a.mask_tag) {
-        have_mask = false;
-        if (late || a.mask_tag_prev) {
-            unsigned long long *word = const_cast<unsigned long long *>(a.tile_mask) + tile;
-            const unsigned long long t0 = __builtin_amdgcn_s_memrealtime();
-            if (a.mask_tag_prev) {
-                const unsigned long long w = a.tile_mask[tile];
-                if ((uint32_t)(w >> 56) == a.mask_tag || (uint32_t)(w >> 56) == a.mask_tag_prev) { first_mask = w & 0x00FFFFFFFFFFFFFFull; have_mask = true; }
-            }
-            while (!have_mask) {
-                const unsigned long long w = uniform_u64(__hip_atomic_load(word, __ATOMIC_RELAXED, __HIP_MEMORY_SCOPE_AGENT));
-                if ((uint32_t)(w >> 56) == a.mask_tag || (a.mask_tag_prev && (uint32_t)(w >> 56) == a.mask_tag_prev)) { first_mask = w & 0x00FFFFFFFFFFFFFFull; have_mask = true; break; }
-                if (__builtin_amdgcn_s_memrealtime() - t0 > 2000ull) break;
-                __builtin_amdgcn_s_sleep(4);
-            }
-        }
-    } else if (a.tile_mask) {
-        first_mask = uniform_u64(a.tile_mask[tile]);
-    }
-    if (a.tile_mask) {
-        if (first_mask == 0ull && !listed_tile) {
-            const uint32_t lane = threadIdx.x & 63u;
-            constexpr uint32_t PIECES = TILE_W * 3u / 2u, P8 = TILE_W * 3u / 8u;
-            for (uint32_t q = lane; q < 96u; q += 64u) {
-                double2 *dst = reinterpret_cast<double2 *>(frame + ((size_t)(tyf + q / PIECES) * a.frame_width + tx0) * 3u);
-                dst[q % PIECES] = double2{0., 0.};
-            }
-            if (a.frame8 && lane < 24u) {
-                unsigned long long *dst = reinterpret_cast<unsigned long long *>(a.frame8 + ((size_t)(ty8 + lane / P8) * a.frame_width + tx0) * 3u);
-                dst[lane % P8] = 0ull;
-            }
-            if (feedback && (threadIdx.x & 63u) == 0u) a.fb_next_flag[tile] = 0;
-            stamp();
-            return;
-        }
-    }
-
-#ifdef RM_EXP_STAMPS
-    st_tile = tile; st_mask = have_mask ? first_mask : ~0ull;
-#endif
-    have_mask = have_mask & (a.mask_exact != 0u);
-#if defined(RM_EXP_STAMPS) && defined(RM_EXP_STARTUP)
-    cull_counts[0] |= (((uint32_t)__builtin_amdgcn_s_memrealtime() - cull_counts[3]) & 0xFFFFu) << 16;
-#endif
-    if (STAGED) { if (EARLY) stage_scene_put(scene_asked, a.H); else stage_scene(scene_blob, a.H); }
-#if defined(RM_EXP_STAMPS) && defined(RM_EXP_STARTUP)
-    cull_counts[1] = ((uint32_t)__builtin_amdgcn_s_memrealtime() - cull_counts[3]) & 0xFFFFu;
-#endif
-    const uint32_t cull_words = (!STAGED && CULL) ? a.cull_lds_words : 0u;
-    if (!STAGED && CULL && cull_words) { cull_stage(scene_blob, a.H, rm_lds); __syncthreads(); }
-    double *wl = rm_lds + (STAGED ? a.H.total_words : cull_words);
-    if (ORDER && (threadIdx.x & 63u) == 0u) reinterpret_cast<uint32_t *>(wl + RM_WAVE_T0_WORDS)[0] = (uint32_t)__builtin_amdgcn_s_memrealtime();
-#ifdef RM_CHECKED_NS
-    constexpr bool CHECKED = STAGED && !BVH && !CULL;
-    namespace tile_ns = RM_CHECKED_NS;
-#else
-    constexpr bool CHECKED = false;
-    namespace tile_ns = RM_FLAVOR_NS;
-#endif
-    const unsigned long long fb_t0 = feedback ? __builtin_amdgcn_s_memrealtime() : 0ull;
-    bool exact = CHECKED && a.exact_only != 0u;
-    if (!exact) {
-        tile_ns::SceneView sc;
-        if (STAGED) sc.S = rm_lds; else sc.S = scene_blob;
-        sc.G = scene_blob;
-        sc.cull_bounds = cull_words ? rm_lds : scene_blob + a.H.off_bounds;
-        sc.cull_planar = cull_words ? rm_lds + 4u * (a.H.n_spheres + a.H.n_polygons + a.H.n_triangles) : scene_blob + a.H.off_planar;
-        sc.bstack = reinterpret_cast<uint32_t *>(wl + RM_WAVE_BVH_STACK_WORDS);
-        sc.cull_cos = own_sgpr(a.cull_cos);
-#ifdef RM_EXP_STAMPS
-        sc.cnt = cull_counts;
-#endif
-        sc.H.n_spheres = own_sgpr(a.H.n_spheres);         sc.H.n_polygons = own_sgpr(a.H.n_polygons);
-        sc.H.n_triangles = own_sgpr(a.H.n_triangles);     sc.H.n_lights = own_sgpr(a.H.n_lights);
-        sc.H.off_spheres = own_sgpr(a.H.off_spheres);     sc.H.off_polygons = own_sgpr(a.H.off_polygons);
-        sc.H.off_pverts = own_sgpr(a.H.off_pverts);       sc.H.off_triangles = own_sgpr(a.H.off_triangles);
-        sc.H.off_materials = own_sgpr(a.H.off_materials); sc.H.off_lights = own_sgpr(a.H.off_lights);
-        sc.H.off_keys = own_sgpr(a.H.off_keys);           sc.H.total_words = a.H.total_words;
-        sc.H.list_ordered = own_sgpr(a.H.list_ordered);   sc.H.off_bvh_spheres = own_sgpr(a.H.off_bvh_spheres);
-        sc.H.off_bvh_triangles = own_sgpr(a.H.off_bvh_triangles); sc.H.off_bounds = own_sgpr(a.H.off_bounds);
-        sc.H.off_planar = own_sgpr(a.H.off_planar);       sc.H.off_groups = own_sgpr(a.H.off_groups);
-        sc.H.off_occ = own_sgpr(a.H.off_occ);
-        sc.H.shadow_rho = own_sgpr(a.H.shadow_rho);
-
-#if defined(RM_EXP_STAMPS) && defined(RM_EXP_PHASES)
-        cull_counts[2] = (uint32_t)(__builtin_amdgcn_s_memrealtime() - t_start);
-#endif
-#ifdef RM_EXP_STAMPS
-        exact = tile_ns::render_tile<STACK, POW, BVH, CULL, EDGES, FEEDBACK || EARLY>(sc, a, tx0, ty0, tyf, ty8, bp_x, bp_y, wl, frame, &tile_stats, have_mask, first_mask, (const char *)__builtin_amdgcn_kernarg_segment_ptr());
-#else
-        exact = tile_ns::render_tile<STACK, POW, BVH, CULL, EDGES, FEEDBACK || EARLY>(sc, a, tx0, ty0, tyf, ty8, bp_x, bp_y, wl, frame, nullptr, have_mask, first_mask, (const char *)__builtin_amdgcn_kernarg_segment_ptr());
-#endif
-        if (CHECKED && exact) {
-            const KernelArgs &b = *reinterpret_cast<const KernelArgs *>(reread_kernargs((const char *)__builtin_amdgcn_kernarg_segment_ptr()) + sizeof(const double *));
-            if (b.redo_count && (threadIdx.x & 63u) == 0u) atomicAdd(b.redo_count, 1u);
-        }
-    }
-    if constexpr (CHECKED) if (exact) render_patch_alone<STACK, POW, STAGED, BVH, CULL, EDGES>((const char *)__builtin_amdgcn_kernarg_segment_ptr(), tile, 1u, true);
-    if (ORDER) {
-#ifdef RM_NO_REREAD
-        const KernelArgs &b = a;
-#else
-        const KernelArgs &b = *reinterpret_cast<const KernelArgs *>(reread_kernargs((const char *)__builtin_amdgcn_kernarg_segment_ptr()) + sizeof(const double *));
-#endif
-        if (b.patch_cost) {
-            const uint32_t dt = min(uniform_u32((uint32_t)__builtin_amdgcn_s_memrealtime() - reinterpret_cast<const uint32_t *>(wl + RM_WAVE_T0_WORDS)[0]), 0x00FFFFFFu);
-            if ((threadIdx.x & 63u) == 0u) RM_PATCH_COST_OP(b.patch_cost + (tile >> 4), dt);
-            if ((tile & 15u) == 0u && b.ctab_cur && b.tile_mask && b.mask_tag && b.mask_exact) {
-                const unsigned long long w = uniform_u64(__hip_atomic_load(const_cast<unsigned long long *>(b.tile_mask) + tile, __ATOMIC_RELAXED, __HIP_MEMORY_SCOPE_AGENT));
-                if ((uint32_t)(w >> 56) == b.mask_tag && ((w >> (threadIdx.x & 63u)) & 1ull) && (threadIdx.x & 63u) < 56u) {
-                    atomicAdd(b.ctab_cur + (threadIdx.x & 63u), dt >> 6);
-                    atomicAdd(b.ctab_cur + 64u + (threadIdx.x & 63u), 1u);
-                }
-            }
-        }
-    }
-#ifdef RM_EXP_STAMPS
-    if (a.tile_mask) st_mask = __hip_atomic_load(const_cast<unsigned long long *>(a.tile_mask) + tile, __ATOMIC_RELAXED, __HIP_MEMORY_SCOPE_AGENT) & 0x00FFFFFFFFFFFFFFull;
-#endif
-    if (feedback) {
-        const unsigned long long fb_dt = __builtin_amdgcn_s_memrealtime() - fb_t0;
-        const uint32_t ticks = fb_dt < 0x7FFFFFFFull ? (uint32_t)fb_dt : 0x7FFFFFFFu;
-        const bool is_long = ticks >= fb_thr;
-        if ((threadIdx.x & 63u) == 0u) {
-            if (a.fb_target != 0u && tile % RM_FB_SAMPLE == 0u) atomicAdd(a.fb_next_hist + fb_bucket(ticks), 1u);
-            bool listed = false;
-            if (is_long) {
-                const uint32_t slot = atomicAdd(a.fb_next_count, 1u);
-                if (slot < a.fb_cap) { a.fb_next_list[slot] = tile; listed = true; }
-            }
-            a.fb_next_flag[tile] = listed ? 1 : 0;
-        }
-    }
-    stamp();
-}
-
-#endif
-
-}
+    render_kernel_body<STACK, POW, WAVES, TPW, STAGED, BVH, CULL, EDGES, ORDER, FEEDBACK>(scene_blob, a, frame);
+}
+template <int STACK, int POW>
+__global__ __launch_bounds__(64) __attribute__((amdgpu_waves_per_eu(POW == POW_INTEGER ? RM_MIN_WAVES : 1, 8))) void rm_render_static_tb(const double *__restrict__ scene_blob, KernelArgs a,
+                                                              double *__restrict__ frame) {
+    constexpr int WAVES = 1, TPW = 1;
+    constexpr bool STAGED = true, BVH = false, CULL = false, EDGES = false, ORDER = true, FEEDBACK = false, TBK = tb_kernel<false, false>;
+#include "rm_render_kernel_body.inc"
+}
+
+#endif
+
+}
diff --git a/rusty-marcher_amd/csrc/rm_render_kernel_body.inc b/rusty-marcher_amd/csrc/rm_render_kernel_body.inc
--- /dev/null
+++ b/rusty-marcher_amd/csrc/rm_render_kernel_body.inc
@@ -0,0 +1,250 @@
+    static_assert(WAVES == 1 && TPW == 1, "one tile per wave, one wave per workgroup");
+    static_assert(!TBK || tb_kernel<BVH, CULL>, "the fields are the plain walk's, in the fixed view");
+#ifdef RM_EXP_STAMPS
+    const unsigned long long t_start = __builtin_amdgcn_s_memrealtime();
+    unsigned long long tile_stats = 0;
+    uint32_t cull_counts[4] = {0u, 0u, 0u, 0u};
+    uint32_t st_tile = ~0u;
+    unsigned long long st_mask = ~0ull;
+    auto stamp = [&]() {
+        if ((threadIdx.x & 63u) == 0 && a.debug_stamps) {
+            unsigned long long *o = a.debug_stamps + 4ull * blockIdx.x;
+            o[0] = t_start; o[1] = tile_stats; o[2] = __builtin_amdgcn_s_memrealtime();
+            unsigned long long *x = a.debug_stamps + 4ull * gridDim.x + 2ull * blockIdx.x;
+#if defined(RM_EXP_WALKSTATS) || defined(RM_EXP_PHASES) || defined(RM_EXP_STARTUP)
+            o[3] = (unsigned long long)cull_counts[0] | ((unsigned long long)cull_counts[1] << 32);
+            x[0] = st_tile; x[1] = (unsigned long long)cull_counts[2] | ((unsigned long long)cull_counts[3] << 32);
+#else
+            o[3] = (unsigned long long)cull_counts[0] | ((unsigned long long)cull_counts[1] << 16) |
+                   ((unsigned long long)cull_counts[2] << 40) | ((unsigned long long)cull_counts[3] << 52);
+            x[0] = st_tile; x[1] = st_mask;
+#endif
+        }
+    };
+#else
+    auto stamp = []() {};
+#endif
+    const bool feedback = FEEDBACK && a.fb_flag != nullptr;
+    if (feedback && blockIdx.x == 0u) {
+        const uint32_t b = threadIdx.x;
+        a.fb_zero[b] = 0u;
+        if (b == 0u) a.fb_zero[RM_FB_BUCKETS] = 0u;
+        if (a.fb_target != 0u) {
+            uint32_t above = a.fb_hist[b] * RM_FB_SAMPLE;
+            for (uint32_t off = 1u; off < 64u; off <<= 1) {
+                const uint32_t o = (uint32_t)__shfl_down((int)above, off, 64);
+                above += (b + off < 64u) ? o : 0u;
+            }
+            const unsigned long long fits = __ballot(above <= a.fb_target);
+            const uint32_t first = (uint32_t)__builtin_ctzll(fits | (1ull << 63));
+            const uint32_t total = (uint32_t)__shfl((int)above, 0, 64);
+            if (b == 0u) *a.fb_threshold = total == 0u ? a.fb_long_ticks : max(fb_edge(first), 200u);
+        }
+    }
+
+    uint32_t id = blockIdx.x;
+    if (a.cls_blocks) {
+        if (id < a.cls_blocks) {
+#ifdef RM_EXP_STAMPS
+            tile_stats = classify_workgroup<ORDER, STAGED, TBK>((const char *)__builtin_amdgcn_kernarg_segment_ptr(), id, t_start);
+#else
+            (void)classify_workgroup<ORDER, STAGED, TBK>((const char *)__builtin_amdgcn_kernarg_segment_ptr(), id, 0ull);
+#endif
+            stamp();
+            return;
+        }
+        id -= a.cls_blocks;
+    }
+#ifdef RM_EARLY_LOADS
+    constexpr bool EARLY = ORDER;
+#else
+    constexpr bool EARLY = false;
+#endif
+    SceneAsked scene_asked;
+    if (STAGED && EARLY) scene_asked = stage_scene_ask(scene_blob, a.H);
+    uint32_t tile = 0u;
+    bool late = id >= a.first_round;
+    bool listed_tile = false;
+    if (ORDER && a.ord_cnt && id >= a.n_static) {
+        tile = uniform_u32(ordered_tile<STACK, POW, STAGED, BVH, CULL, EDGES, TBK>((const char *)__builtin_amdgcn_kernarg_segment_ptr(), id));
+        if (tile == ~0u) { stamp(); return; }
+        late = true;
+    } else if (feedback && id < a.fb_cap) {
+        if (id >= min(a.fb_count[0], a.fb_cap)) { stamp(); return; }
+        tile = a.fb_list[id];
+        if (tile >= a.n_tiles) { stamp(); return; }
+        listed_tile = true;
+    } else {
+        if (feedback) id -= a.fb_cap;
+        if (id >= a.n_tiles) { stamp(); return; }
+        if (ORDER && a.ord_cnt && a.static_list && a.lists_done) {
+            const uint32_t done = *a.lists_done, cand = a.static_list[id >> 4];
+            tile = done == a.lists_tag ? cand * 16u + (15u - (id & 15u)) : tile_of_id(a, id);
+        } else {
+            tile = tile_of_id(a, id);
+        }
+    }
+#if defined(RM_EXP_STAMPS) && defined(RM_EXP_STARTUP)
+    cull_counts[3] = (uint32_t)t_start;
+    cull_counts[0] = ((uint32_t)__builtin_amdgcn_s_memrealtime() - cull_counts[3]) & 0xFFFFu;
+#endif
+    const uint32_t flagged = (feedback && !listed_tile) ? a.fb_flag[tile] : 0u;
+    uint32_t tx0, ty0, tyf, ty8;
+    tile_origin(a, tile, tx0, ty0, tyf, ty8);
+    double bp_x = 0., bp_y = 0.;
+    if (FEEDBACK || EARLY) { bp_x = a.bp_x[tx0 + ((threadIdx.x & 63u) % TILE_W)]; bp_y = a.bp_y[ty0 + ((threadIdx.x & 63u) / TILE_W)]; }
+    uint32_t fb_thr = a.fb_long_ticks;
+    if (feedback && a.fb_target != 0u) {
+        fb_thr = __hip_atomic_load(a.fb_threshold, __ATOMIC_RELAXED, __HIP_MEMORY_SCOPE_AGENT);
+        fb_thr = fb_thr ? fb_thr : a.fb_long_ticks;
+    }
+    if (flagged) { stamp(); return; }
+
+    bool have_mask = a.tile_mask != nullptr && a.mask_exact != 0u;
+    unsigned long long first_mask = ~0ull;
+    if (a.tile_mask && a.mask_tag) {
+        have_mask = false;
+        if (late || a.mask_tag_prev) {
+            unsigned long long *word = const_cast<unsigned long long *>(a.tile_mask) + tile;
+            const unsigned long long t0 = __builtin_amdgcn_s_memrealtime();
+            if (a.mask_tag_prev) {
+                const unsigned long long w = a.tile_mask[tile];
+                if ((uint32_t)(w >> 56) == a.mask_tag || (uint32_t)(w >> 56) == a.mask_tag_prev) { first_mask = w & 0x00FFFFFFFFFFFFFFull; have_mask = true; }
+            }
+            while (!have_mask) {
+                const unsigned long long w = uniform_u64(__hip_atomic_load(word, __ATOMIC_RELAXED, __HIP_MEMORY_SCOPE_AGENT));
+                if ((uint32_t)(w >> 56) == a.mask_tag || (a.mask_tag_prev && (uint32_t)(w >> 56) == a.mask_tag_prev)) { first_mask = w & 0x00FFFFFFFFFFFFFFull; have_mask = true; break; }
+                if (__builtin_amdgcn_s_memrealtime() - t0 > 2000ull) break;
+                __builtin_amdgcn_s_sleep(4);
+            }
+        }
+    } else if (a.tile_mask) {
+        first_mask = uniform_u64(a.tile_mask[tile]);
+    }
+    unsigned long long tb_word = 0ull;
+    if (TBK && a.tile_bundles && a.tile_mask && a.mask_tag) {
+        tb_word = have_mask ? first_mask >> RM_TB_BITS : 0ull;
+        first_mask = have_mask ? first_mask & RM_TB_FIELD : first_mask;
+    }
+    if (a.tile_mask) {
+        if (first_mask == 0ull && !listed_tile) {
+            const uint32_t lane = threadIdx.x & 63u;
+            constexpr uint32_t PIECES = TILE_W * 3u / 2u, P8 = TILE_W * 3u / 8u;
+            for (uint32_t q = lane; q < 96u; q += 64u) {
+                double2 *dst = reinterpret_cast<double2 *>(frame + ((size_t)(tyf + q / PIECES) * a.frame_width + tx0) * 3u);
+                dst[q % PIECES] = double2{0., 0.};
+            }
+            if (a.frame8 && lane < 24u) {
+                unsigned long long *dst = reinterpret_cast<unsigned long long *>(a.frame8 + ((size_t)(ty8 + lane / P8) * a.frame_width + tx0) * 3u);
+                dst[lane % P8] = 0ull;
+            }
+            if (feedback && (threadIdx.x & 63u) == 0u) a.fb_next_flag[tile] = 0;
+            stamp();
+            return;
+        }
+    }
+
+#ifdef RM_EXP_STAMPS
+    st_tile = tile; st_mask = have_mask ? first_mask : ~0ull;
+#endif
+    have_mask = have_mask & (a.mask_exact != 0u);
+    tb_word = have_mask ? tb_word : 0ull;
+#if defined(RM_EXP_STAMPS) && defined(RM_EXP_STARTUP)
+    cull_counts[0] |= (((uint32_t)__builtin_amdgcn_s_memrealtime() - cull_counts[3]) & 0xFFFFu) << 16;
+#endif
+    if (STAGED) { if (EARLY) stage_scene_put(scene_asked, a.H); else stage_scene(scene_blob, a.H); }
+#if defined(RM_EXP_STAMPS) && defined(RM_EXP_STARTUP)
+    cull_counts[1] = ((uint32_t)__builtin_amdgcn_s_memrealtime() - cull_counts[3]) & 0xFFFFu;
+#endif
+    const uint32_t cull_words = (!STAGED && CULL) ? a.cull_lds_words : 0u;
+    if (!STAGED && CULL && cull_words) { cull_stage(scene_blob, a.H, rm_lds); __syncthreads(); }
+    double *wl = rm_lds + (STAGED ? a.H.total_words : cull_words);
+    if (ORDER && (threadIdx.x & 63u) == 0u) reinterpret_cast<uint32_t *>(wl + RM_WAVE_T0_WORDS)[0] = (uint32_t)__builtin_amdgcn_s_memrealtime();
+#ifdef RM_CHECKED_NS
+    constexpr bool CHECKED = STAGED && !BVH && !CULL;
+    namespace tile_ns = RM_CHECKED_NS;
+#else
+    constexpr bool CHECKED = false;
+    namespace tile_ns = RM_FLAVOR_NS;
+#endif
+    const unsigned long long fb_t0 = feedback ? __builtin_amdgcn_s_memrealtime() : 0ull;
+    bool exact = CHECKED && a.exact_only != 0u;
+    if (!exact) {
+        tile_ns::SceneView sc;
+        if (STAGED) sc.S = rm_lds; else sc.S = scene_blob;
+        sc.G = scene_blob;
+        sc.cull_bounds = cull_words ? rm_lds : scene_blob + a.H.off_bounds;
+        sc.cull_planar = cull_words ? rm_lds + 4u * (a.H.n_spheres + a.H.n_polygons + a.H.n_triangles) : scene_blob + a.H.off_planar;
+        sc.bstack = reinterpret_cast<uint32_t *>(wl + RM_WAVE_BVH_STACK_WORDS);
+        sc.cull_cos = own_sgpr(a.cull_cos);
+#ifdef RM_EXP_STAMPS
+        sc.cnt = cull_counts;
+#endif
+        sc.H.n_spheres = own_sgpr(a.H.n_spheres);         sc.H.n_polygons = own_sgpr(a.H.n_polygons);
+        sc.H.n_triangles = own_sgpr(a.H.n_triangles);     sc.H.n_lights = own_sgpr(a.H.n_lights);
+        sc.H.off_spheres = own_sgpr(a.H.off_spheres);     sc.H.off_polygons = own_sgpr(a.H.off_polygons);
+        sc.H.off_pverts = own_sgpr(a.H.off_pverts);       sc.H.off_triangles = own_sgpr(a.H.off_triangles);
+        sc.H.off_materials = own_sgpr(a.H.off_materials); sc.H.off_lights = own_sgpr(a.H.off_lights);
+        sc.H.off_keys = own_sgpr(a.H.off_keys);           sc.H.total_words = a.H.total_words;
+        sc.H.list_ordered = own_sgpr(a.H.list_ordered);   sc.H.off_bvh_spheres = own_sgpr(a.H.off_bvh_spheres);
+        sc.H.off_bvh_triangles = own_sgpr(a.H.off_bvh_triangles); sc.H.off_bounds = own_sgpr(a.H.off_bounds);
+        sc.H.off_planar = own_sgpr(a.H.off_planar);       sc.H.off_groups = own_sgpr(a.H.off_groups);
+        sc.H.off_occ = own_sgpr(a.H.off_occ);
+        sc.H.shadow_rho = own_sgpr(a.H.shadow_rho);
+
+#if defined(RM_EXP_STAMPS) && defined(RM_EXP_PHASES)
+        cull_counts[2] = (uint32_t)(__builtin_amdgcn_s_memrealtime() - t_start);
+#endif
+#ifdef RM_EXP_STAMPS
+        if (TBK && tb_word != 0ull)
+            exact = tile_ns::render_tile<STACK, POW, BVH, CULL, EDGES, FEEDBACK || EARLY, TBK>(sc, a, tx0, ty0, tyf, ty8, bp_x, bp_y, wl, frame, &tile_stats, have_mask, first_mask, (const char *)__builtin_amdgcn_kernarg_segment_ptr(), tb_word);
+        else
+            exact = tile_ns::render_tile<STACK, POW, BVH, CULL, EDGES, FEEDBACK || EARLY>(sc, a, tx0, ty0, tyf, ty8, bp_x, bp_y, wl, frame, &tile_stats, have_mask, first_mask, (const char *)__builtin_amdgcn_kernarg_segment_ptr());
+#else
+        if (TBK && tb_word != 0ull)
+            exact = tile_ns::render_tile<STACK, POW, BVH, CULL, EDGES, FEEDBACK || EARLY, TBK>(sc, a, tx0, ty0, tyf, ty8, bp_x, bp_y, wl, frame, nullptr, have_mask, first_mask, (const char *)__builtin_amdgcn_kernarg_segment_ptr(), tb_word);
+        else
+            exact = tile_ns::render_tile<STACK, POW, BVH, CULL, EDGES, FEEDBACK || EARLY>(sc, a, tx0, ty0, tyf, ty8, bp_x, bp_y, wl, frame, nullptr, have_mask, first_mask, (const char *)__builtin_amdgcn_kernarg_segment_ptr());
+#endif
+        if (CHECKED && exact) {
+            const KernelArgs &b = *reinterpret_cast<const KernelArgs *>(reread_kernargs((const char *)__builtin_amdgcn_kernarg_segment_ptr()) + sizeof(const double *));
+            if (b.redo_count && (threadIdx.x & 63u) == 0u) atomicAdd(b.redo_count, 1u);
+        }
+    }
+    if constexpr (CHECKED) if (exact) render_patch_alone<STACK, POW, STAGED, BVH, CULL, EDGES, TBK>((const char *)__builtin_amdgcn_kernarg_segment_ptr(), tile, 1u, true);
+    if (ORDER) {
+#ifdef RM_NO_REREAD
+        const KernelArgs &b = a;
+#else
+        const KernelArgs &b = *reinterpret_cast<const KernelArgs *>(reread_kernargs((const char *)__builtin_amdgcn_kernarg_segment_ptr()) + sizeof(const double *));
+#endif
+        if (b.patch_cost) {
+            const uint32_t dt = min(uniform_u32((uint32_t)__builtin_amdgcn_s_memrealtime() - reinterpret_cast<const uint32_t *>(wl + RM_WAVE_T0_WORDS)[0]), 0x00FFFFFFu);
+            if ((threadIdx.x & 63u) == 0u) RM_PATCH_COST_OP(b.patch_cost + (tile >> 4), dt);
+            if ((tile & 15u) == 0u && b.ctab_cur && b.tile_mask && b.mask_tag && b.mask_exact) {
+                const unsigned long long w = uniform_u64(__hip_atomic_load(const_cast<unsigned long long *>(b.tile_mask) + tile, __ATOMIC_RELAXED, __HIP_MEMORY_SCOPE_AGENT));
+                if ((uint32_t)(w >> 56) == b.mask_tag && ((w >> (threadIdx.x & 63u)) & 1ull) && (threadIdx.x & 63u) < ((TBK && b.tile_bundles) ? RM_TB_BITS : 56u)) {
+                    atomicAdd(b.ctab_cur + (threadIdx.x & 63u), dt >> 6);
+                    atomicAdd(b.ctab_cur + 64u + (threadIdx.x & 63u), 1u);
+                }
+            }
+        }
+    }
+#ifdef RM_EXP_STAMPS
+    if (a.tile_mask) st_mask = __hip_atomic_load(const_cast<unsigned long long *>(a.tile_mask) + tile, __ATOMIC_RELAXED, __HIP_MEMORY_SCOPE_AGENT) & ((TBK && a.tile_bundles) ? RM_TB_FIELD : 0x00FFFFFFFFFFFFFFull);
+#endif
+    if (feedback) {
+        const unsigned long long fb_dt = __builtin_amdgcn_s_memrealtime() - fb_t0;
+        const uint32_t ticks = fb_dt < 0x7FFFFFFFull ? (uint32_t)fb_dt : 0x7FFFFFFFu;
+        const bool is_long = ticks >= fb_thr;
+        if ((threadIdx.x & 63u) == 0u) {
+            if (a.fb_target != 0u && tile % RM_FB_SAMPLE == 0u) atomicAdd(a.fb_next_hist + fb_bucket(ticks), 1u);
+            bool listed = false;
+            if (is_long) {
+                const uint32_t slot = atomicAdd(a.fb_next_count, 1u);
+                if (slot < a.fb_cap) { a.fb_next_list[slot] = tile; listed = true; }
+            }
+            a.fb_next_flag[tile] = listed ? 1 : 0;
+        }
+    }
+    stamp();
diff --git a/rusty-marcher_amd/csrc/rm_trace.inc b/rusty-marcher_amd/csrc/rm_trace.inc
--- a/rusty-marcher_amd/csrc/rm_trace.inc
+++ b/rusty-marcher_amd/csrc/rm_trace.inc
@@ -975,7 +975,8 @@
 
 template <int POW, bool BVH, bool CULL, bool EDGES, class LIGHTS = StoredLights, class SPHERES = StoredSpheres>
 __device__ __forceinline__ V3 shade_direct(const SceneView &sc, V3 neg_dir, const Surface &s, bool got, uint32_t pid RM_SUS_PARAM,
-                                           const LIGHTS &lights = LIGHTS(), const SPHERES &spheres = SPHERES()) {
+                                           const LIGHTS &lights = LIGHTS(), const SPHERES &spheres = SPHERES(), bool tb = false,
+                                           unsigned long long tb0 = 0ull, unsigned long long tb1 = 0ull) {
     const double *m = s.mat;
     const double exponent = m[5];
     const V3 dir_to_viewer = neg_dir;
@@ -1008,8 +1009,10 @@
                 const V3 from = pick(dec_a, b.from, a.from);
                 unsigned long long m_a = 0ull, m_b = 0ull;
                 if (masks) shadow_masks2(sc, got, pid, l, m_a, m_b);
+                const bool bundles = tb & (l == 0u);
+                if (bundles) { m_a = masks ? m_a & tb0 : tb0; m_b = masks ? m_b & tb1 : tb1; }
                 const uint32_t n = sc.H.n_spheres + sc.H.n_polygons + sc.H.n_triangles;
-                if (masks && (m_a & m_b) != ((n >= 64u) ? ~0ull : (1ull << n) - 1ull))
+                if ((masks | bundles) && (m_a & m_b) != ((n >= 64u) ? ~0ull : (1ull << n) - 1ull))
                     any_hit2_masked(sc, from, a.dir, b.dir, dec_a, dec_b, occ_a, occ_b, m_a, m_b);
                 else
                     any_hit2(sc, from, a.dir, b.dir, dec_a, dec_b, occ_a, occ_b, spheres);
```

Result: faster. 33280 (median of 6 runs) (+2.2%).
